# castorini/dhr

Measured on AMD Instinct MI355X. Metric: queries/sec (exact top-1000, brute-force dense-hybrid GIP retrieval), higher is better.
Workload: dtype i8 (bound GEMM: gated AND ungated columns int8 x int8 -> int32 on the matrix cores, every gated rounding upward, the ungated quantisation error paid by the filter margin) + f64-accumulated f16 x f32 exact rescoring of the survivors -- the returned scores are the exact scores rounded once, identical

## Files before the change

dhr_amd/csrc/dhr_internal.h:

```cpp
#pragma once
#include <hip/hip_runtime.h>
#include <hip/hip_fp16.h>
#include <stdint.h>

#include "../../include/dhr_hip.h"
#include "abi_guard.h"

extern "C" int dhr_set_error_message(int code, const char* msg);
extern "C" int dhr_index_device(const dhr_index* ix);
extern "C" void dhr_internal_index_arena(dhr_index* ix, void*** base, size_t** bytes);
extern "C" int dhr_internal_search_begin_async(dhr_index* ix, const dhr_query_batch* qb, int32_t k, float* out_sample_scores_dev, void* stream);
extern "C" void dhr_internal_search_abort(dhr_index* ix);
extern "C" int dhr_internal_search_pre_async(dhr_index* ix, const dhr_query_batch* qb, int32_t k, int32_t r_local, float* out_scores_dev, void* stream);
extern "C" int dhr_internal_search_begin_rest_async(dhr_index* ix, const float* tau_dev, float* out_sample_scores_dev, void* stream);
extern "C" int dhr_internal_search_mid_async(dhr_index* ix, const float* tau_hat_dev, int32_t r_local, float* out_scores_dev, void* stream);
extern "C" int dhr_internal_search_finish_async(dhr_index* ix, const float* tau_hat_dev, float* out_scores, int64_t* out_rows, int32_t* out_count_dev,
                                                int32_t out_mem_kind, void* stream);

namespace dhr {

constexpr int TILE_ROWS = 256;
constexpr int TILE_K = 64;
constexpr int CHUNK = 8;
constexpr int TILE_HALVES = TILE_ROWS * TILE_K;
// ... 127 lines not shown
__host__ __device__ inline int quant_i8(float v, float inv_scale) {
  float r = rintf(v * inv_scale);
  r = r < -127.f ? -127.f : (r > 127.f ? 127.f : r);
  return (int)r;
}

struct RescoreArgs {
  const __half* vals_rm;
  const void* c_idx;
  int c_idx_dtype;
  const float* q32;
  const int16_t* q_idx;
  const __half* q16; const uint8_t* q_idx8; const uint32_t* q_inexact;
  int d_dlr, k_rm;
  int gate;
  int64_t n_rows;
  const uint2* cand; const uint32_t* cnt; uint32_t cap;
  const uint32_t* rows32;
  int64_t ld_rows;
  int64_t row0; uint32_t count_all;
  const float* thr_exact;
  uint64_t* out_keys;
  int64_t ld_keys;
  float* out_scores;
  int64_t ld_scores;
  int n_queries;
  uint32_t max_count;
  const uint32_t* blk_off; uint32_t flat_blocks;
  int split;
};

struct SelectArgs {
  uint64_t* topk_keys;
  const uint64_t* in_keys;
  int64_t ld_keys;
  const uint32_t* cnt;
  uint32_t count_all, cap;
  int k, kp, sort_n;
  int k_keep;
  int kps;
  int monotone;
  const float* margin;
  float* tau;
  float* thr;
  int n_queries;
};

hipError_t launch_scan_rows(const __half* src, int64_t ld, int64_t n_rows, int d_dlr, int k, uint32_t* max_sq_bits,
                            uint32_t* neg_flag, hipStream_t s);
hipError_t launch_i8_row_err(const __half* vals_rm, int k_rm, int64_t n_rows, int d_dlr, int d_cls, float scale, const float* col_scale,
                             uint32_t* out_bits, hipStream_t s);
hipError_t launch_col_absmax(const __half* vals_rm, int k_rm, int64_t n_rows, int col0, int n_cols, uint32_t* colmax_bits, hipStream_t s);
hipError_t launch_tile_rows_sparse(const __half* src, int64_t ld, int64_t row_lo, int64_t n_rows_src, int64_t n_rows_fill,
                                   int d_dlr, int d_cls, int ts, int td, const void* idx, int idx_dtype, const uint8_t* map,
                                   bool abs_dlr, char* tiles, float i8_inv_scale , const float* col_scale,
                                   const float* g8_inv_cs , hipStream_t s);
hipError_t launch_g8_row_sum(const __half* vals_rm, int k_rm, int64_t n_rows, int64_t n_rows_fill, int d_dlr, bool abs_dlr, const float* g8_inv_cs,
                             int32_t* rsum128, hipStream_t s);
hipError_t launch_copy_rows(const __half* src, int64_t ld, int64_t n_rows, int k, int k_rm, __half* dst, hipStream_t s);
hipError_t launch_idx_hist(const uint8_t* idx, const __half* vals_rm, int k_rm, int64_t n_rows, int d_dlr, float* hist, hipStream_t s);
struct G8Prep {
  const float* inv_cs;
  const float* w;
  float s_ref;
  int max_shift;
  uint8_t* q8;
  int32_t* shift;
  float* unit;
  float* thr_raise;
  float resid_ec2;
};
hipError_t launch_query_prep(const void* src, int src_is_f32, int64_t ld, const void* idx, int idx_dtype, int64_t ld_idx,
                             int n_queries, int q_pad, int d_dlr, int d_cls, int k_rm, int n_buckets, int kt,
                             const uint8_t* map, bool abs_dlr, float dmax, __half* q_tiles, float* q32, int16_t* q_idx,
                             float* margin, float* tau, float* thr, int ts, int td, uint32_t* q_pack, __half* q16, uint8_t* q_idx8,
                             uint32_t* q_inexact, int c_idx_dtype,
                             float i8_scale , float i8_ec, float i8_nc, float* i8_mul, const float* col_scale,
                             const G8Prep& g8, hipStream_t s);
#if defined(__HIPCC__)
constexpr int MAP_SPREAD_Q = 0x100;
__device__ __forceinline__ bool gemm_wg_tile(const GemmArgs& p, int64_t& dt, int& qt) {
  const int r = (int)blockIdx.y;
  const int mode = p.map_mode;
  int64_t seq;
  if (mode & MAP_SPREAD_Q) {
    const int qg = r / DOC_GROUP;
    const int dl = r - qg * DOC_GROUP;
    qt = qg * 8 + (int)blockIdx.x;
    if (qt >= p.n_qtiles) return false;
    seq = p.seq_lo + (int64_t)blockIdx.z * DOC_GROUP + dl;
  } else {
    qt = r / DOC_GROUP;
    const int dl = r - qt * DOC_GROUP;
    seq = p.seq_lo + ((int64_t)blockIdx.z * 8 + (int64_t)blockIdx.x) * DOC_GROUP + dl;
  }
  if (seq >= p.seq_hi) return false;
  dt = seq_to_tile_fast(seq, mode & 0xff, p.period, p.head, p.perm_mul, p.perm_n, p.inv_perm_n, p.inv_pm1);
  return dt < p.n_tiles;
}
#endif
inline int sparse_query_stages(int ts, bool gated, bool g8 = false) { return ts > 0 ? ((gated || g8) ? ts : 2 * ts) : 0; }
hipError_t launch_gemm_filter(const GemmArgs& a, hipStream_t s);
hipError_t launch_heavy_build(const __half* vals_rm, int k_rm, const void* idx, int idx_dtype, int64_t n_rows, int d_dlr,
                              const uint8_t* map, int n_buckets, uint32_t* heavy_key, __half* heavy_val,
                              const float* g8_inv_cs , int abs_mode, hipStream_t s);
#ifndef REFINE_PER_WG_N
#define REFINE_PER_WG_N 512
#endif
constexpr int REFINE_PER_WG = REFINE_PER_WG_N;
struct RefineArgs {
  const uint2* cand; const uint32_t* cnt; uint32_t cap;
  const uint2* ovf; const uint32_t* ovf_off; const uint32_t* ovf_cap;
  const uint32_t* heavy_key; const __half* heavy_val;
  const uint32_t* q_pack; int d_dlr;
  const float* thr;
  uint2* out; uint32_t* out_cnt; uint32_t out_cap;
  int n_queries; uint32_t max_count;
  const uint32_t* blk_off; uint32_t flat_blocks;
  const uint8_t* g8_q8;
  const float* g8_inv_cs;
  const float* g8_unit;
  int abs_mode;
  int ungated;
  const uint8_t* resid8; int resid_ld;
  const float* q32; int64_t q32_ld;
  const float* col_scale; int d_cls;
  const float* thr_raise;
};
hipError_t launch_resid_build(const __half* vals_rm, int k_rm, int64_t n_rows, int d_dlr, int d_cls, const float* col_scale, uint8_t* resid8, int resid_ld, hipStream_t s);
hipError_t launch_refine(const RefineArgs& a, hipStream_t s);
hipError_t launch_rescore(const RescoreArgs& a, hipStream_t s);
hipError_t launch_select(const SelectArgs& a, hipStream_t s);
hipError_t launch_select_global(const SelectArgs& a, hipStream_t s);
hipError_t launch_merge_topk_global(int n_queries, int n_in, const float* in_scores, const int64_t* in_rows, int k_out, float* out_scores,
                                    int64_t* out_rows, hipStream_t s);
hipError_t launch_emit(const uint64_t* topk_keys, int kp, int n_queries, int k, int64_t row_offset, float* out_scores,
                       int64_t* out_rows, hipStream_t s);
hipError_t launch_keys_to_rows(const uint64_t* topk_keys, int kp, int n_queries, int k, uint32_t* rows, hipStream_t s);
hipError_t launch_bound_topm(const float* bound , int n_rows, int n_queries, int m, uint32_t* rows , hipStream_t s);
hipError_t launch_densify(const void* lex, int in_is_f32, int64_t ld, int64_t batch, int remove, int dims, int n_groups, void* out_val,
                          int val_is_f32, int64_t ld_val, void* out_idx, int idx_is_i16, int64_t ld_idx, hipStream_t s);
hipError_t launch_pq_init(const __half* vals, int64_t ld, int64_t n, int64_t stride, int dsub, int M, float* cb, int ksub, hipStream_t s);
hipError_t launch_pq_assign(const __half* vals, int64_t ld, int64_t n, int64_t stride, int dsub, int M, const float* cb, uint8_t* codes,
                            int64_t ld_codes, float* sums, uint32_t* counts, float* err, int ksub, hipStream_t s);
hipError_t launch_pq_update(float* cb, const float* sums, const uint32_t* counts, int dsub, int M, int ksub, hipStream_t s);
hipError_t launch_pq_decode(const uint8_t* codes, int64_t ld_codes, int64_t n, int M, int dsub, const float* cb, __half* out, int64_t ld_out,
                            int ksub, hipStream_t s);
hipError_t launch_block_offsets(const uint32_t* cnt, uint32_t cap, int n_queries, uint32_t per, uint32_t* offs, hipStream_t s);
hipError_t launch_plan_overflow(const uint32_t* cnt_prev, double rows_ratio, uint32_t cap, uint32_t max_extra, uint32_t arena_entries, int n_queries,
                                uint32_t* ovf_off, uint32_t* ovf_cap, hipStream_t s);
hipError_t launch_max_u32(const uint32_t* v, int n, uint32_t* out_max, unsigned long long* out_sum, hipStream_t s);
hipError_t launch_lists_ready(const uint32_t* cnt, uint32_t cap, int n_queries, uint32_t per, uint32_t* offs, uint32_t* out_max, uint32_t* out_max2,
                              unsigned long long* out_sum, unsigned long long* out_sum2, uint32_t* fail_flags, uint32_t* zero, int n_zero,
                              hipStream_t s, const uint32_t* ovf_cap = nullptr);
hipError_t launch_rows_to_local(const int64_t* rows, int64_t n, int64_t row_offset, int64_t n_rows, uint32_t* out,
                                hipStream_t s);
hipError_t launch_mark_overflow(const uint32_t* cnt, uint32_t cap, int n_queries, uint32_t* fail_flags, hipStream_t s);
hipError_t launch_verify(const uint64_t* topk_keys, int kp, int k, const float* tau_hat, int n_queries, uint32_t* fail_flags,
                         uint32_t* n_fail, hipStream_t s);
hipError_t launch_gather_queries(const float* q32, const int16_t* q_idx, int k_rm, int d_dlr, const int32_t* ids, int n,
                                 float* out32, int16_t* out_idx, hipStream_t s);
hipError_t launch_scatter_keys(const uint64_t* src, uint64_t* dst, int kp, const int32_t* ids, int n, hipStream_t s);
hipError_t launch_emit_scores(const uint64_t* topk_keys, int kp, int n_queries, int r, float* out, hipStream_t s);
hipError_t launch_make_thr(const float* tau, const float* margin, int n_queries, int q_pad, float* thr, hipStream_t s);
hipError_t launch_raise_thr(float* thr_hat, const float* thr_run, int n_queries, hipStream_t s);
hipError_t launch_flag_tau_above(const float* tau_own, const float* tau_ext, int n_queries, uint32_t* fail_flags, hipStream_t s);
hipError_t launch_raise_thr_rank(float* thr_hat, float* tau_hat, const uint64_t* topk_keys, int kp, int r, const float* margin, int n_queries, hipStream_t s);
hipError_t launch_count_ge(const uint64_t* topk_keys, int kp, int k, const float* tau, const uint32_t* fail_flags, int n_queries,
                           int32_t* out, hipStream_t s);
hipError_t launch_merge_topk(int n_queries, int n_in, const float* in_scores, const int64_t* in_rows, int k_out,
                             float* out_scores, int64_t* out_rows, hipStream_t s);
hipError_t launch_merge_lists(int n_queries, int n_lists, int list_len, const float* in_scores, const int64_t* in_rows, int k_out,
                              float* out_scores, int64_t* out_rows, hipStream_t s, int64_t stride_s = 0, int64_t stride_r = 0);

extern int g_gemm_variant;
extern thread_local int g_last_gemm_kernel;
constexpr int RESCORE_CANDS_PER_WG = 32;
constexpr uint32_t FLAT_GRID_MAX = 1u << 20;
constexpr uint32_t FLAT_GRID_ASYNC = 16384;
constexpr int SELECT_THREADS = 1024;

}
```

dhr_amd/csrc/dhr_state.h:

```cpp
#pragma once
#include <algorithm>
#include <cmath>
#include <cstdio>
#include <cstring>
#include <string>
#include <vector>

#include "dhr_internal.h"
#include "search_plan.h"
#include <hip/hip_ext.h>

using namespace dhr;
static_assert(plan::TILE_ROWS == TILE_ROWS && plan::DOC_GROUP == DOC_GROUP, "search_plan.h restates the tile geometry of dhr_internal.h");
using plan::BOOT_M;
using plan::SearchPlan;
using plan::round_up;

inline int set_error(int code, const std::string& msg) { return dhr_set_error_message(code, msg.c_str()); }
#define HIP_TRY(expr)                                                                                          \
  do {                                                                                                         \
    hipError_t _e = (expr);                                                                                    \
    if (_e != hipSuccess)                                                                                      \
      return set_error(DHR_ERR_HIP, std::string(#expr) + ": " + hipGetErrorString(_e) + " (" __FILE__ ":" +    \
                                        std::to_string(__LINE__) + ")");                                       \
  } while (0)

struct DevMem {
  void* p = nullptr;
  DevMem() = default;
  DevMem(const DevMem&) = delete;
  DevMem& operator=(const DevMem&) = delete;
  ~DevMem() { if (p) (void)hipFree(p); }
};
struct Events {
  std::vector<hipEvent_t> v;
  Events() = default;
  Events(const Events&) = delete;
  Events& operator=(const Events&) = delete;
  ~Events() { for (hipEvent_t e : v) if (e) (void)hipEventDestroy(e); }
  hipError_t add(hipEvent_t* out, unsigned flags = hipEventDefault) {
    v.reserve(v.size() + 1);
    hipEvent_t e = nullptr;
    const hipError_t rc = hipEventCreateWithFlags(&e, flags);
    if (rc == hipSuccess) v.push_back(e);
    *out = e;
    return rc;
  }
};
static inline int idx_esize(int dt) { return dt == DHR_IDX_I16 ? 2 : 1; }

struct Workspace {
  int q_pad = 0, kp = 0;
  int q_alloc = 0;
  int64_t cap = 0;
  int64_t cap_deep = 0;
  int64_t arena = 0;
  uint2 *ovf = nullptr, *ovf2 = nullptr;
  uint32_t *ovf_off = nullptr, *ovf_cap = nullptr;
  uint32_t* boot_rows = nullptr;
  float* boot_bound = nullptr;
  bool keys_alias = false;
  ListTier* tier_dev = nullptr;
  uint32_t* cnt_plan = nullptr;
  int64_t plan_rows = 0;
  uint32_t last_maxr = 0;
  int64_t cap_r = 0;
  int64_t keys_ld = 0, kt = 0, d_dlr = 0;
  int ts_q = 0;
  __half* q_tiles = nullptr;
  float* q32 = nullptr;
  int16_t* q_idx = nullptr;
  __half* q16 = nullptr;
  uint8_t* q_idx8 = nullptr;
  uint32_t* q_inexact = nullptr;
  float *margin = nullptr, *tau = nullptr, *thr = nullptr;
  float* i8_mul = nullptr;
  uint8_t* g8_q8 = nullptr;
  int32_t* g8_shift = nullptr;
  float* g8_unit = nullptr;
  uint32_t* cnt = nullptr;
  uint2* cand = nullptr;
  uint64_t *rs_keys = nullptr, *topk_keys = nullptr;
  uint32_t* d_max = nullptr;
  float* tau_hat = nullptr;
  float* thr_hat = nullptr;
  uint32_t* fail_flags = nullptr;
  uint32_t* q_pack = nullptr;
  float* thr_raise = nullptr;
  uint2* cand_r = nullptr;
  uint32_t* cnt_r = nullptr;
  uint32_t* blk_off = nullptr;
  uint2* cand2 = nullptr;
  uint32_t* cnt2 = nullptr;
  void* h_pinned = nullptr;
  char* h_pinned2 = nullptr;
  uint32_t* d_max2 = nullptr;
  unsigned long long* d_stats = nullptr;
  void* h_stats = nullptr;
  uint32_t* d_ref = nullptr;
  void* h_ref = nullptr;
  void* q_stage = nullptr;  size_t q_stage_bytes = 0;
  void* qi_stage = nullptr; size_t qi_stage_bytes = 0;
  void* out_stage = nullptr; size_t out_stage_bytes = 0;
  int64_t bytes = 0;
};

enum class StagedState { None, AfterPre, AfterBegin, AfterMid, Complete };
enum class Stage { Whole, Begin, Finish, Mid, Pre, BeginRest };

struct dhr_index {
  int device = 0;
  int64_t n_rows = 0, n_tiles = 0, row_offset = 0;
  int d_dlr = 0, d_cls = 0, k = 0, idx_dtype = DHR_IDX_NONE;
  int dlr_pad = 0;
  int k_rm = 0;
  int n_buckets = 1;
  int idx_buckets_req = 0;
  int kt = 0;
  int ksteps = 0;
  int ts = 0, td = 0;
  __half* tiles = nullptr;
  __half* vals_rm = nullptr;
  void* c_idx = nullptr;
  uint8_t* bucket_map = nullptr;
  uint32_t* heavy_key = nullptr;
  __half* heavy_val = nullptr;
  bool abs_mode = false;
  float dmax = 0.f;
  bool dense_i8 = false;
  float i8_scale = 0.f, i8_ec = 0.f, i8_nc = 0.f;
  uint8_t* resid8 = nullptr;
  int resid_ld = 0;
  float resid_ec2 = 0.f;
  float* i8_col_scale = nullptr;
  bool gated_i8 = false;
  float g8_sref = 0.f;
  int g8_max_shift = 0;
  float* g8_inv_cs = nullptr;
  float* g8_w = nullptr;
  int32_t* g8_rsum = nullptr;
  int64_t index_bytes = 0;
  int64_t cand_cap = 0, first_rows = 0;
  int64_t list_stride = 0;
  int profile = 0, max_growth16 = 32;
  int sample_period = 32;
  int async_ctl = 2;
  int sample_share = 1;
  int main_chunks = 2;
  int progressive_thr = 2;
  int n_cu = 256;
  int gemm_variant = 0;
  int last_gemm_kernel = 0;
  int overlap_aux = -1;
  int aux_cus = -1, gemm_exclusive = 0;
  int aux_cus_made = -1, gemm_excl_made = -1;
  hipStream_t s_gemm = nullptr;
  hipStream_t s_aux = nullptr;
  struct {
    StagedState state = StagedState::None;
    bool gate = false; int Q = 0, k = 0;
    double rate = 0.0, rate_r = 0.0;
    int64_t dev_bound = 0, dev_exact = 0;
    int64_t pre_pos = 0, pre_seen = 0, pre_last_rows = 0;
  } pend;
  Workspace ws, ws_fb[2];
  void* sh_arena = nullptr;
  size_t sh_arena_bytes = 0;
  dhr_search_stats stats{};
};

inline void free_ws(Workspace& w) {
  hipFree(w.q_tiles); hipFree(w.q32); hipFree(w.q_idx); hipFree(w.q16); hipFree(w.q_idx8); hipFree(w.q_inexact); hipFree(w.margin); hipFree(w.i8_mul); hipFree(w.g8_q8); hipFree(w.g8_shift); hipFree(w.g8_unit); hipFree(w.tau); hipFree(w.thr);
  hipFree(w.cnt); hipFree(w.cand); if (!w.keys_alias) hipFree(w.rs_keys); hipFree(w.topk_keys); hipFree(w.d_max); hipFree(w.tau_hat); hipFree(w.fail_flags); hipFree(w.thr_hat); hipFree(w.cand2); hipFree(w.cnt2); hipFree(w.q_pack); hipFree(w.cand_r); hipFree(w.cnt_r); hipFree(w.thr_raise); hipFree(w.blk_off); hipFree(w.ovf); hipFree(w.ovf2); hipFree(w.ovf_off); hipFree(w.ovf_cap); hipFree(w.cnt_plan); hipFree(w.tier_dev); hipFree(w.boot_rows); hipFree(w.boot_bound);
  if (w.h_pinned) hipHostFree(w.h_pinned);
  if (w.h_pinned2) hipHostFree(w.h_pinned2);
  hipFree(w.d_max2); hipFree(w.d_ref); hipFree(w.d_stats);
  if (w.h_ref) hipHostFree(w.h_ref);
  if (w.h_stats) hipHostFree(w.h_stats);
  hipFree(w.q_stage); hipFree(w.qi_stage); hipFree(w.out_stage);
  w = Workspace();
}


constexpr int32_t MEM_DEVICE_PADDED = 2;
#ifndef SELECT_SORT_Q
#define SELECT_SORT_Q 8
#endif
inline int select_sort_n(int kp) { return kp * SELECT_SORT_Q / 4; }
enum { T_GEMM = 0, T_REFINE = 1, T_RESCORE = 2, T_SELECT = 3, T_PREP = 4 };
struct Drain {
  dhr_index* ix; hipStream_t s; bool armed = true;
  ~Drain() {
    if (!armed) return;
    (void)hipStreamSynchronize(s);
    if (ix->s_aux) (void)hipStreamSynchronize(ix->s_aux);
    if (ix->s_gemm) (void)hipStreamSynchronize(ix->s_gemm);
    (void)hipGetLastError();
  }
};
struct Timer {
  bool on; hipStream_t s; std::vector<std::pair<hipEvent_t, hipEvent_t>> ev; std::vector<int> kind;
  ~Timer() { for (auto& e : ev) { (void)hipEventDestroy(e.first); (void)hipEventDestroy(e.second); } }
  void begin(int k) { begin_on(k, s); }
  void end() { end_on(s); }
  void begin_on(int k, hipStream_t st) { if (!on) return; ev.reserve(ev.size() + 1); kind.reserve(kind.size() + 1); hipEvent_t a, b; hipEventCreate(&a); hipEventCreate(&b); hipEventRecord(a, st); ev.push_back({a, b}); kind.push_back(k); }
  void end_on(hipStream_t st) { if (!on) return; hipEventRecord(ev.back().second, st); }
  void collect(double* ms ) {
    for (size_t i = 0; i < ev.size(); ++i) {
      float t = 0.f;
      if (hipEventElapsedTime(&t, ev[i].first, ev[i].second) == hipSuccess) ms[kind[i]] += t;
      hipEventDestroy(ev[i].first); hipEventDestroy(ev[i].second);
    }
    ev.clear(); kind.clear();
  }
};

int ensure_ws(dhr_index* ix, Workspace& w, int n_queries, int k, int64_t keys_ld_min, int64_t cap_mult = 1, bool use_refine = true, bool queries_only = false);
int check_queries(const dhr_index* ix, const dhr_query_batch* qb);
int grow(void*& p, size_t& have, size_t need, int64_t& total);
int prep_queries(dhr_index* ix, Workspace& w, const dhr_query_batch* qb, hipStream_t s);
dhr::RescoreArgs base_rescore_args(const dhr_index* ix, const Workspace& w, int n_queries, bool gate);
inline SearchPlan search_plan_of(const dhr_index* ix, int k, int depth, bool staged) {
  plan::PlanInput in;
  in.n_rows = ix->n_rows; in.n_tiles = ix->n_tiles; in.k = k; in.sample_period = ix->sample_period; in.sample_share = ix->sample_share;
  in.first_rows = ix->first_rows; in.depth = depth; in.staged = staged;
  return plan::make_search_plan(in);
}
inline void staged_set(dhr_index* ix, StagedState to) { ix->pend.state = to; }
inline void staged_open(dhr_index* ix, StagedState to, bool gate, int Q, int k) { staged_set(ix, to); ix->pend.gate = gate; ix->pend.Q = Q; ix->pend.k = k; }
int search_core(dhr_index* ix, Workspace& w, const dhr_query_batch* qb, int k, int depth, Timer& tm, dhr_search_stats& st, hipStream_t s,
                Stage stage = Stage::Whole, const float* tau_ext = nullptr);
```

dhr_amd/csrc/gemm_g8.hip:

```cpp
#include "gemm_g8.h"
#include <mutex>
#include <type_traits>

#ifndef G8_TRACE
#define G8_TRACE 0
#endif
#ifndef G8_ABL
#define G8_ABL 0
#endif
namespace dhr {

#if G8_TRACE
constexpr int G8_TRACE_SLOTS = 1 << 18;
__device__ unsigned long long g8_trace_buf[G8_TRACE_SLOTS * 8];
__device__ unsigned int g8_trace_n;
#define G8_T(i) do { if (threadIdx.x == 0 && tslot < G8_TRACE_SLOTS) g8_trace_buf[(size_t)tslot * 8 + (i)] = __builtin_readcyclecounter(); } while (0)
#else
#define G8_T(i) do { } while (0)
#endif
__device__ __forceinline__ void g8_dump_tile(const GemmArgs& p, floatx16 (&acc)[4][2], int64_t dt, int qt, int wm, int wn, int lane,
                                             const float (&mul_r)[2]) {
  const int fhalf = lane >> 5;
  const int64_t row_base = dt * TILE_ROWS + wm * 128;
#pragma unroll
  for (int ni = 0; ni < 2; ++ni) {
    const int q = qt * TILE_ROWS + wn * 64 + ni * 32 + (lane & 31);
    if (q < p.n_queries) {
#pragma unroll
      for (int mi = 0; mi < 4; ++mi)
#pragma unroll
        for (int e = 0; e < 16; ++e) {
          const int64_t row = row_base + mi * 32 + (e & 3) + 8 * (e >> 2) + 4 * fhalf;
          if (row < p.n_rows && row >= p.dump_row0 && row - p.dump_row0 < p.dump_ld)
            p.dump[(int64_t)q * p.dump_ld + (row - p.dump_row0)] = g8_score(__float_as_int(acc[mi][ni][e]), mul_r[ni]);
        }
    }
  }
}

template <bool SURPLUS, int NI_, bool CHECK_ROWS = true>
__device__ __forceinline__ void g8_scan_half(const GemmArgs& p, floatx16 (&acc)[4][2], int qt, int wm, int wn, int lane, int rows_valid, int64_t row0,
                                             uint2* stack, const int t, const float mul, uint32_t& j) {
  const int fhalf = lane >> 5;
  const int rbase = wm * 128 + 4 * fhalf;
  const int q = qt * TILE_ROWS + wn * 64 + NI_ * 32 + (lane & 31);
#pragma unroll
  for (int mi = 0; mi < 4; ++mi) {
    const floatx16& a = acc[mi][NI_];
#pragma unroll
    for (int g = 0; g < 4; ++g) {
      const int gm = max(max(__float_as_int(a[4 * g]), __float_as_int(a[4 * g + 1])), max(__float_as_int(a[4 * g + 2]), __float_as_int(a[4 * g + 3])));
      if (gm >= t) {
        asm volatile("");
        if constexpr (!SURPLUS && !CHECK_ROWS) {
#pragma unroll
          for (int e = 4 * g; e < 4 * g + 4; ++e) {
            const int v = __float_as_int(a[e]);
            const int rl = rbase + mi * 32 + (e & 3) + 8 * (e >> 2);
            const uint32_t slot = j < (uint32_t)EPI_STACK ? j : (uint32_t)EPI_STACK;
            stack[slot * G8_NT] = make_uint2((uint32_t)rl, (uint32_t)v);
            j += v >= t ? 1u : 0u;
          }
        } else
#pragma unroll
        for (int e = 4 * g; e < 4 * g + 4; ++e) {
          const int v = __float_as_int(a[e]);
          const int rl = rbase + mi * 32 + (e & 3) + 8 * (e >> 2);
          if (v >= t && (!CHECK_ROWS || rl < rows_valid)) {
            asm volatile("");
            if constexpr (SURPLUS) {
              if (j >= EPI_STACK) {
                const uint32_t slot = atomicAdd(p.cnt + q, 1u);
                cand_store(p, q, slot, make_uint2((uint32_t)(row0 + rl), __float_as_uint(g8_score(v, mul))));
              }
            } else if (j < EPI_STACK) stack[j * G8_NT] = make_uint2((uint32_t)rl, (uint32_t)v);
            ++j;
          }
        }
      }
    }
  }
}
__device__ __forceinline__ void g8_epilogue_surplus(const GemmArgs& p, floatx16 (&acc)[4][2], int qt, int wm, int wn, int lane, int rows_valid, int64_t row0,
                                                 const int (&thr_r)[2], const float (&mul_r)[2]) {
  uint32_t j = 0;
  g8_scan_half<true, 0>(p, acc, qt, wm, wn, lane, rows_valid, row0, nullptr, thr_r[0], mul_r[0], j);
  g8_scan_half<true, 1>(p, acc, qt, wm, wn, lane, rows_valid, row0, nullptr, thr_r[1], mul_r[1], j);
}
__device__ __forceinline__ void g8_epilogue(const GemmArgs& p, floatx16 (&acc)[4][2], int64_t dt, int qt, int wm, int wn, int tid, int lane,
                                            char* smem, const int (&thr_r)[2], const float (&mul_r)[2]) {
  __syncthreads();
  const int64_t row0 = dt * TILE_ROWS;
  const int rows_valid = (int)(p.n_rows - row0 < TILE_ROWS ? p.n_rows - row0 : TILE_ROWS);
  uint2* stack = (uint2*)smem + tid;
  const int q0 = qt * TILE_ROWS + wn * 64 + (lane & 31);
  const bool full = rows_valid == TILE_ROWS;
  uint32_t j = 0;
  if (full) g8_scan_half<false, 0, false>(p, acc, qt, wm, wn, lane, rows_valid, row0, stack, thr_r[0], mul_r[0], j);
  else g8_scan_half<false, 0, true>(p, acc, qt, wm, wn, lane, rows_valid, row0, stack, thr_r[0], mul_r[0], j);
  const uint32_t s0 = j < (uint32_t)EPI_STACK ? j : (uint32_t)EPI_STACK;
#if G8_ABL != 16
  uint32_t base0 = 0u, base1 = 0u;
  if (s0 > 0) base0 = atomicAdd(p.cnt + q0, s0);
#endif
  if (full) g8_scan_half<false, 1, false>(p, acc, qt, wm, wn, lane, rows_valid, row0, stack, thr_r[1], mul_r[1], j);
  else g8_scan_half<false, 1, true>(p, acc, qt, wm, wn, lane, rows_valid, row0, stack, thr_r[1], mul_r[1], j);
  const uint32_t s1 = j < (uint32_t)EPI_STACK ? j : (uint32_t)EPI_STACK;
#if G8_ABL == 16
  return;
#else
  if (s1 > s0) base1 = atomicAdd(p.cnt + q0 + 32, s1 - s0);
  if (__builtin_amdgcn_ballot_w64(j > (uint32_t)EPI_STACK) != 0) g8_epilogue_surplus(p, acc, qt, wm, wn, lane, rows_valid, row0, thr_r, mul_r);
  for (uint32_t i = 0; i < s0; ++i) {
    const uint2 en = stack[i * G8_NT];
    const uint32_t slot = base0 + i;
    cand_store(p, q0, slot, make_uint2((uint32_t)row0 + en.x, __float_as_uint(g8_score((int)en.y, mul_r[0]))));
  }
  for (uint32_t i = s0; i < s1; ++i) {
    const uint2 en = stack[i * G8_NT];
    const uint32_t slot = base1 + (i - s0);
    cand_store(p, q0 + 32, slot, make_uint2((uint32_t)row0 + en.x, __float_as_uint(g8_score((int)en.y, mul_r[1]))));
  }
#endif
}

#if G8_ABL == 2
#define G8_PAIR_SYNC() do { asm volatile("s_waitcnt lgkmcnt(0)" ::: "memory"); __builtin_amdgcn_s_barrier(); } while (0)
#elif G8_ABL == 3
#define G8_PAIR_SYNC() do { asm volatile("s_waitcnt lgkmcnt(0)" ::: "memory"); } while (0)
#else
#define G8_PAIR_SYNC() do { asm volatile("s_waitcnt vmcnt(0) lgkmcnt(0)" ::: "memory"); __builtin_amdgcn_s_barrier(); } while (0)
#endif

#ifndef G8_DMA_SCHED
#define G8_DMA_SCHED 1
#endif
#if G8_DMA_SCHED == 1
__host__ __device__ constexpr int g8_dma_piece(int ph, int g) { return ph == 0 ? g : -1; }
#elif G8_DMA_SCHED == 2
__host__ __device__ constexpr int g8_dma_piece(int ph, int g) { return ph == 0 ? (g >= 2 ? g - 2 : -1) : (ph == 1 && g < 2) ? 6 + g : -1; }
#else
__host__ __device__ constexpr int g8_dma_piece(int ph, int g) { return (ph <= 1 && (g & 1)) ? ph * 4 + (g >> 1) : -1; }
#endif

template <bool DUMP, bool PARTIAL>
__device__ __forceinline__ void g8_tile(const GemmArgs& p, char* smem, const int64_t dt, const int qt, const unsigned tslot = 0) {
  const int lane = threadIdx.x & 63;
  const int wave = __builtin_amdgcn_readfirstlane(threadIdx.x >> 6);
  const int ts = p.ts, td = p.td;
  const int nsp = ts >> 1, npairs = (ts + td) >> 1;
  const char* a_src = (const char*)p.a_tiles + dt * ((int64_t)ts * S8_STAGE_A + (int64_t)td * SP_DENSE);
  const char* b_src = (const char*)p.b_tiles + (int64_t)qt * ((int64_t)ts * SP_STAGE_B + (int64_t)td * SP_DENSE);
  const int wm = PARTIAL ? (wave & 1) : (wave >> 2), wn = PARTIAL ? (wave >> 1) : (wave & 3);
  const bool active = !PARTIAL || wn < p.partial_wn;

  const bool dma_b = ((wave >> 1) & 1) != 0;
  const int dma_s = wave >> 2;
  const int dma_h = wave & 1;
  const uint32_t lane_off = (uint32_t)lane * 16u;
  const uint32_t smem_u = (uint32_t)(uintptr_t)LDS_PTR(smem);
  const __amdgpu_buffer_rsrc_t role_rsrc = __builtin_amdgcn_make_buffer_rsrc((void*)(dma_b ? b_src : a_src), (short)0, 0x7fffffff, 0x00020000);
  int dma_soff = 0, dma_n = 0, nx_soff = 0, nx_n = 0;
  uint32_t dma_lds = 0, nx_lds = 0;
  auto dma_prepare = [&](int g) __attribute__((always_inline)) {
    const int u = 2 * g + dma_s;
    const bool sp = u < ts;
    const int half_bytes = dma_h * ((!dma_b && sp) ? S8_STAGE_A / 2 : 8192);
    if (dma_b) nx_soff = (sp ? u * SP_STAGE_B : ts * SP_STAGE_B + (u - ts) * SP_DENSE) + half_bytes;
    else nx_soff = (sp ? u * S8_STAGE_A : ts * S8_STAGE_A + (u - ts) * SP_DENSE) + half_bytes;
    nx_lds = smem_u + (uint32_t)((u & 3) * G8_SLOT + (dma_b ? G8_QOFF : 0) + half_bytes);
    nx_n = g < npairs ? ((!dma_b && sp) ? 5 : 8) : 0;
    if ((G8_ABL == 4 || G8_ABL == 8) && g >= 2) nx_n = 0;
  };
  auto dma_commit = [&]() __attribute__((always_inline)) { dma_soff = nx_soff; dma_lds = nx_lds; dma_n = nx_n; };
  auto dma_piece = [&](int j) __attribute__((always_inline)) {
    if (j < dma_n) {
      __attribute__((address_space(3))) void* l = (__attribute__((address_space(3))) void*)(uintptr_t)(dma_lds + (uint32_t)(j >> 2) * 4096u);
      const int so = dma_soff + (j >> 2) * 4096;
      switch (j & 3) {
        case 0: __builtin_amdgcn_raw_ptr_buffer_load_lds(role_rsrc, l, 16, (int)lane_off, so, 0, 0); break;
        case 1: __builtin_amdgcn_raw_ptr_buffer_load_lds(role_rsrc, l, 16, (int)lane_off, so, 1024, 0); break;
        case 2: __builtin_amdgcn_raw_ptr_buffer_load_lds(role_rsrc, l, 16, (int)lane_off, so, 2048, 0); break;
        default: __builtin_amdgcn_raw_ptr_buffer_load_lds(role_rsrc, l, 16, (int)lane_off, so, 3072, 0); break;
      }
    }
  };
  auto issue_pair = [&](int g) {
    dma_prepare(g);
    dma_commit();
#pragma unroll
    for (int j = 0; j < 8; ++j) dma_piece(j);
  };

  floatx16 acc[4][2];
  const int frow = lane & 31;
  const int fhalf = lane >> 5;
  const int swz4 = (frow >> 2) & 3;
  const int c0 = (fhalf ^ swz4) << 4, c1 = ((2 + fhalf) ^ swz4) << 4;
  const int a8_off = ((wm * 8 + fhalf) * 32 + frow) * 16;
  const int p8_off = S8_A_BYTES + ((wm * 2 + fhalf) * 32 + frow) * 16;
  const int ad_row = (wm * 128 + frow) * 64;
  const int q_row = G8_QOFF + (wn * 64 + frow) * 64;

  auto read_s8 = [&](G8Frag& f, const char* sl, int g) __attribute__((always_inline)) {
    if (g < 4) f.b[g >> 1].h[g & 1] = *(const intx4*)(sl + q_row + (g >> 1) * 2048 + ((g & 1) ? c1 : c0));
    else if (g < 8) f.a[g - 4] = *(const intx4*)(sl + a8_off + (g - 4) * 1024);
    else if (g == 8) f.pw = *(const intx4*)(sl + p8_off);
  };
  auto read_dn = [&](G8Frag& f, const char* sl, int cc, int g) __attribute__((always_inline)) {
    if (g < 2) f.b[g].h[0] = *(const intx4*)(sl + q_row + g * 2048 + cc);
    else if (g < 6) f.a[g - 2] = *(const intx4*)(sl + ad_row + (g - 2) * 2048 + cc);
  };
  auto blk_s8 = [&](const G8Frag& fc, G8Frag& fn, int un, bool do_load, auto ph_c) __attribute__((always_inline)) {
    constexpr int PH = decltype(ph_c)::value;
    const char* sl = smem + (un & 3) * G8_SLOT;
#pragma unroll
    for (int g = 0; g < 8; ++g) {
      const int ni = g >> 2, mi = g & 3;
      if (!PARTIAL || active) {
        if (do_load && G8_ABL != 8) {
          read_s8(fn, sl, g);
          if (g == 0) read_s8(fn, sl, 8);
        }
        g8_smfmac(acc[mi][ni], fc.a[mi], fc.b[ni].v, (uint32_t)fc.pw[mi]);
      }
      if (g8_dma_piece(PH, g) >= 0) dma_piece(g8_dma_piece(PH, g));
      __builtin_amdgcn_sched_barrier(0);
    }
  };
  auto blk_dn = [&](const G8Frag& fc, G8Frag& fn, int tn, bool do_load, auto ph_c) __attribute__((always_inline)) {
    constexpr int PH = decltype(ph_c)::value;
    const char* sl = smem + ((ts + (tn >> 1)) & 3) * G8_SLOT;
    const int cc = (tn & 1) ? c1 : c0;
#pragma unroll
    for (int g = 0; g < 8; ++g) {
      const int ni = g >> 2, mi = g & 3;
      if (!PARTIAL || active) {
        if (do_load && G8_ABL != 8) read_dn(fn, sl, cc, g);
        g8_mfma(acc[mi][ni], fc.a[mi], fc.b[ni].h[0]);
      }
      if (g8_dma_piece(PH, g) >= 0) dma_piece(g8_dma_piece(PH, g));
      __builtin_amdgcn_sched_barrier(0);
    }
  };

  if (wave < 4 && (ts > 0 || wave == 1 || wave == 2)) {
    const char* src = wave == 0 ? (const char*)(p.g8_rsum + dt * TILE_ROWS) : wave == 1 ? (const char*)(p.i8_mul + qt * TILE_ROWS)
                    : wave == 2 ? (const char*)(p.thr + qt * TILE_ROWS) : (const char*)(p.g8_shift + qt * TILE_ROWS);
    __builtin_amdgcn_global_load_lds(GLOBAL_PTR(src + lane_off), LDS_PTR(smem + G8_META + wave * 1024), 16, 0, 0);
  }
  issue_pair(0);
  if (npairs > 1) {
    issue_pair(1);
    if (dma_n == 5) asm volatile("s_waitcnt vmcnt(5)" ::: "memory"); else asm volatile("s_waitcnt vmcnt(8)" ::: "memory");
  } else asm volatile("s_waitcnt vmcnt(0)" ::: "memory");
  __builtin_amdgcn_s_barrier();
  G8_T(2);
  if (ts > 0) {
    const int32_t* rs = (const int32_t*)(smem + G8_META) + wm * 128 + 4 * (lane >> 5);
#pragma unroll
    for (int mi = 0; mi < 4; ++mi)
#pragma unroll
      for (int g4 = 0; g4 < 4; ++g4) {
        const intx4 v = *(const intx4*)(rs + mi * 32 + 8 * g4);
#pragma unroll
        for (int i4 = 0; i4 < 4; ++i4) acc[mi][0][4 * g4 + i4] = acc[mi][1][4 * g4 + i4] = __int_as_float(v[i4]);
      }
  } else {
#pragma unroll
    for (int mi = 0; mi < 4; ++mi)
#pragma unroll
      for (int e = 0; e < 16; ++e) acc[mi][0][e] = acc[mi][1][e] = 0.f;
  }
  int sh_r[2];
  float mul_r[2], thr_f[2];
#pragma unroll
  for (int ni = 0; ni < 2; ++ni) {
    const int ql = wn * 64 + ni * 32 + (lane & 31);
    mul_r[ni] = ((const float*)(smem + G8_META + 1024))[ql];
    thr_f[ni] = ((const float*)(smem + G8_META + 2048))[ql];
    sh_r[ni] = ts > 0 ? ((const int*)(smem + G8_META + 3072))[ql] : 0;
    asm volatile("" : "+v"(mul_r[ni]), "+v"(thr_f[ni]), "+v"(sh_r[ni]));
  }
  G8Frag f0, f1;
  if (ts > 0) {
#pragma unroll
    for (int g = 0; g < 9; ++g) read_s8(f0, smem, g);
  }
  if (G8_ABL == 8) f1 = f0;
  constexpr std::integral_constant<int, 0> PH0{};
  constexpr std::integral_constant<int, 1> PH1{};
  constexpr std::integral_constant<int, 2> PH2{};
  dma_n = 0;
#pragma unroll 1
  for (int g = 0; g + 1 < nsp; ++g) {
    blk_s8(f0, f1, 2 * g + 1, true, PH1);
    dma_prepare(g + 2);
    __builtin_amdgcn_sched_barrier(0);
    G8_PAIR_SYNC();
    dma_commit();
    blk_s8(f1, f0, 2 * g + 2, true, PH0);
  }
  if (nsp > 0) {
    const int g = nsp - 1;
    blk_s8(f0, f1, 2 * g + 1, true, PH1);
    dma_prepare(g + 2);
    __builtin_amdgcn_sched_barrier(0);
    G8_PAIR_SYNC();
    dma_commit();
    blk_s8(f1, f0, 2 * g + 2, false, PH0);
  }
  G8_T(3);
  if (td > 0) {
    __builtin_amdgcn_sched_barrier(0);
    asm volatile("s_waitcnt lgkmcnt(0)\n\ts_nop 15\n\ts_nop 7" ::: "memory");
    __builtin_amdgcn_sched_barrier(0);
    if (ts > 0)
#pragma unroll
    for (int mi = 0; mi < 4; ++mi)
#pragma unroll
      for (int ni = 0; ni < 2; ++ni)
#pragma unroll
        for (int e = 0; e < 16; ++e) acc[mi][ni][e] = __uint_as_float(__float_as_uint(acc[mi][ni][e]) << sh_r[ni]);
    __builtin_amdgcn_sched_barrier(0);
    {
      const char* sl = smem + (ts & 3) * G8_SLOT;
#pragma unroll
      for (int g = 0; g < 6; ++g) read_dn(f0, sl, c0, g);
    }
    asm volatile("s_nop 4" ::: "memory");
    __builtin_amdgcn_sched_barrier(0);
#pragma unroll 1
    for (int g = nsp; g + 1 < npairs; ++g) {
      const int t0 = 4 * (g - nsp);
      blk_dn(f0, f1, t0 + 1, true, PH1);
      blk_dn(f1, f0, t0 + 2, true, PH2);
      blk_dn(f0, f1, t0 + 3, true, PH2);
      dma_prepare(g + 2);
      __builtin_amdgcn_sched_barrier(0);
      G8_PAIR_SYNC();
      dma_commit();
      blk_dn(f1, f0, t0 + 4, true, PH0);
    }
    {
      const int g = npairs - 1;
      const int t0 = 4 * (g - nsp);
      blk_dn(f0, f1, t0 + 1, true, PH1);
      blk_dn(f1, f0, t0 + 2, true, PH2);
      blk_dn(f0, f1, t0 + 3, true, PH2);
      dma_prepare(g + 2);
      __builtin_amdgcn_sched_barrier(0);
      G8_PAIR_SYNC();
      dma_commit();
      blk_dn(f1, f0, t0 + 4, false, PH0);
    }
  }
  G8_T(4);
  asm volatile("s_waitcnt vmcnt(0) lgkmcnt(0)\n\ts_nop 15\n\ts_nop 7" ::: "memory");
  G8_T(5);
  if (DUMP) { g8_dump_tile(p, acc, dt, qt, wm, wn, lane, mul_r); return; }
  int thr_r[2];
#pragma unroll
  for (int ni = 0; ni < 2; ++ni) {
    asm volatile("" : "+v"(thr_f[ni]));
    thr_r[ni] = g8_thr_units(thr_f[ni], mul_r[ni]);
  }
#if G8_ABL == 32
  if (p.n_queries >= 0) { if (__float_as_int(acc[0][0][0]) == 0x7fffffff) p.cnt[0] = 1; return; }
#endif
  if (PARTIAL && !active) { __syncthreads(); return; }
  g8_epilogue(p, acc, dt, qt, wm, wn, (int)threadIdx.x, lane, smem, thr_r, mul_r);
}

#define G8_KERNEL_ATTR __attribute__((amdgpu_waves_per_eu(2, 2)))
template <bool DUMP>
__global__ void __launch_bounds__(G8_NT) G8_KERNEL_ATTR gemm_filter_g8_kernel(GemmArgs p) {
  extern __shared__ __attribute__((aligned(16))) char smem[];
  int64_t dt;
  int qt;
  if (!gemm_wg_tile(p, dt, qt)) return;
#if G8_TRACE
  unsigned tslot = 0;
  if (threadIdx.x == 0) tslot = atomicAdd(&g8_trace_n, 1u);
  tslot = __builtin_amdgcn_readfirstlane(tslot);
  if (threadIdx.x == 0 && tslot < G8_TRACE_SLOTS) {
    unsigned hw, xcc;
    asm volatile("s_getreg_b32 %0, hwreg(HW_REG_HW_ID)" : "=s"(hw));
    asm volatile("s_getreg_b32 %0, hwreg(HW_REG_XCC_ID)" : "=s"(xcc));
    g8_trace_buf[(size_t)tslot * 8 + 0] = __builtin_amdgcn_s_memrealtime();
    g8_trace_buf[(size_t)tslot * 8 + 7] = (unsigned long long)hw | ((unsigned long long)(xcc & 0xf) << 32) | ((unsigned long long)qt << 40) | ((unsigned long long)(dt & 0xffff) << 48);
  }
  G8_T(1);
  if (!DUMP && p.partial_wn > 0 && qt == p.n_qtiles - 1) g8_tile<false, true>(p, smem, dt, qt, tslot);
  else g8_tile<DUMP, false>(p, smem, dt, qt, tslot);
  G8_T(6);
#else
  if (!DUMP && p.partial_wn > 0 && qt == p.n_qtiles - 1) g8_tile<false, true>(p, smem, dt, qt);
  else g8_tile<DUMP, false>(p, smem, dt, qt);
#endif
}
#if G8_TRACE
}
extern "C" int dhr_debug_g8_trace(unsigned long long* out, int max_slots, unsigned* n_out) try {
  unsigned n = 0;
  if (hipMemcpyFromSymbol(&n, HIP_SYMBOL(dhr::g8_trace_n), 4) != hipSuccess) return -1;
  if (n_out) *n_out = n;
  const unsigned m = n < (unsigned)max_slots ? n : (unsigned)max_slots;
  const unsigned mm = m < (unsigned)dhr::G8_TRACE_SLOTS ? m : (unsigned)dhr::G8_TRACE_SLOTS;
  if (out && mm && hipMemcpyFromSymbol(out, HIP_SYMBOL(dhr::g8_trace_buf), (size_t)mm * 64) != hipSuccess) return -1;
  const unsigned zero = 0;
  if (hipMemcpyToSymbol(HIP_SYMBOL(dhr::g8_trace_n), &zero, 4) != hipSuccess) return -1;
  return 0;
} DHR_CATCH_STATUS
namespace dhr {
#endif

hipError_t launch_gemm_g8(const GemmArgs& a, dim3 grid, hipStream_t s) {
  static std::mutex attr_mu;
  static bool attr_set_dev[64] = {};
  int dev_ = 0;
  (void)hipGetDevice(&dev_);
  {
    std::lock_guard<std::mutex> attr_lock(attr_mu);
    bool& attr_set = attr_set_dev[dev_ & 63];
    if (!attr_set) {
      hipError_t e = hipFuncSetAttribute((const void*)gemm_filter_g8_kernel<false>, hipFuncAttributeMaxDynamicSharedMemorySize, G8_RING_LDS);
      if (e != hipSuccess) return e;
      e = hipFuncSetAttribute((const void*)gemm_filter_g8_kernel<true>, hipFuncAttributeMaxDynamicSharedMemorySize, G8_RING_LDS);
      if (e != hipSuccess) return e;
      attr_set = true;
    }
  }
  if (a.dump) { hipLaunchKernelGGL(gemm_filter_g8_kernel<true>, grid, dim3(G8_NT), G8_RING_LDS, s, a); return hipGetLastError(); }
  GemmArgs b = a;
  constexpr int partial_on = 1;
  const int valid_last = a.n_queries - (a.n_qtiles - 1) * TILE_ROWS;
  b.partial_wn = (partial_on && valid_last > 0 && valid_last <= 128) ? (valid_last + 63) / 64 : 0;
  hipLaunchKernelGGL(gemm_filter_g8_kernel<false>, grid, dim3(G8_NT), G8_RING_LDS, s, b);
  return hipGetLastError();
}

}
```

dhr_amd/csrc/index_build.hip:

```cpp
#include <fcntl.h>
#include <sys/mman.h>
#include <sys/stat.h>
#include <unistd.h>

#include "dhr_state.h"

extern "C" void dhr_index_destroy(dhr_index* ix) try {
  if (!ix) return;
  hipSetDevice(ix->device);
  free_ws(ix->ws);
  free_ws(ix->ws_fb[0]);
  free_ws(ix->ws_fb[1]);
  if (ix->s_aux) hipStreamDestroy(ix->s_aux);
  if (ix->s_gemm) hipStreamDestroy(ix->s_gemm);
  hipFree(ix->sh_arena);
  hipFree(ix->resid8); hipFree(ix->i8_col_scale); hipFree(ix->g8_inv_cs); hipFree(ix->g8_w); hipFree(ix->g8_rsum); hipFree(ix->tiles); hipFree(ix->c_idx); hipFree(ix->vals_rm); hipFree(ix->bucket_map); hipFree(ix->heavy_key);
  delete ix;
} DHR_CATCH_VOID

static int g_opt_dense_i8 = -1;
static int g_opt_gated_i8 = -1;
constexpr int64_t GATED_I8_MIN_ROWS = 1000000, GATED_I8_MIN_ROWS_NARROW = 4000000;
constexpr int64_t DENSE_ONLY_I8_MIN_ROWS = 1000000;
extern "C" int dhr_set_option(int32_t option, int64_t value) try {
  if (option == DHR_OPT_DENSE_I8) { g_opt_dense_i8 = value < 0 ? -1 : (value != 0); return DHR_OK; }
  if (option == DHR_OPT_GATED_I8) { g_opt_gated_i8 = value < 0 ? -1 : (value != 0); return DHR_OK; }
  return set_error(DHR_ERR_INVALID, "unknown option");
} DHR_CATCH_STATUS
extern "C" int dhr_index_get_info(const dhr_index* ix, int32_t what, double* out) try {
  if (!ix || !out) return set_error(DHR_ERR_INVALID, "null argument");
  switch (what) {
    case DHR_INFO_DENSE_I8: *out = ix->dense_i8 ? 1.0 : 0.0; return DHR_OK;
    case DHR_INFO_I8_SCALE: *out = ix->i8_scale; return DHR_OK;
    case DHR_INFO_I8_ROW_ERR: *out = ix->i8_ec; return DHR_OK;
    case DHR_INFO_I8_ROW_NORM: *out = ix->i8_nc; return DHR_OK;
    case DHR_INFO_ROW_NORM_MAX: *out = ix->dmax; return DHR_OK;
    case DHR_INFO_GATED_I8: *out = ix->gated_i8 ? 1.0 : 0.0; return DHR_OK;
    case DHR_INFO_GEMM_KERNEL: *out = (double)ix->last_gemm_kernel; return DHR_OK;
    case DHR_INFO_TILE_BYTES: *out = (double)((size_t)ix->n_tiles * ((size_t)ix->ts * (ix->gated_i8 ? S8_STAGE_A : SP_STAGE_A) + (size_t)ix->td * SP_DENSE)); return DHR_OK;
  }
  return set_error(DHR_ERR_INVALID, "unknown info id");
} DHR_CATCH_STATUS

extern "C" int dhr_index_set_param(dhr_index* ix, int32_t param, int64_t value) try {
  if (!ix) return set_error(DHR_ERR_INVALID, "null index");
  switch (param) {
    case DHR_PARAM_CAND_CAP:
      if (value < DOC_GROUP * TILE_ROWS || value > (1 << 22)) return set_error(DHR_ERR_INVALID, "cand_cap must be in [1024, 4194304]");
      ix->cand_cap = value; return DHR_OK;
    case DHR_PARAM_FIRST_ROWS:
      if (value < 0) return set_error(DHR_ERR_INVALID, "first_rows must be >= 0");
      ix->first_rows = value; return DHR_OK;
    case DHR_PARAM_PROFILE: ix->profile = value != 0; return DHR_OK;
    case DHR_PARAM_SAMPLE_PERIOD:
      if (value < 0 || value > 256) return set_error(DHR_ERR_INVALID, "sample_period must be in [0,256] (0/1 = off)");
      ix->sample_period = (int)value; return DHR_OK;
    case DHR_PARAM_ASYNC_CONTROLLER: ix->async_ctl = value < 0 ? 0 : (value > 2 ? 2 : (int)value); return DHR_OK;
    case DHR_PARAM_LIST_STRIDE:
      if (value != 0 && (value < DOC_GROUP * TILE_ROWS || value > (1 << 22) || value % 256))
        return set_error(DHR_ERR_INVALID, "list_stride must be 0 (default) or a multiple of 256 in [1024, 4194304]");
      ix->list_stride = value; return DHR_OK;
    case DHR_PARAM_SAMPLE_SHARE:
      if (value < 1 || value > 4096) return set_error(DHR_ERR_INVALID, "sample_share must be in [1,4096]");
      ix->sample_share = (int)value; return DHR_OK;
    case DHR_PARAM_MAIN_CHUNKS:
      if (value < 1 || value > 64) return set_error(DHR_ERR_INVALID, "main_chunks must be in [1,64]");
      ix->main_chunks = (int)value; return DHR_OK;
    case DHR_PARAM_PROGRESSIVE_THR: ix->progressive_thr = value < 0 ? 0 : (value > 2 ? 2 : (int)value); return DHR_OK;
    case DHR_PARAM_AUX_CUS:
      if (value < 0 || value > 192 || value % 8) return set_error(DHR_ERR_INVALID, "aux_cus must be a multiple of 8 in [0,192]");
      ix->aux_cus = (int)value; return DHR_OK;
    case DHR_PARAM_GEMM_EXCLUSIVE: ix->gemm_exclusive = value != 0; return DHR_OK;
    case DHR_PARAM_OVERLAP_AUX: ix->overlap_aux = value < 0 ? -1 : value != 0; return DHR_OK;
    case DHR_PARAM_GEMM_VARIANT:
#ifdef DHR_AB_VARIANTS
      if (value == 6) { ix->gemm_variant = 6; return DHR_OK; }
#endif
      if (value != 4 && value != 5) return set_error(DHR_ERR_INVALID, "gemm_variant: 4 (4 waves, 128 x 128 wave tiles) or 5 (8 waves, 128 x 64 wave tiles; default) -- the fp16-gated kernel; integer (gated_i8) indexes have one kernel");
      ix->gemm_variant = (int)value; return DHR_OK;
    case DHR_PARAM_MAX_GROWTH:
      if (value < 1 || value > 1024) return set_error(DHR_ERR_INVALID, "max_growth must be in [1,1024] sixteenths");
      ix->max_growth16 = (int)value; return DHR_OK;
  }
  return set_error(DHR_ERR_INVALID, "unknown parameter");
} DHR_CATCH_STATUS

extern "C" int dhr_index_device(const dhr_index* ix) try { return ix ? ix->device : -1; } DHR_CATCH_VALUE(-1)
extern "C" void dhr_internal_index_arena(dhr_index* ix, void*** base, size_t** bytes) try { *base = &ix->sh_arena; *bytes = &ix->sh_arena_bytes; } DHR_CATCH_VOID
extern "C" int64_t dhr_index_device_bytes(const dhr_index* ix) try { return ix ? ix->index_bytes + ix->ws.bytes + ix->ws_fb[0].bytes + ix->ws_fb[1].bytes + (int64_t)ix->sh_arena_bytes : 0; } DHR_CATCH_VALUE(0)
extern "C" int dhr_get_stats(const dhr_index* ix, dhr_search_stats* out) try {
  if (!ix || !out) return set_error(DHR_ERR_INVALID, "null argument");
  *out = ix->stats;
  return DHR_OK;
} DHR_CATCH_STATUS

static int ingest(dhr_index* ix, const dhr_index_desc* d, uint32_t* d_flags , void* stage, int64_t block_rows,
                  hipStream_t s) {
  const int64_t n = ix->n_rows;
  for (int64_t lo = 0; lo < n; lo += block_rows) {
    const int64_t rows = std::min(block_rows, n - lo);
    const __half* src;
    int64_t ld;
    if (ix->dlr_pad > 0) {
      const hipMemcpyKind kind = d->mem_kind == DHR_MEM_HOST ? hipMemcpyHostToDevice : hipMemcpyDeviceToDevice;
      const int d_in = ix->d_dlr - ix->dlr_pad;
      const char* base = (const char*)d->value + lo * d->ld_value * 2;
      HIP_TRY(hipMemcpy2DAsync(stage, (size_t)ix->k * 2, base, (size_t)d->ld_value * 2, (size_t)d_in * 2, (size_t)rows, kind, s));
      if (ix->d_cls > 0)
        HIP_TRY(hipMemcpy2DAsync((char*)stage + (size_t)ix->d_dlr * 2, (size_t)ix->k * 2, base + (size_t)d_in * 2, (size_t)d->ld_value * 2,
                                 (size_t)ix->d_cls * 2, (size_t)rows, kind, s));
      src = (const __half*)stage;
      ld = ix->k;
    } else if (d->mem_kind == DHR_MEM_HOST) {
      HIP_TRY(hipMemcpy2DAsync(stage, (size_t)ix->k * 2, (const char*)d->value + lo * d->ld_value * 2,
                               (size_t)d->ld_value * 2, (size_t)ix->k * 2, (size_t)rows, hipMemcpyHostToDevice, s));
      src = (const __half*)stage;
      ld = ix->k;
    } else {
      src = (const __half*)d->value + lo * d->ld_value;
      ld = d->ld_value;
    }
    HIP_TRY(launch_scan_rows(src, ld, rows, ix->d_dlr, ix->k, d_flags, d_flags + 1, s));
    HIP_TRY(launch_copy_rows(src, ld, rows, ix->k, ix->k_rm, ix->vals_rm + lo * ix->k_rm, s));
    if (d->mem_kind == DHR_MEM_HOST || ix->dlr_pad > 0) HIP_TRY(hipStreamSynchronize(s));
  }
  return DHR_OK;
}
static int build_tiles(dhr_index* ix, hipStream_t s) {
  const int64_t n = ix->n_rows, fill = ix->n_tiles * TILE_ROWS;
  HIP_TRY(launch_tile_rows_sparse(ix->vals_rm, ix->k_rm, 0, n, fill, ix->d_dlr, ix->d_cls, ix->ts, ix->td, ix->c_idx, ix->idx_dtype,
                                  ix->bucket_map, ix->abs_mode, (char*)ix->tiles, ix->dense_i8 ? 1.f / ix->i8_scale : 0.f, ix->i8_col_scale,
                                  ix->gated_i8 ? ix->g8_inv_cs : nullptr, s));
  return DHR_OK;
}

static void build_bucket_map(const std::vector<float>& hist, int d_dlr, int nb, std::vector<uint8_t>& map) {
  map.assign((size_t)d_dlr * 256, 0);
  std::vector<int> order(256);
  std::vector<double> load(nb);
  for (int j = 0; j < d_dlr; ++j) {
    const float* h = &hist[(size_t)j * 256];
    for (int v = 0; v < 256; ++v) order[v] = v;
    std::stable_sort(order.begin(), order.end(), [&](int a, int b) { return h[a] > h[b]; });
    std::fill(load.begin(), load.end(), 0);
    int rr = 0;
    for (int v : order) {
      int best = 0;
      if (h[v] == 0) best = rr++ % nb;
      else
        for (int b = 1; b < nb; ++b)
          if (load[b] < load[best]) best = b;
      map[(size_t)j * 256 + v] = (uint8_t)best;
      load[best] += h[v];
    }
  }
}

extern "C" int dhr_index_create(const dhr_index_desc* d_user, dhr_index** out) try {
  if (!d_user || !out) return set_error(DHR_ERR_INVALID, "null argument");
  dhr_index_desc d_padded = *d_user;
  const int dlr_pad = (d_user->d_dlr > 0 && d_user->index != nullptr && d_user->d_dlr % 8) ? 8 - d_user->d_dlr % 8 : 0;
  if (d_user->ld_value < (int64_t)d_user->d_dlr + d_user->d_cls) return set_error(DHR_ERR_INVALID, "bad value pointer / ld_value");
  if (d_user->index && d_user->index_dtype != DHR_IDX_NONE && d_user->ld_index < d_user->d_dlr) return set_error(DHR_ERR_INVALID, "bad ld_index");
  d_padded.d_dlr += dlr_pad;
  if (dlr_pad) { d_padded.ld_value = std::max<int64_t>(d_padded.ld_value, (int64_t)d_padded.d_dlr + d_padded.d_cls); d_padded.ld_index = std::max<int64_t>(d_padded.ld_index, d_padded.d_dlr); }
  const dhr_index_desc* d = &d_padded;
  *out = nullptr;
  if (d->n_rows <= 0 || d->n_rows >= (int64_t)0xFFFFFF00ll) return set_error(DHR_ERR_INVALID, "n_rows must be in [1, 2^32-256)");
  if (d->d_dlr < 0 || d->d_cls < 0 || d->d_dlr + d->d_cls <= 0) return set_error(DHR_ERR_INVALID, "bad d_dlr/d_cls");
  if (!d->value || d->ld_value < d->d_dlr + d->d_cls) return set_error(DHR_ERR_INVALID, "bad value pointer / ld_value");
  const bool has_idx = d->index != nullptr && d->index_dtype != DHR_IDX_NONE;
  if (has_idx != (d->d_dlr > 0))
    return set_error(DHR_ERR_INVALID, "an index array is required iff d_dlr > 0 (dense-only: index=NULL, d_dlr=0)");
  if (has_idx && (d->index_dtype < DHR_IDX_U8 || d->index_dtype > DHR_IDX_I16)) return set_error(DHR_ERR_INVALID, "bad index_dtype");
  if (has_idx && d->ld_index < d->d_dlr) return set_error(DHR_ERR_INVALID, "bad ld_index");
  if (d->d_dlr + d->d_cls > 8192) return set_error(DHR_ERR_UNSUPPORTED, "more than 8192 columns");
  if (d->idx_buckets < 0 || d->idx_buckets > 2)
    return set_error(d->idx_buckets > 2 ? DHR_ERR_UNSUPPORTED : DHR_ERR_INVALID, "idx_buckets must be 0 (default: 2), 1 (ungated bound) or 2: the bucket-split operands of more than two buckets went with the K-step tile layout (round 6)");
  if (d->mem_kind != DHR_MEM_HOST && d->mem_kind != DHR_MEM_DEVICE) return set_error(DHR_ERR_INVALID, "bad mem_kind");
  dhr::alloc_checkpoint();
  HIP_TRY(hipSetDevice(d->device));

  struct Build {
    dhr_index* ix = nullptr; void* stage = nullptr; uint32_t* d_flags = nullptr; uint32_t* d_hist = nullptr;
    ~Build() { (void)hipFree(stage); (void)hipFree(d_flags); (void)hipFree(d_hist); if (ix) dhr_index_destroy(ix); }
  } build;
  dhr_index* ix = build.ix = new dhr_index();
  ix->device = d->device;
  ix->idx_buckets_req = d->idx_buckets;
  { hipDeviceProp_t pr; HIP_TRY(hipGetDeviceProperties(&pr, d->device)); ix->n_cu = pr.multiProcessorCount; }
  ix->n_rows = d->n_rows;
  ix->row_offset = d->row_offset;
  ix->d_dlr = d->d_dlr;
  ix->d_cls = d->d_cls;
  ix->dlr_pad = dlr_pad;
  ix->k = d->d_dlr + d->d_cls;
  ix->k_rm = (int)round_up(ix->k, TILE_K);
  auto even_up = [](int v) { return v + (v & 1); };
  int want_i8 = g_opt_dense_i8;
  if (const char* e = getenv("DHR_DENSE_I8")) want_i8 = atoi(e);
  bool dense_only_trial = false;
  if (has_idx) {
    ix->n_buckets = d->idx_buckets == 1 ? 1 : 2;
    ix->ts = even_up((d->d_dlr + 31) / 32);
    ix->dense_i8 = d->d_cls > 0 && (want_i8 < 0 || want_i8 > 0);
    ix->td = ix->dense_i8 ? 2 * ((d->d_cls + 127) / 128) : even_up((d->d_cls + 31) / 32);
    ix->kt = ix->ts * TILE_K + ix->td * 32;
    int want_g8 = g_opt_gated_i8;
    if (const char* e = getenv("DHR_GATED_I8")) want_g8 = atoi(e);
    if (want_g8 < 0) want_g8 = d->n_rows >= (2 * d->d_cls >= d->d_dlr ? GATED_I8_MIN_ROWS : GATED_I8_MIN_ROWS_NARROW) ? 1 : 0;
    ix->gated_i8 = want_g8 != 0 && ix->n_buckets == 2 && (d->d_cls == 0 || ix->dense_i8) && d->d_dlr <= 4096;
  } else {
    ix->n_buckets = 1;
    ix->ts = 0;
    dense_only_trial = want_i8 < 0 && d->n_rows >= DENSE_ONLY_I8_MIN_ROWS && d->d_cls >= 128;
    ix->dense_i8 = want_i8 > 0 || dense_only_trial;
    ix->td = ix->dense_i8 ? 2 * ((d->d_cls + 127) / 128) : even_up((d->d_cls + 31) / 32);
    ix->kt = ix->td * 32;
  }
  ix->ksteps = (ix->kt + TILE_K - 1) / TILE_K;
  ix->idx_dtype = has_idx ? d->index_dtype : DHR_IDX_NONE;
// ... 298 lines not shown
```

dhr_amd/csrc/kernels.hip:

```cpp
#include <algorithm>
#include <cstdlib>
#include <mutex>

#include "dhr_internal.h"
#include "gemm_common.h"
#include <type_traits>

namespace dhr {

typedef short short8 __attribute__((ext_vector_type(8)));

static hipError_t ensure_lds_attr(const void* fn, int bytes, int (&have)[64]) {
  static std::mutex mu;
  int dev = 0;
  (void)hipGetDevice(&dev);
  std::lock_guard<std::mutex> lock(mu);
  if (bytes <= have[dev & 63]) return hipSuccess;
  const hipError_t e = hipFuncSetAttribute(fn, hipFuncAttributeMaxDynamicSharedMemorySize, bytes);
  if (e == hipSuccess) have[dev & 63] = bytes;
  return e;
}

__device__ __forceinline__ float wave_sum(float v) {
#pragma unroll
// ... 446 lines not shown
        *(half8*)(tile + (int64_t)st * SP_STAGE_B + r * 64 + ((cc ^ ((r >> 2) & 3)) * 16)) = o.h;
      } else if (c < ts_q * 4) {
        const int st = c >> 2, cc = c & 3;
        const int kb = cc >> 1, hh = cc & 1;
        const int cst = st < ts ? st : st - ts;
#pragma unroll
        for (int e8 = 0; e8 < 8; ++e8) {
          float v = 0.f;
          const int j = cst * 32 + kb * 16 + 8 * (e8 >> 2) + 4 * hh + (e8 & 3);
          bool neg_b = false;
          if (j < d_dlr) {
            v = qval(j);
            v = abs_dlr ? fabsf(v) : fmaxf(v, 0.f);
            neg_b = (idx ? bucket_of(qidx(j), j, map, 2) : (st >= ts)) != 0;
          }
          _Float16 hv = (i8_scale > 0.f && v > 0.f) ? half_up(v * i8_inv_q) : (_Float16)v;
          h8[e8] = neg_b ? -hv : hv;
        }
        *(half8*)(tile + (int64_t)st * SP_STAGE_B + r * 64 + ((cc ^ ((r >> 2) & 3)) * 16)) = h8;
      } else if (i8_scale > 0.f) {
        const int dc = c - ts_q * 4, st = dc >> 2, cc = dc & 3;
        union { half8 h; int8_t b[16]; } o;
#pragma unroll
        for (int e = 0; e < 16; ++e) {
          const int j = d_dlr + dc * 16 + e;
          o.b[e] = (i8_zero || j >= k) ? (int8_t)0 : (int8_t)quant_i8(qval(j) * (col_scale[j - d_dlr] * (1.f / i8_scale)), i8_inv_q);
        }
        *(half8*)(tile + (int64_t)ts_q * SP_STAGE_B + (int64_t)st * SP_DENSE + r * 64 + ((cc ^ ((r >> 2) & 3)) * 16)) = o.h;
      } else {
        const int dc = c - ts_q * 4, st = dc >> 2, cc = dc & 3;
#pragma unroll
        for (int e8 = 0; e8 < 8; ++e8) h8[e8] = (_Float16)qval(d_dlr + dc * 8 + e8);
        *(half8*)(tile + (int64_t)ts_q * SP_STAGE_B + (int64_t)st * SP_DENSE + r * 64 + ((cc ^ ((r >> 2) & 3)) * 16)) = h8;
      }
    }
  }
  s16 = wave_sum(s16);
  sr = wave_sum(sr);
  if (lane == 0) {
    float m = 1.05f * (float)(kt + 256) * 5.9604645e-8f * sqrtf(s16) * dmax + 1.0001f * sqrtf(sr) * dmax;
    if (g8.inv_cs) {
      m = 1.001f * (i8_qn * i8_ec + i8_qe * i8_nc) + 1.2e-6f * (i8_qn + i8_qe) * i8_nc + 2.f * g8_uf;
      if (!(m >= 0.f)) m = INFINITY;
      i8_mul[q] = real ? g8_uf : 0.f;
      g8.shift[q] = g8_sh;
      g8.unit[q] = ldexpf(g8_uf, g8_sh);
    } else
    if (i8_scale > 0.f) {
      const float mul = __uint_as_float(__float_as_uint(i8_scale * i8_sq) + 8u);
      m += 1.001f * (i8_qn * i8_ec + i8_qe * i8_nc) + 1.2e-6f * (i8_qn + i8_qe) * i8_nc + 4.f * (float)(2 * (idx ? ts : 2 * ts) + 8) * mul;
      if (!(m >= 0.f)) m = INFINITY;
      i8_mul[q] = real ? mul : 0.f;
      if (g8.thr_raise) {
        const float gone = 1.001f * i8_qn * i8_ec;
        const float left = 1.01f * i8_qn * g8.resid_ec2 + 1e-3f * gone + 4e-6f * (i8_qn + i8_qe) * i8_nc;
        const float up = gone - left;
        g8.thr_raise[q] = (up > 0.f && m < INFINITY) ? up : 0.f;
      }
    }
    margin[q] = m;
    tau[q] = -INFINITY;
    thr[q] = real ? -INFINITY : INFINITY;
  }
}

hipError_t launch_query_prep(const void* src, int src_is_f32, int64_t ld, const void* idx, int idx_dtype, int64_t ld_idx,
                             int n_queries, int q_pad, int d_dlr, int d_cls, int k_rm, int n_buckets, int kt,
                             const uint8_t* map, bool abs_dlr, float dmax, __half* q_tiles, float* q32, int16_t* q_idx,
                             float* margin, float* tau, float* thr, int ts, int td, uint32_t* q_pack, __half* q16, uint8_t* q_idx8,
                             uint32_t* q_inexact, int c_idx_dtype, float i8_scale, float i8_ec, float i8_nc, float* i8_mul,
                             const float* col_scale, const G8Prep& g8, hipStream_t s) {
  hipLaunchKernelGGL(query_prep_kernel, dim3((q_pad + 3) / 4), dim3(256), 0, s, src, src_is_f32, ld, idx, idx_dtype,
                     ld_idx, n_queries, q_pad, d_dlr, d_cls, k_rm, n_buckets, kt, map, abs_dlr ? 1 : 0, dmax, q_tiles, q32,
                     q_idx, margin, tau, thr, ts, td, q_pack, q16, q_idx8, q_inexact, c_idx_dtype, i8_scale, i8_ec, i8_nc, i8_mul, col_scale, g8);
  return hipGetLastError();
}


int g_gemm_variant = 5;

thread_local int g_last_gemm_kernel = 0;
static hipError_t launch_gemm_filter_grid(const GemmArgs& a, dim3 grid, hipStream_t s);
hipError_t launch_gemm_filter(const GemmArgs& a_in, hipStream_t s) {
  static bool env_read = false;
  if (!env_read) {
    if (const char* e = getenv("DHR_GEMM_VARIANT")) g_gemm_variant = atoi(e) == 4 ? 4 : 5;
    env_read = true;
  }
  const int64_t n_tiles = a_in.seq_hi - a_in.seq_lo;
  if (n_tiles <= 0) return hipSuccess;
  const int64_t groups = (n_tiles + DOC_GROUP - 1) / DOC_GROUP;
  const int64_t groups_per_xcd = (groups + 7) / 8;
  if ((int64_t)DOC_GROUP * a_in.n_qtiles > 65535 || a_in.perm_n >= (1 << 24) || a_in.period > (1 << 20)) return hipErrorInvalidValue;
  if (a_in.map_mode >= 2 && a_in.period < 2) return hipErrorInvalidValue;
#ifdef DHR_AB_VARIANTS
  static const int g8_persist = getenv("DHR_G8_PERSIST") ? atoi(getenv("DHR_G8_PERSIST")) : 0;
  if (a_in.g8_shift && (g8_persist || a_in.variant == 6) && gemm_g8p_ok(a_in)) { g_last_gemm_kernel = 6; return launch_gemm_g8p(a_in, s); }
#endif
  GemmArgs a = a_in;
  a.inv_perm_n = 1.0 / (double)(a.perm_n > 0 ? a.perm_n : 1);
  a.inv_pm1 = 1.0 / (double)(a.period > 1 ? a.period - 1 : 1);
  if (groups < 8) {
    a.map_mode |= MAP_SPREAD_Q;
    const dim3 grid(8u, (unsigned)(DOC_GROUP * ((a.n_qtiles + 7) / 8)), (unsigned)groups);
    return launch_gemm_filter_grid(a, grid, s);
  }
  for (int64_t z0 = 0; z0 < groups_per_xcd; z0 += 65535) {
    GemmArgs c = a;
    c.seq_lo = a.seq_lo + z0 * 8 * DOC_GROUP;
    const dim3 grid(8u, (unsigned)(DOC_GROUP * a.n_qtiles), (unsigned)std::min<int64_t>(65535, groups_per_xcd - z0));
    const hipError_t e = launch_gemm_filter_grid(c, grid, s);
    if (e != hipSuccess) return e;
  }
  return hipSuccess;
}
static hipError_t launch_gemm_filter_grid(const GemmArgs& a, dim3 grid, hipStream_t s) {
  const int variant = a.variant == 4 ? 4 : a.variant ? 5 : g_gemm_variant;
  if (a.ts + a.td <= 0 || (a.ts & 1) || (a.td & 1) || (a.ts_q & 1)) return hipErrorInvalidValue;
  if (a.g8_shift) { g_last_gemm_kernel = 5; return (a.ts > 0 && a.ts_q == a.ts) ? launch_gemm_g8(a, grid, s) : hipErrorInvalidValue; }
  static const int dense_g8 = getenv("DHR_DENSE_G8") ? atoi(getenv("DHR_DENSE_G8")) : 1;
  if (a.i8_mul && dense_g8 && a.ts == 0 && a.ts_q == 0 && a.td > 0) { g_last_gemm_kernel = 5; return launch_gemm_g8(a, grid, s); }
  g_last_gemm_kernel = variant == 4 ? 4 : 3;
  return launch_gemm_wx(a, grid, variant, s);
}

__global__ void __launch_bounds__(1024) block_offsets_kernel(const uint32_t* __restrict__ cnt, uint32_t cap, int n_queries, uint32_t per,
                                                             uint32_t* __restrict__ offs) {
  __shared__ uint32_t part[1024];
  const int tid = threadIdx.x;
  const int chunk = (n_queries + 1023) / 1024;
  const int lo = tid * chunk, hi = min(lo + chunk, n_queries);
  uint32_t s = 0;
  for (int q = lo; q < hi; ++q) { uint32_t c = cnt[q]; if (c > cap) c = cap; s += (c + per - 1) / per; }
  part[tid] = s;
  __syncthreads();
  for (int d = 1; d < 1024; d <<= 1) {
    const uint32_t v = tid >= d ? part[tid - d] : 0u;
    __syncthreads();
    part[tid] += v;
    __syncthreads();
  }
  uint32_t run = tid ? part[tid - 1] : 0u;
  for (int q = lo; q < hi; ++q) { offs[q] = run; uint32_t c = cnt[q]; if (c > cap) c = cap; run += (c + per - 1) / per; }
  if (tid == 1023) offs[n_queries] = part[1023];
}
hipError_t launch_block_offsets(const uint32_t* cnt, uint32_t cap, int n_queries, uint32_t per, uint32_t* offs, hipStream_t s) {
  hipLaunchKernelGGL(block_offsets_kernel, dim3(1), dim3(1024), 0, s, cnt, cap, n_queries, per, offs);
  return hipGetLastError();
}
__global__ void __launch_bounds__(1024) lists_ready_kernel(const uint32_t* __restrict__ cnt, uint32_t cap, int n_queries, uint32_t per,
                                                           uint32_t* __restrict__ offs, uint32_t* __restrict__ out_max, uint32_t* __restrict__ out_max2,
                                                           unsigned long long* __restrict__ out_sum, unsigned long long* __restrict__ out_sum2,
                                                           uint32_t* __restrict__ fail_flags, uint32_t* __restrict__ zero, int n_zero,
                                                           const uint32_t* __restrict__ ovf_cap) {
  __shared__ uint32_t part[1024];
  __shared__ uint32_t wmax[16];
  __shared__ unsigned long long wsum[16];
  const int tid = threadIdx.x;
  const int chunk = (n_queries + 1023) / 1024;
  const int lo = tid * chunk, hi = min(lo + chunk, n_queries);
  uint32_t s = 0, m = 0;
  unsigned long long tot = 0;
  for (int q = lo; q < hi; ++q) {
    uint32_t c = cnt[q];
    m = c > m ? c : m;
    tot += c;
    const uint32_t cq = ovf_cap ? cap + ovf_cap[q] : cap;
    if (c > cq) { c = cq; if (fail_flags) fail_flags[q] = 1u; }
    s += (c + per - 1) / per;
  }
  part[tid] = s;
#pragma unroll
  for (int o = 32; o > 0; o >>= 1) {
    const uint32_t om = __shfl_xor(m, o, 64);
    m = om > m ? om : m;
    tot += __shfl_xor(tot, o, 64);
  }
  if ((tid & 63) == 0) { wmax[tid >> 6] = m; wsum[tid >> 6] = tot; }
  __syncthreads();
  for (int d = 1; d < 1024; d <<= 1) {
    const uint32_t v = tid >= d ? part[tid - d] : 0u;
    __syncthreads();
    part[tid] += v;
    __syncthreads();
  }
  uint32_t run = tid ? part[tid - 1] : 0u;
  for (int q = lo; q < hi; ++q) { offs[q] = run; uint32_t c = cnt[q]; const uint32_t cq = ovf_cap ? cap + ovf_cap[q] : cap; if (c > cq) c = cq; run += (c + per - 1) / per; }
  if (tid == 1023) offs[n_queries] = part[1023];
  if (tid == 0) {
    for (int i = 1; i < 16; ++i) { m = wmax[i] > m ? wmax[i] : m; tot += wsum[i]; }
    if (out_max) *out_max = m;
    if (out_max2) *out_max2 = m;
    if (out_sum) atomicAdd(out_sum, tot);
    if (out_sum2) atomicAdd(out_sum2, tot);
  }
  for (int j = tid; j < n_zero; j += 1024) zero[j] = 0u;
}
hipError_t launch_lists_ready(const uint32_t* cnt, uint32_t cap, int n_queries, uint32_t per, uint32_t* offs, uint32_t* out_max, uint32_t* out_max2,
                              unsigned long long* out_sum, unsigned long long* out_sum2, uint32_t* fail_flags, uint32_t* zero, int n_zero,
                              hipStream_t s, const uint32_t* ovf_cap) {
  hipLaunchKernelGGL(lists_ready_kernel, dim3(1), dim3(1024), 0, s, cnt, cap, n_queries, per, offs, out_max, out_max2, out_sum, out_sum2, fail_flags,
                     zero, n_zero, ovf_cap);
  return hipGetLastError();
}
__global__ void __launch_bounds__(1024) plan_overflow_kernel(const uint32_t* __restrict__ cnt_prev, double rows_ratio, uint32_t cap, uint32_t max_extra,
                                                             uint32_t arena_entries, int n_queries, uint32_t* __restrict__ ovf_off,
                                                             uint32_t* __restrict__ ovf_cap) {
  __shared__ unsigned long long part[1024];
  __shared__ double scale_s;
  const int tid = threadIdx.x;
  const int chunk = (n_queries + 1023) / 1024;
  const int lo = tid * chunk, hi = min(lo + chunk, n_queries);
  auto want = [&](int q) -> uint32_t {
    if (!cnt_prev) return 0u;
    const double need = 2.0 * (double)cnt_prev[q] * rows_ratio + 2048.0;
    if (!(need > (double)cap)) return 0u;
    const double extra = need - (double)cap;
    return extra >= (double)max_extra ? max_extra : (uint32_t)extra;
  };
  unsigned long long s = 0;
  for (int q = lo; q < hi; ++q) s += want(q);
  part[tid] = s;
  __syncthreads();
  for (int d = 512; d > 0; d >>= 1) {
    if (tid < d) part[tid] += part[tid + d];
    __syncthreads();
  }
  if (tid == 0) {
    const unsigned long long total = part[0] + 256ull * (unsigned long long)n_queries;
    scale_s = total > arena_entries ? (double)arena_entries / (double)total : 1.0;
  }
  __syncthreads();
  const double scale = scale_s;
  auto seg = [&](int q) -> uint32_t {
    const uint32_t w = want(q);
    if (w == 0u) return 0u;
    const uint32_t v = scale < 1.0 ? (uint32_t)((double)w * scale) : w;
    return (v + 255u) & ~255u;
  };
  __syncthreads();
  s = 0;
  for (int q = lo; q < hi; ++q) s += seg(q);
  part[tid] = s;
  __syncthreads();
  for (int d = 1; d < 1024; d <<= 1) {
    const unsigned long long v = tid >= d ? part[tid - d] : 0ull;
    __syncthreads();
    part[tid] += v;
    __syncthreads();
  }
  unsigned long long run = tid ? part[tid - 1] : 0ull;
  for (int q = lo; q < hi; ++q) {
    uint32_t w = seg(q);
    if (run >= arena_entries) w = 0u;
    else if (run + w > arena_entries) w = (uint32_t)(arena_entries - run);
    ovf_off[q] = (uint32_t)(run < arena_entries ? run : arena_entries);
    ovf_cap[q] = w;
    run += seg(q);
  }
}
hipError_t launch_plan_overflow(const uint32_t* cnt_prev, double rows_ratio, uint32_t cap, uint32_t max_extra, uint32_t arena_entries, int n_queries,
                                uint32_t* ovf_off, uint32_t* ovf_cap, hipStream_t s) {
  hipLaunchKernelGGL(plan_overflow_kernel, dim3(1), dim3(1024), 0, s, cnt_prev, rows_ratio, cap, max_extra, arena_entries, n_queries, ovf_off, ovf_cap);
  return hipGetLastError();
}
__device__ __forceinline__ bool flat_block(const uint32_t* __restrict__ offs, int n_queries, uint32_t b, int& q, uint32_t& blk) {
  if (b >= offs[n_queries]) return false;
  int lo = 0, hi = n_queries;
  while (hi - lo > 1) {
    const int mid = (lo + hi) >> 1;
    if (offs[mid] <= b) lo = mid; else hi = mid;
  }
  q = lo; blk = b - offs[lo];
  return true;
}

template <int SL>
__global__ void __launch_bounds__(256) heavy_build_kernel(const __half* __restrict__ vals_rm, int k_rm,
                                                          const void* __restrict__ idx, int idx_dtype, int64_t n_rows,
                                                          int d_dlr, const uint8_t* __restrict__ map, int n_buckets,
                                                          uint32_t* __restrict__ heavy_key, __half* __restrict__ heavy_val,
                                                          const float* __restrict__ g8_inv_cs, int abs_mode) {
  const int lane = threadIdx.x & 63;
  const int64_t wave0 = (int64_t)blockIdx.x * 4 + (threadIdx.x >> 6);
  const int64_t nwaves = (int64_t)gridDim.x * 4;
  for (int64_t row = wave0; row < n_rows; row += nwaves) {
    constexpr int MAXJ = 64 * SL - 1;
    uint32_t key[SL];
#pragma unroll
    for (int sl = 0; sl < SL; ++sl) {
      const int j = lane + 64 * sl;
      key[sl] = 0u;
      if (j < d_dlr) {
        union { _Float16 h; uint16_t u; } cv; cv.h = (_Float16)__half2float(vals_rm[row * k_rm + j]);
        const uint32_t mag = cv.u & 0x7FFFu;
        if (mag) key[sl] = (mag << 16) | (uint32_t)(MAXJ - j);
      }
    }
    for (int r = 0; r < HEAVY; ++r) {
      uint32_t best = 0u;
#pragma unroll
      for (int sl = 0; sl < SL; ++sl) best = key[sl] > best ? key[sl] : best;
#pragma unroll
      for (int o = 32; o > 0; o >>= 1) { const uint32_t ob = __shfl_xor(best, o, 64); best = ob > best ? ob : best; }
      if (best == 0u) {
        if (lane == 0) for (int rr = r; rr < HEAVY; ++rr) { heavy_key[row * HEAVY_KEY_STRIDE + heavy_key_word(rr)] = 0xFFFFFFFFu; heavy_val[row * HEAVY_VAL_STRIDE + heavy_val_half(rr)] = __float2half(0.f); }
        break;
      }
      const int j = MAXJ - (int)(best & 0xFFFFu);
      if ((j & 63) == lane) {
        const int iv = load_idx(idx, idx_dtype, row * d_dlr + j);
        const uint32_t bk = n_buckets > 1 ? (uint32_t)bucket_of(iv, j, map, n_buckets) : 0u;
        uint32_t key_out = ((uint32_t)j << 20) | (bk << 16) | ((uint32_t)iv & 0xFFFFu);
        if (g8_inv_cs) {
          float d = __half2float(vals_rm[row * k_rm + j]);
          if (abs_mode) d = fabsf(d);
          const uint32_t lvl = d > 0.f ? (uint32_t)quant_up_i8(d, g8_inv_cs[j]) : 0u;
          key_out = ((uint32_t)j << 20) | ((lvl >> 4) << 17) | ((bk & 1u) << 16) | ((lvl & 0xFu) << 12) | ((uint32_t)iv & 0xFFFu);
        }
        heavy_key[row * HEAVY_KEY_STRIDE + heavy_key_word(r)] = key_out;
        heavy_val[row * HEAVY_VAL_STRIDE + heavy_val_half(r)] = vals_rm[row * k_rm + j];
#pragma unroll
        for (int sl = 0; sl < SL; ++sl) if (sl == (j >> 6)) key[sl] = 0u;
      }
    }
  }
}
hipError_t launch_heavy_build(const __half* vals_rm, int k_rm, const void* idx, int idx_dtype, int64_t n_rows, int d_dlr,
                              const uint8_t* map, int n_buckets, uint32_t* heavy_key, __half* heavy_val, const float* g8_inv_cs, int abs_mode, hipStream_t s) {
  if (n_rows <= 0) return hipSuccess;
  const int64_t blocks = (n_rows + 3) / 4;
  if (d_dlr <= 1024)
    hipLaunchKernelGGL(heavy_build_kernel<16>, dim3((unsigned)(blocks < 16384 ? blocks : 16384)), dim3(256), 0, s, vals_rm, k_rm,
                       idx, idx_dtype, n_rows, d_dlr, map, n_buckets, heavy_key, heavy_val, g8_inv_cs, abs_mode);
  else
    hipLaunchKernelGGL(heavy_build_kernel<64>, dim3((unsigned)(blocks < 16384 ? blocks : 16384)), dim3(256), 0, s, vals_rm, k_rm,
                       idx, idx_dtype, n_rows, d_dlr, map, n_buckets, heavy_key, heavy_val, g8_inv_cs, abs_mode);
  return hipGetLastError();
}

static __device__ __forceinline__ uint4 gather16(const void* p) { return *(const uint4*)p; }
static __device__ __forceinline__ uint2 gather8(const void* p) { return *(const uint2*)p; }
#ifndef REFINE_PREFETCH
#define REFINE_PREFETCH 2
#endif
#ifndef REFINE_L2_PREFETCH
#define REFINE_L2_PREFETCH 0
#endif
#ifndef REFINE_WPE
#define REFINE_WPE 8
#endif
#if REFINE_WPE > 0
#define REFINE_ATTR __attribute__((amdgpu_waves_per_eu(REFINE_WPE)))
#else
#define REFINE_ATTR
// ... 1175 lines not shown
  const int64_t g = (int64_t)blockIdx.x * blockDim.x + threadIdx.x;
  if (g >= (int64_t)n_queries * k) return;
  const int q = (int)(g / k), j = (int)(g - (int64_t)q * k);
  const uint64_t key = topk_keys[(int64_t)q * kp + j];
  rows[g] = key ? 0xFFFFFFFFu - (uint32_t)key : 0xFFFFFFFFu;
}
__global__ void __launch_bounds__(256) bound_topm_kernel(const float* __restrict__ bound, int n_rows, int n_queries, int m, uint32_t* __restrict__ rows) {
  __shared__ uint64_t key[256];
  const int q = blockIdx.x, t = threadIdx.x;
  uint64_t mine = 0ull;
  if (t < n_rows) mine = make_key(bound[(int64_t)q * 256 + t], (uint32_t)t);
  key[t] = mine;
  if (t < m) rows[(int64_t)q * m + t] = 0xFFFFFFFFu;
  __syncthreads();
  if (mine) {
    int rank = 0;
    for (int j = 0; j < 256; ++j) rank += key[j] > mine ? 1 : 0;
    if (rank < m) rows[(int64_t)q * m + rank] = 0xFFFFFFFFu - (uint32_t)mine;
  }
}
hipError_t launch_bound_topm(const float* bound, int n_rows, int n_queries, int m, uint32_t* rows, hipStream_t s) {
  if (n_queries <= 0) return hipSuccess;
  hipLaunchKernelGGL(bound_topm_kernel, dim3((unsigned)n_queries), dim3(256), 0, s, bound, n_rows, n_queries, m, rows);
  return hipGetLastError();
}
hipError_t launch_keys_to_rows(const uint64_t* topk_keys, int kp, int n_queries, int k, uint32_t* rows, hipStream_t s) {
  const int64_t total = (int64_t)n_queries * k;
  if (total <= 0) return hipSuccess;
  hipLaunchKernelGGL(keys_to_rows_kernel, dim3((unsigned)((total + 255) / 256)), dim3(256), 0, s, topk_keys, kp, n_queries, k, rows);
  return hipGetLastError();
}
hipError_t launch_emit(const uint64_t* topk_keys, int kp, int n_queries, int k, int64_t row_offset, float* out_scores,
                       int64_t* out_rows, hipStream_t s) {
  const int64_t total = (int64_t)n_queries * k;
  if (total <= 0) return hipSuccess;
  hipLaunchKernelGGL(emit_kernel, dim3((unsigned)((total + 255) / 256)), dim3(256), 0, s, topk_keys, kp, n_queries, k,
                     row_offset, out_scores, out_rows);
  return hipGetLastError();
}

__global__ void max_u32_kernel(const uint32_t* __restrict__ v, int n, uint32_t* out_max, unsigned long long* out_sum) {
  uint32_t m = 0;
  unsigned long long s = 0;
  for (int i = blockIdx.x * blockDim.x + threadIdx.x; i < n; i += gridDim.x * blockDim.x) {
    const uint32_t x = v[i];
    m = x > m ? x : m;
    s += x;
  }
#pragma unroll
  for (int o = 32; o > 0; o >>= 1) {
    const uint32_t om = __shfl_xor(m, o, 64);
    m = om > m ? om : m;
    s += __shfl_xor(s, o, 64);
  }
  if ((threadIdx.x & 63) == 0) {
    atomicMax(out_max, m);
    atomicAdd(out_sum, s);
  }
}
hipError_t launch_max_u32(const uint32_t* v, int n, uint32_t* out_max, unsigned long long* out_sum, hipStream_t s) {
  hipLaunchKernelGGL(max_u32_kernel, dim3(32), dim3(256), 0, s, v, n, out_max, out_sum);
  return hipGetLastError();
}

__global__ void rows_to_local_kernel(const int64_t* __restrict__ rows, int64_t n, int64_t row_offset, int64_t n_rows,
                                     uint32_t* __restrict__ out) {
  const int64_t g = (int64_t)blockIdx.x * blockDim.x + threadIdx.x;
  if (g >= n) return;
  const int64_t r = rows[g] - row_offset;
  out[g] = (rows[g] >= 0 && r >= 0 && r < n_rows) ? (uint32_t)r : 0xFFFFFFFFu;
}
hipError_t launch_rows_to_local(const int64_t* rows, int64_t n, int64_t row_offset, int64_t n_rows, uint32_t* out,
                                hipStream_t s) {
  if (n <= 0) return hipSuccess;
  hipLaunchKernelGGL(rows_to_local_kernel, dim3((unsigned)((n + 255) / 256)), dim3(256), 0, s, rows, n, row_offset,
                     n_rows, out);
  return hipGetLastError();
}

__global__ void mark_overflow_kernel(const uint32_t* __restrict__ cnt, uint32_t cap, int n_queries, uint32_t* fail_flags) {
  const int q = blockIdx.x * blockDim.x + threadIdx.x;
  if (q < n_queries && cnt[q] > cap) fail_flags[q] = 1u;
}
hipError_t launch_mark_overflow(const uint32_t* cnt, uint32_t cap, int n_queries, uint32_t* fail_flags, hipStream_t s) {
  hipLaunchKernelGGL(mark_overflow_kernel, dim3((n_queries + 255) / 256), dim3(256), 0, s, cnt, cap, n_queries, fail_flags);
  return hipGetLastError();
}
__global__ void verify_kernel(const uint64_t* __restrict__ topk_keys, int kp, int k, const float* __restrict__ tau_hat,
                              int n_queries, uint32_t* fail_flags, uint32_t* n_fail) {
  const int q = blockIdx.x * blockDim.x + threadIdx.x;
  if (q >= n_queries) return;
  const uint64_t kth = topk_keys[(int64_t)q * kp + (k - 1)];
  const bool ok = fail_flags[q] == 0u && kth != 0ull && ordered_f32((uint32_t)(kth >> 32)) >= tau_hat[q];
  fail_flags[q] = ok ? 0u : 1u;
  if (!ok) atomicAdd(n_fail, 1u);
}
hipError_t launch_verify(const uint64_t* topk_keys, int kp, int k, const float* tau_hat, int n_queries, uint32_t* fail_flags,
                         uint32_t* n_fail, hipStream_t s) {
  hipLaunchKernelGGL(verify_kernel, dim3((n_queries + 255) / 256), dim3(256), 0, s, topk_keys, kp, k, tau_hat, n_queries,
                     fail_flags, n_fail);
  return hipGetLastError();
}

__global__ void gather_queries_kernel(const float* __restrict__ q32, const int16_t* __restrict__ q_idx, int k_pad,
                                      int d_dlr, const int32_t* __restrict__ ids, int n, float* __restrict__ out32,
                                      int16_t* __restrict__ out_idx) {
  const int i = blockIdx.x;
  if (i >= n) return;
  const int64_t src = ids[i];
  for (int j = threadIdx.x; j < k_pad; j += blockDim.x) out32[(int64_t)i * k_pad + j] = q32[src * k_pad + j];
  for (int j = threadIdx.x; j < d_dlr; j += blockDim.x) out_idx[(int64_t)i * d_dlr + j] = q_idx[src * d_dlr + j];
}
hipError_t launch_gather_queries(const float* q32, const int16_t* q_idx, int k_pad, int d_dlr, const int32_t* ids, int n,
                                 float* out32, int16_t* out_idx, hipStream_t s) {
  if (n <= 0) return hipSuccess;
  hipLaunchKernelGGL(gather_queries_kernel, dim3(n), dim3(256), 0, s, q32, q_idx, k_pad, d_dlr, ids, n, out32, out_idx);
  return hipGetLastError();
}

__global__ void scatter_keys_kernel(const uint64_t* __restrict__ src, uint64_t* __restrict__ dst, int kp,
                                    const int32_t* __restrict__ ids, int n) {
  const int i = blockIdx.x;
  if (i >= n) return;
  for (int j = threadIdx.x; j < kp; j += blockDim.x) dst[(int64_t)ids[i] * kp + j] = src[(int64_t)i * kp + j];
}
hipError_t launch_scatter_keys(const uint64_t* src, uint64_t* dst, int kp, const int32_t* ids, int n, hipStream_t s) {
  if (n <= 0) return hipSuccess;
  hipLaunchKernelGGL(scatter_keys_kernel, dim3(n), dim3(256), 0, s, src, dst, kp, ids, n);
  return hipGetLastError();
}

__global__ void emit_scores_kernel(const uint64_t* __restrict__ topk_keys, int kp, int n_queries, int r, float* __restrict__ out) {
  const int64_t g = (int64_t)blockIdx.x * blockDim.x + threadIdx.x;
  if (g >= (int64_t)n_queries * r) return;
  const int q = (int)(g / r), j = (int)(g - (int64_t)q * r);
  const uint64_t key = topk_keys[(int64_t)q * kp + j];
  out[g] = key ? ordered_f32((uint32_t)(key >> 32)) : -INFINITY;
}
hipError_t launch_emit_scores(const uint64_t* topk_keys, int kp, int n_queries, int r, float* out, hipStream_t s) {
  const int64_t total = (int64_t)n_queries * r;
  if (total <= 0) return hipSuccess;
  hipLaunchKernelGGL(emit_scores_kernel, dim3((unsigned)((total + 255) / 256)), dim3(256), 0, s, topk_keys, kp, n_queries, r, out);
  return hipGetLastError();
}
__global__ void make_thr_kernel(const float* __restrict__ tau, const float* __restrict__ margin, int n_queries, int q_pad,
                                float* __restrict__ thr) {
  const int q = blockIdx.x * blockDim.x + threadIdx.x;
  if (q < q_pad) thr[q] = q < n_queries ? tau[q] - margin[q] : INFINITY;
}
hipError_t launch_make_thr(const float* tau, const float* margin, int n_queries, int q_pad, float* thr, hipStream_t s) {
  hipLaunchKernelGGL(make_thr_kernel, dim3((q_pad + 255) / 256), dim3(256), 0, s, tau, margin, n_queries, q_pad, thr);
  return hipGetLastError();
}
__global__ void raise_thr_kernel(float* __restrict__ thr_hat, const float* __restrict__ thr_run, int n_queries) {
  const int q = blockIdx.x * blockDim.x + threadIdx.x;
  if (q < n_queries) thr_hat[q] = fmaxf(thr_hat[q], thr_run[q]);
}
hipError_t launch_raise_thr(float* thr_hat, const float* thr_run, int n_queries, hipStream_t s) {
  hipLaunchKernelGGL(raise_thr_kernel, dim3((n_queries + 255) / 256), dim3(256), 0, s, thr_hat, thr_run, n_queries);
  return hipGetLastError();
}
__global__ void flag_tau_above_kernel(const float* __restrict__ tau_own, const float* __restrict__ tau_ext, int n_queries, uint32_t* __restrict__ fail_flags) {
  const int q = blockIdx.x * blockDim.x + threadIdx.x;
  if (q < n_queries && tau_own[q] > tau_ext[q]) fail_flags[q] = 1u;
}
hipError_t launch_flag_tau_above(const float* tau_own, const float* tau_ext, int n_queries, uint32_t* fail_flags, hipStream_t s) {
  hipLaunchKernelGGL(flag_tau_above_kernel, dim3((n_queries + 255) / 256), dim3(256), 0, s, tau_own, tau_ext, n_queries, fail_flags);
  return hipGetLastError();
}
__global__ void raise_thr_rank_kernel(float* __restrict__ thr_hat, float* __restrict__ tau_hat, const uint64_t* __restrict__ topk_keys, int kp, int r,
                                      const float* __restrict__ margin, int n_queries) {
  const int q = blockIdx.x * blockDim.x + threadIdx.x;
  if (q >= n_queries) return;
  const uint64_t key = topk_keys[(int64_t)q * kp + (r - 1)];
  if (key == 0ull) return;
  const float t = ordered_f32((uint32_t)(key >> 32));
  if (!(t > tau_hat[q])) return;
  tau_hat[q] = t;
  thr_hat[q] = fmaxf(thr_hat[q], t - margin[q]);
}
hipError_t launch_raise_thr_rank(float* thr_hat, float* tau_hat, const uint64_t* topk_keys, int kp, int r, const float* margin, int n_queries, hipStream_t s) {
  hipLaunchKernelGGL(raise_thr_rank_kernel, dim3((n_queries + 255) / 256), dim3(256), 0, s, thr_hat, tau_hat, topk_keys, kp, r, margin, n_queries);
  return hipGetLastError();
}
__global__ void count_ge_kernel(const uint64_t* __restrict__ topk_keys, int kp, int k, const float* __restrict__ tau,
                                const uint32_t* __restrict__ fail_flags, int n_queries, int32_t* __restrict__ out) {
  const int q = blockIdx.x;
  if (q >= n_queries) return;
  __shared__ int cnt;
  if (threadIdx.x == 0) cnt = 0;
  __syncthreads();
  const float t = tau ? tau[q] : -INFINITY;
  int c = 0;
  for (int j = threadIdx.x; j < k; j += blockDim.x) {
    const uint64_t key = topk_keys[(int64_t)q * kp + j];
    if (key && ordered_f32((uint32_t)(key >> 32)) >= t) ++c;
  }
  atomicAdd(&cnt, c);
  __syncthreads();
  if (threadIdx.x == 0) out[q] = (fail_flags && fail_flags[q]) ? -1 : cnt;
}
hipError_t launch_count_ge(const uint64_t* topk_keys, int kp, int k, const float* tau, const uint32_t* fail_flags, int n_queries,
                           int32_t* out, hipStream_t s) {
  if (n_queries <= 0) return hipSuccess;
  hipLaunchKernelGGL(count_ge_kernel, dim3((unsigned)n_queries), dim3(256), 0, s, topk_keys, kp, k, tau, fail_flags, n_queries, out);
  return hipGetLastError();
}

__global__ void __launch_bounds__(1024) merge_topk_kernel(int n_in, int n_pad, const float* __restrict__ in_scores,
                                                          const int64_t* __restrict__ in_rows, int k_out,
                                                          float* __restrict__ out_scores, int64_t* __restrict__ out_rows) {
  extern __shared__ __attribute__((aligned(16))) char smem[];
  uint32_t* sk = (uint32_t*)smem;
  uint32_t* pos = sk + n_pad;
  const int q = blockIdx.x, tid = threadIdx.x;
  const float* s = in_scores + (int64_t)q * n_in;
  const int64_t* r = in_rows + (int64_t)q * n_in;
  for (int j = tid; j < n_pad; j += 1024) {
    const bool ok = j < n_in && r[j] >= 0;
    sk[j] = ok ? f32_ordered(s[j]) : 0u;
    pos[j] = ok ? (uint32_t)j : 0xFFFFFFFFu;
  }
  __syncthreads();
  auto before = [&](uint32_t ka, uint32_t pa, uint32_t kb, uint32_t pb) -> bool {
    if (pa == 0xFFFFFFFFu) return false;
    if (pb == 0xFFFFFFFFu) return true;
    if (ka != kb) return ka > kb;
    return r[pa] < r[pb];
  };
  for (int size = 2; size <= n_pad; size <<= 1)
    for (int stride = size >> 1; stride > 0; stride >>= 1) {
      for (int t = tid; t < (n_pad >> 1); t += 1024) {
        const int p0 = 2 * t - (t & (stride - 1)), p1 = p0 + stride;
        const uint32_t ka = sk[p0], pa = pos[p0], kb = sk[p1], pb = pos[p1];
        const bool desc = (p0 & size) == 0;
        const bool swap = desc ? before(kb, pb, ka, pa) : before(ka, pa, kb, pb);
        if (swap) { sk[p0] = kb; pos[p0] = pb; sk[p1] = ka; pos[p1] = pa; }
      }
      __syncthreads();
    }
  for (int j = tid; j < k_out; j += 1024) {
    const uint32_t pj = (j < n_pad) ? pos[j] : 0xFFFFFFFFu;
    out_scores[(int64_t)q * k_out + j] = (pj != 0xFFFFFFFFu) ? s[pj] : -INFINITY;
    out_rows[(int64_t)q * k_out + j] = (pj != 0xFFFFFFFFu) ? r[pj] : -1;
  }
}
hipError_t launch_merge_topk(int n_queries, int n_in, const float* in_scores, const int64_t* in_rows, int k_out,
                             float* out_scores, int64_t* out_rows, hipStream_t s) {
  if (n_queries <= 0) return hipSuccess;
  int n_pad = 2;
  while (n_pad < n_in) n_pad <<= 1;
  const int bytes = n_pad * 8;
  if (bytes > 160 * 1024) return hipErrorInvalidValue;
  static int attr_bytes[64] = {};
  if (hipError_t e = ensure_lds_attr((const void*)merge_topk_kernel, bytes, attr_bytes); e != hipSuccess) return e;
  hipLaunchKernelGGL(merge_topk_kernel, dim3((unsigned)n_queries), dim3(1024), bytes, s, n_in, n_pad, in_scores, in_rows,
                     k_out, out_scores, out_rows);
  return hipGetLastError();
}

template <int NL>
__global__ void __launch_bounds__(1024) merge_lists_kernel(int n_lists, int L, int n_queries, const float* __restrict__ in_scores,
                                                          const int64_t* __restrict__ in_rows, int k_out,
                                                          float* __restrict__ out_scores, int64_t* __restrict__ out_rows,
                                                          int64_t stride_s, int64_t stride_r) {
  extern __shared__ __attribute__((aligned(16))) char smem[];
  const int n_tot = n_lists * L;
  int64_t* rw = (int64_t*)smem;
  int64_t* orow = rw + (in_rows ? n_tot : 0);
  uint32_t* sk = (uint32_t*)(orow + (in_rows ? k_out : 0));
  float* osc = (float*)(sk + n_tot);
  const int q = blockIdx.x, tid = threadIdx.x, nthr = blockDim.x;
  for (int j = tid; j < k_out; j += nthr) {
    osc[j] = -INFINITY;
    if (in_rows) orow[j] = -1;
  }
  for (int l0 = 0; l0 < n_lists; l0 += 8)
    for (int j = tid; j < L; j += nthr) {
      float sc[8];
      int64_t rr[8];
      const int64_t in_list = (int64_t)q * L + j;
#pragma unroll
      for (int u = 0; u < 8; ++u) {
        sc[u] = 0.f; rr[u] = 0;
        if (l0 + u < n_lists) {
          sc[u] = in_scores[(int64_t)(l0 + u) * stride_s + in_list];
          if (in_rows) rr[u] = in_rows[(int64_t)(l0 + u) * stride_r + in_list];
        }
      }
#pragma unroll
      for (int u = 0; u < 8; ++u)
        if (l0 + u < n_lists) {
          const int e = (l0 + u) * L + j;
          uint32_t key = f32_ordered(sc[u]);
          if (in_rows) {
            if (rr[u] < 0) key = 0u;
            rw[e] = rr[u] < 0 ? INT64_MAX : rr[u];
          }
          sk[e] = key;
        }
    }
  __syncthreads();
  __shared__ int act[64];
  __shared__ uint32_t t_min;
  if (tid == 0) t_min = 0xFFFFFFFFu;
  __syncthreads();
  const int P = (k_out + n_lists - 1) / n_lists;
  if (tid < n_lists) atomicMin(&t_min, P <= L ? sk[tid * L + P - 1] : 0u);
  __syncthreads();
  if (tid < n_lists) {
    const uint32_t t = t_min;
    int lo = 0, hi = L;
    while (lo < hi) {
      const int mid = (lo + hi) >> 1;
      if (sk[tid * L + mid] >= t) lo = mid + 1; else hi = mid;
    }
    act[tid] = lo;
  }
  __syncthreads();
  int n_act = 0;
  for (int m = 0; m < n_lists; ++m) n_act += act[m];
  const int run = (n_act + nthr - 1) / nthr;
  const int f0 = tid * run, f1 = min(n_act, f0 + run);
  if (f0 < f1) {
    int l = 0, base = 0;
    while (f0 >= base + act[l]) { base += act[l]; ++l; }
    int j = f0 - base;
    bool fresh = true;
    int pos[NL];
    for (int f = f0; f < f1; ++f, ++j) {
      while (j >= act[l]) { ++l; j = 0; fresh = true; }
      const int e = l * L + j;
// ... 73 lines not shown
```

dhr_amd/csrc/search_core.hip:

```cpp
#include "dhr_state.h"

template <typename T>
static hipError_t re_malloc(T*& p, size_t bytes, int64_t& total) {
  if (p) hipFree(p);
  p = nullptr;
  total += (int64_t)bytes;
  return hipMalloc((void**)&p, bytes ? bytes : 16);
}

int ensure_ws(dhr_index* ix, Workspace& w, int n_queries, int k, int64_t keys_ld_min, int64_t cap_mult, bool use_refine, bool queries_only) {
  const int q_pad = (int)round_up(n_queries, TILE_ROWS);
  if (queries_only && w.q_alloc >= q_pad && w.kt == ix->kt && w.q32 != nullptr) { w.q_pad = q_pad; return DHR_OK; }
  int kp = 1;
  while (kp < k) kp <<= 1;
  if (kp < 64) kp = 64;
  const bool refine = (ix->heavy_key != nullptr || ix->resid8 != nullptr) && use_refine;
  int64_t cap = 0, cap_r = 0, keys_ld = 0, cap_deep = 0, arena = 0;
  auto plan_depths = [&](int q_for_cap) {
    int64_t base_cap = refine ? 262144 : 65536;
    const int64_t by_rows = ix->gated_i8 ? std::min<int64_t>(std::max<int64_t>(ix->n_rows / 8, 32768), 262144)
                                         : std::max<int64_t>(ix->n_rows / 128, refine ? 32768 : 16384);
    while (base_cap > by_rows && base_cap > 4096) base_cap >>= 1;
    while (base_cap > 4096 && (int64_t)q_for_cap * base_cap * 16 > ((int64_t)32 << 30)) base_cap >>= 1;
    if (ix->cand_cap > 0) base_cap = ix->cand_cap;
    cap = std::min<int64_t>(base_cap * cap_mult, (int64_t)1 << 22);
    cap_deep = cap;
    const int64_t stride = ix->list_stride > 0 ? ix->list_stride : 32768;
    arena = 0;
    const int variant = ix->gemm_variant ? ix->gemm_variant : g_gemm_variant;
    const bool kernel_writes_tier = ix->gated_i8 || variant != 4;
    if (refine && cap_mult == 1 && ix->cand_cap <= 0 && cap > stride && kernel_writes_tier) {
      cap = stride;
      arena = std::max<int64_t>((int64_t)4 << 20, std::min<int64_t>((int64_t)q_for_cap * 8192, (int64_t)128 << 20));
      arena = std::max(arena, 2 * (cap_deep - cap));
    }
    cap_r = refine ? std::min<int64_t>(cap_deep, std::max<int64_t>(32768, 4 * (int64_t)kp) * cap_mult) : cap;
    keys_ld = std::max<int64_t>(cap_r, keys_ld_min);
  };
  if (w.q_alloc >= q_pad && w.kt == ix->kt) {
    plan_depths(w.q_alloc);
    if (w.kp == kp && w.cap == cap && w.cap_deep == cap_deep && w.arena == arena && w.cap_r == cap_r && w.keys_ld >= keys_ld) { w.q_pad = q_pad; return DHR_OK; }
  }
  plan_depths(q_pad);
  free_ws(w);
  int64_t tot = 0;
  HIP_TRY(re_malloc(w.q_tiles, (size_t)q_pad * ix->kt * 2, tot));
  HIP_TRY(re_malloc(w.q32, (size_t)q_pad * ix->k_rm * 4, tot));
  HIP_TRY(re_malloc(w.q_idx, (size_t)q_pad * std::max(ix->d_dlr, 8) * 2, tot));
  HIP_TRY(re_malloc(w.q16, (size_t)q_pad * ix->k_rm * 2, tot));
  HIP_TRY(re_malloc(w.q_idx8, (size_t)q_pad * std::max(ix->d_dlr, 8), tot));
  HIP_TRY(re_malloc(w.q_inexact, 16, tot));
  HIP_TRY(re_malloc(w.margin, (size_t)q_pad * 4, tot));
  HIP_TRY(re_malloc(w.i8_mul, (size_t)q_pad * 4, tot));
  if (ix->gated_i8) {
    HIP_TRY(re_malloc(w.g8_q8, (size_t)q_pad * ix->d_dlr, tot));
    HIP_TRY(re_malloc(w.g8_shift, (size_t)q_pad * 4, tot));
    HIP_TRY(re_malloc(w.g8_unit, (size_t)q_pad * 4, tot));
  }
  HIP_TRY(re_malloc(w.tau, (size_t)q_pad * 4, tot));
  HIP_TRY(re_malloc(w.thr, (size_t)q_pad * 4, tot));
  HIP_TRY(re_malloc(w.cnt, (size_t)q_pad * 4, tot));
  HIP_TRY(re_malloc(w.cand, (size_t)q_pad * cap * 8, tot));
  const bool alias = refine && keys_ld == cap_r;
  if (!alias) HIP_TRY(re_malloc(w.rs_keys, (size_t)q_pad * keys_ld * 8, tot));
  HIP_TRY(re_malloc(w.topk_keys, (size_t)q_pad * kp * 8, tot));
  HIP_TRY(re_malloc(w.d_max, 16, tot));
  HIP_TRY(re_malloc(w.tau_hat, (size_t)q_pad * 4, tot));
  HIP_TRY(re_malloc(w.fail_flags, (size_t)q_pad * 4, tot));
  HIP_TRY(re_malloc(w.thr_hat, (size_t)q_pad * 4, tot));
  HIP_TRY(re_malloc(w.blk_off, (size_t)2 * (q_pad + 1) * 4, tot));
  HIP_TRY(re_malloc(w.boot_rows, (size_t)q_pad * BOOT_M * 4, tot));
  HIP_TRY(re_malloc(w.boot_bound, (size_t)q_pad * TILE_ROWS * 4, tot));
  if (ix->resid8) HIP_TRY(re_malloc(w.thr_raise, (size_t)q_pad * 4, tot));
  if (arena > 0) {
    HIP_TRY(re_malloc(w.ovf, (size_t)arena * 8, tot));
    HIP_TRY(re_malloc(w.ovf_off, (size_t)q_pad * 4, tot));
    HIP_TRY(re_malloc(w.ovf_cap, (size_t)q_pad * 4, tot));
    HIP_TRY(re_malloc(w.cnt_plan, (size_t)q_pad * 4, tot));
    HIP_TRY(re_malloc(w.tier_dev, 2 * sizeof(ListTier), tot));
    { const ListTier t0{w.ovf, w.ovf_off, w.ovf_cap}; HIP_TRY(hipMemcpy(w.tier_dev, &t0, sizeof t0, hipMemcpyHostToDevice)); }
    HIP_TRY(hipMemset(w.cnt_plan, 0, (size_t)q_pad * 4));
    HIP_TRY(hipMemset(w.ovf_off, 0, (size_t)q_pad * 4));
    HIP_TRY(hipMemset(w.ovf_cap, 0, (size_t)q_pad * 4));
  }
  if (refine) {
    HIP_TRY(re_malloc(w.q_pack, (size_t)q_pad * std::max(ix->d_dlr, 8) * 4, tot));
    HIP_TRY(re_malloc(w.cand_r, (size_t)q_pad * cap_r * 8, tot));
    HIP_TRY(re_malloc(w.cnt_r, (size_t)q_pad * 4, tot));
    if (alias) { w.rs_keys = (uint64_t*)w.cand_r; w.keys_alias = true; }
  }
  HIP_TRY(hipHostMalloc(&w.h_pinned, 16, hipHostMallocDefault));
  HIP_TRY(hipHostMalloc((void**)&w.h_pinned2, 32, hipHostMallocDefault));
  HIP_TRY(re_malloc(w.d_max2, 32, tot));
  HIP_TRY(re_malloc(w.d_ref, 16, tot));
  HIP_TRY(hipHostMalloc(&w.h_ref, 16, hipHostMallocDefault));
  HIP_TRY(re_malloc(w.d_stats, 32, tot));
  HIP_TRY(hipHostMalloc(&w.h_stats, 32, hipHostMallocDefault));
  w.q_pad = w.q_alloc = q_pad; w.kp = kp; w.cap = cap; w.cap_deep = cap_deep; w.arena = arena; w.cap_r = cap_r; w.keys_ld = keys_ld; w.kt = ix->kt; w.d_dlr = ix->d_dlr;
  w.bytes = tot;
  return DHR_OK;
}

int check_queries(const dhr_index* ix, const dhr_query_batch* qb) {
  if (!ix || !qb) return set_error(DHR_ERR_INVALID, "null argument");
  if (qb->n_queries <= 0) return set_error(DHR_ERR_INVALID, "n_queries must be > 0");
  if ((int64_t)DOC_GROUP * ((qb->n_queries + TILE_ROWS - 1) / TILE_ROWS) > 65535)
    return set_error(DHR_ERR_UNSUPPORTED, "more than 4 194 048 queries in one call: split the batch (the Python mirror hands over 8 192 at a time)");
  if (!qb->value || qb->ld_value < ix->k - ix->dlr_pad) return set_error(DHR_ERR_INVALID, "bad query value pointer / ld_value");
  if (qb->value_dtype != DHR_VAL_F16 && qb->value_dtype != DHR_VAL_F32) return set_error(DHR_ERR_INVALID, "bad value_dtype");
  const bool has_idx = qb->index != nullptr && qb->index_dtype != DHR_IDX_NONE;
  if (has_idx && ix->d_dlr == 0)
    return set_error(DHR_ERR_INVALID, "the query batch has an index array but the corpus index was built without one");
  if (has_idx && (qb->index_dtype < DHR_IDX_U8 || qb->index_dtype > DHR_IDX_I16)) return set_error(DHR_ERR_INVALID, "bad index_dtype");
  if (has_idx && qb->ld_index < ix->d_dlr - ix->dlr_pad) return set_error(DHR_ERR_INVALID, "bad query ld_index");
  if (qb->mem_kind != DHR_MEM_HOST && qb->mem_kind != DHR_MEM_DEVICE) return set_error(DHR_ERR_INVALID, "bad mem_kind");
  return DHR_OK;
}

int grow(void*& p, size_t& have, size_t need, int64_t& total) {
  if (have >= need) return DHR_OK;
  if (p) hipFree(p);
  p = nullptr;
  HIP_TRY(hipMalloc(&p, need));
  total += (int64_t)(need - have);
  have = need;
  return DHR_OK;
}

int prep_queries(dhr_index* ix, Workspace& w, const dhr_query_batch* qb, hipStream_t s) {
  const void* v = qb->value;
  const void* qi = qb->index;
  int64_t ldv = qb->ld_value, ldi = qb->ld_index;
  const int es = qb->value_dtype == DHR_VAL_F32 ? 4 : 2;
  if (ix->dlr_pad > 0 && qb->mem_kind != MEM_DEVICE_PADDED) {
    const hipMemcpyKind kind = qb->mem_kind == DHR_MEM_HOST ? hipMemcpyHostToDevice : hipMemcpyDeviceToDevice;
    const int d_in = ix->d_dlr - ix->dlr_pad;
    int rc = grow(w.q_stage, w.q_stage_bytes, (size_t)qb->n_queries * ix->k * es, w.bytes);
    if (rc) return rc;
    HIP_TRY(hipMemsetAsync(w.q_stage, 0, (size_t)qb->n_queries * ix->k * es, s));
    HIP_TRY(hipMemcpy2DAsync(w.q_stage, (size_t)ix->k * es, qb->value, (size_t)qb->ld_value * es, (size_t)d_in * es, (size_t)qb->n_queries, kind, s));
    if (ix->d_cls > 0)
      HIP_TRY(hipMemcpy2DAsync((char*)w.q_stage + (size_t)ix->d_dlr * es, (size_t)ix->k * es, (const char*)qb->value + (size_t)d_in * es,
                               (size_t)qb->ld_value * es, (size_t)ix->d_cls * es, (size_t)qb->n_queries, kind, s));
    v = w.q_stage; ldv = ix->k;
    if (qb->index && qb->index_dtype != DHR_IDX_NONE) {
      const int ies = idx_esize(qb->index_dtype);
      rc = grow(w.qi_stage, w.qi_stage_bytes, (size_t)qb->n_queries * ix->d_dlr * ies, w.bytes);
      if (rc) return rc;
      HIP_TRY(hipMemsetAsync(w.qi_stage, 0, (size_t)qb->n_queries * ix->d_dlr * ies, s));
      HIP_TRY(hipMemcpy2DAsync(w.qi_stage, (size_t)ix->d_dlr * ies, qb->index, (size_t)qb->ld_index * ies, (size_t)d_in * ies,
                               (size_t)qb->n_queries, kind, s));
      qi = w.qi_stage; ldi = ix->d_dlr;
    }
  } else if (qb->mem_kind == DHR_MEM_HOST) {
    int rc = grow(w.q_stage, w.q_stage_bytes, (size_t)qb->n_queries * ix->k * es, w.bytes);
    if (rc) return rc;
    HIP_TRY(hipMemcpy2DAsync(w.q_stage, (size_t)ix->k * es, qb->value, (size_t)qb->ld_value * es, (size_t)ix->k * es,
                             (size_t)qb->n_queries, hipMemcpyHostToDevice, s));
    v = w.q_stage; ldv = ix->k;
    if (ix->d_dlr > 0 && qb->index && qb->index_dtype != DHR_IDX_NONE) {
      const int ies = idx_esize(qb->index_dtype);
      rc = grow(w.qi_stage, w.qi_stage_bytes, (size_t)qb->n_queries * ix->d_dlr * ies, w.bytes);
      if (rc) return rc;
      HIP_TRY(hipMemcpy2DAsync(w.qi_stage, (size_t)ix->d_dlr * ies, qb->index, (size_t)qb->ld_index * ies,
                               (size_t)ix->d_dlr * ies, (size_t)qb->n_queries, hipMemcpyHostToDevice, s));
      qi = w.qi_stage; ldi = ix->d_dlr;
    }
  }
  w.ts_q = sparse_query_stages(ix->ts, ix->d_dlr > 0 && qb->index, ix->gated_i8);
  G8Prep g8{};
  if (ix->gated_i8) { g8.inv_cs = ix->g8_inv_cs; g8.w = ix->g8_w; g8.s_ref = ix->g8_sref; g8.max_shift = ix->g8_max_shift; g8.q8 = w.g8_q8; g8.shift = w.g8_shift; g8.unit = w.g8_unit; }
  if (ix->resid8) { g8.thr_raise = w.thr_raise; g8.resid_ec2 = ix->resid_ec2; }
  HIP_TRY(hipMemsetAsync(w.q_inexact, 0, 8, s));
  HIP_TRY(launch_query_prep(v, qb->value_dtype == DHR_VAL_F32, ldv, (ix->d_dlr > 0 && qb->index) ? qi : nullptr, qb->index_dtype, ldi,
                            qb->n_queries, w.q_pad, ix->d_dlr, ix->d_cls, ix->k_rm, ix->n_buckets, ix->kt, ix->bucket_map,
                            ix->abs_mode, ix->dmax, w.q_tiles, w.q32,
                            w.q_idx, w.margin, w.tau, w.thr, ix->ts, ix->td, w.q_pack, w.q16, w.q_idx8, w.q_inexact, ix->idx_dtype,
                            ix->dense_i8 ? ix->i8_scale : 0.f, ix->i8_ec, ix->i8_nc, w.i8_mul, ix->i8_col_scale, g8, s));
  return DHR_OK;
}

static inline bool uses_refine(const dhr_index* ix, bool gate) { return (ix->heavy_key != nullptr && (gate || ix->gated_i8)) || ix->resid8 != nullptr; }
RescoreArgs base_rescore_args(const dhr_index* ix, const Workspace& w, int n_queries, bool gate) {
  RescoreArgs r{};
  r.vals_rm = ix->vals_rm; r.c_idx = ix->c_idx; r.c_idx_dtype = ix->idx_dtype;
  r.q32 = w.q32; r.q_idx = w.q_idx; r.d_dlr = ix->d_dlr; r.k_rm = ix->k_rm;
  r.q16 = w.q16; r.q_idx8 = w.q_idx8; r.q_inexact = w.q_inexact;
  r.n_rows = ix->n_rows; r.n_queries = n_queries; r.gate = gate ? 1 : 0;
  return r;
}
static GemmArgs base_gemm_args(const dhr_index* ix, const Workspace& w, int Q) {
  GemmArgs g{};
  g.a_tiles = ix->tiles; g.b_tiles = w.q_tiles; g.ksteps = ix->ksteps; g.k_split = ix->d_dlr / TILE_K; g.ts = ix->ts; g.td = ix->td; g.ts_q = w.ts_q; g.variant = ix->gemm_variant;
  g.i8_mul = (ix->dense_i8 || ix->gated_i8) ? w.i8_mul : nullptr; g.g8_shift = ix->gated_i8 ? w.g8_shift : nullptr; g.g8_rsum = ix->g8_rsum;
  g.n_tiles = ix->n_tiles; g.n_qtiles = w.q_pad / TILE_ROWS; g.n_rows = ix->n_rows; g.cap = (uint32_t)w.cap; g.n_queries = Q;
  return g;
}
static RefineArgs base_refine_args(const dhr_index* ix, const Workspace& w, int Q, bool gate, const float* thr) {
  RefineArgs f{};
  f.cap = (uint32_t)w.cap; f.heavy_key = ix->heavy_key; f.heavy_val = ix->heavy_val;
  f.q_pack = w.q_pack; f.d_dlr = ix->d_dlr; f.thr = thr; f.out = w.cand_r; f.out_cnt = w.cnt_r; f.out_cap = (uint32_t)w.cap_r;
  f.n_queries = Q;
  if (ix->gated_i8) { f.g8_q8 = w.g8_q8; f.g8_inv_cs = ix->g8_inv_cs; f.g8_unit = w.g8_unit; f.abs_mode = ix->abs_mode ? 1 : 0; f.ungated = gate ? 0 : 1; }
  if (ix->resid8) { f.resid8 = ix->resid8; f.resid_ld = ix->resid_ld; f.q32 = w.q32; f.q32_ld = ix->k_rm; f.col_scale = ix->i8_col_scale; f.d_cls = ix->d_cls; f.thr_raise = w.thr_raise; }
  return f;
}

struct Search {
  dhr_index* ix; Workspace& w; Timer& tm; dhr_search_stats& st; hipStream_t s;
  Stage stage; int depth, k; const float* tau_ext;
  int Q = 0;
  bool gate = false;
  bool after_mid = false;
  bool async_ctl = false;
  SearchPlan p;
  SelectArgs sel{};
  double rate = 0.0, rate_r = 0.0;
  bool whole() const { return stage == Stage::Whole; }
  bool fresh() const { return whole() || stage == Stage::Begin || stage == Stage::Pre; }
};

static void count_gemm(const Search& c, int64_t tiles) {
  const double rows = (double)tiles * TILE_ROWS;
  c.st.phases++;
  c.st.gemm_rows += (int64_t)rows;
  c.st.gemm_flops += 2.0 * (double)c.w.q_pad * rows * (double)c.ix->kt;
  c.st.gemm_flops_alg += 2.0 * (double)c.Q * rows * (double)c.ix->k;
}

static int gemm_phase(Search& c, int64_t lo, int64_t hi, int period, bool enqueue_only, uint32_t* maxc, unsigned long long* sumc) {
  dhr_index* ix = c.ix; Workspace& w = c.w; hipStream_t s = c.s;
  GemmArgs g = base_gemm_args(ix, w, c.Q);
  if (enqueue_only && w.arena > 0) g.tier = w.tier_dev;
  g.seq_lo = lo; g.seq_hi = hi; g.map_mode = 1; g.period = period; g.head = c.p.head;
  g.thr = w.thr; g.cand = w.cand; g.cnt = w.cnt;
  HIP_TRY(hipMemsetAsync(w.cnt, 0, (size_t)w.q_pad * 4, s));
  if (!enqueue_only) HIP_TRY(hipMemsetAsync(w.d_max, 0, 16, s));
  c.tm.begin(T_GEMM); HIP_TRY(launch_gemm_filter(g, s)); c.tm.end();
  ix->last_gemm_kernel = g_last_gemm_kernel;
  if (!enqueue_only) {
    HIP_TRY(launch_max_u32(w.cnt, c.Q, w.d_max, (unsigned long long*)(w.d_max + 2), s));
    HIP_TRY(hipMemcpyAsync(w.h_pinned, w.d_max, 16, hipMemcpyDeviceToHost, s));
    HIP_TRY(hipStreamSynchronize(s));
    *maxc = ((uint32_t*)w.h_pinned)[0];
    memcpy(sumc, (uint32_t*)w.h_pinned + 2, 8);
  }
  count_gemm(c, hi - lo);
  return DHR_OK;
}
static int rescore_and_select(Search& c, const uint2* cand, const uint32_t* cnt, uint32_t list_cap, uint32_t max_count, uint32_t flat_blocks, hipStream_t s) {
  Workspace& w = c.w;
  RescoreArgs r = base_rescore_args(c.ix, w, c.Q, c.gate);
  r.cand = cand; r.cnt = cnt; r.cap = list_cap; r.max_count = max_count;
  r.out_keys = w.rs_keys; r.ld_keys = w.keys_ld;
  r.blk_off = w.blk_off + w.q_pad + 1; r.flat_blocks = flat_blocks;
  c.tm.begin_on(T_RESCORE, s); HIP_TRY(launch_rescore(r, s)); c.tm.end_on(s);
  c.sel.cnt = cnt; c.sel.count_all = 0; c.sel.cap = list_cap;
  c.tm.begin_on(T_SELECT, s); HIP_TRY(launch_select(c.sel, s)); c.tm.end_on(s);
  return DHR_OK;
}
static int rescore_select_async(Search& c, const uint2* cand, const uint32_t* cnt, const float* thr, hipStream_t s, uint32_t* d_fullest_bound = nullptr,
                                uint32_t* d_fullest = nullptr, const uint2* ovf = nullptr) {
  dhr_index* ix = c.ix; Workspace& w = c.w; Timer& tm = c.tm; const int Q = c.Q;
  uint32_t list_cap = (uint32_t)w.cap;
  const bool refine = uses_refine(ix, c.gate);
  if (!refine) ovf = nullptr;
  const uint32_t* ovf_cap = ovf ? w.ovf_cap : nullptr;
  HIP_TRY(launch_lists_ready(cnt, (uint32_t)w.cap, Q, refine ? (uint32_t)REFINE_PER_WG : (uint32_t)RESCORE_CANDS_PER_WG, refine ? w.blk_off : w.blk_off + w.q_pad + 1,
                             d_fullest_bound, refine ? nullptr : d_fullest, w.d_stats + 0, refine ? nullptr : w.d_stats + 1, w.fail_flags,
                             refine ? w.cnt_r : nullptr, refine ? (int)w.q_pad : 0, s, ovf_cap));
  if (refine) {
    RefineArgs f = base_refine_args(ix, w, Q, c.gate, thr);
    f.ovf = ovf; f.ovf_off = ovf ? w.ovf_off : nullptr; f.ovf_cap = ovf_cap;
    f.cand = cand; f.cnt = cnt; f.max_count = 1;
    f.blk_off = w.blk_off; f.flat_blocks = FLAT_GRID_ASYNC;
    tm.begin_on(T_REFINE, s); HIP_TRY(launch_refine(f, s)); tm.end_on(s);
    list_cap = (uint32_t)w.cap_r;
    cand = w.cand_r; cnt = w.cnt_r;
    HIP_TRY(launch_lists_ready(cnt, list_cap, Q, (uint32_t)RESCORE_CANDS_PER_WG, w.blk_off + w.q_pad + 1, d_fullest, nullptr, w.d_stats + 1,
                               nullptr, w.fail_flags, nullptr, 0, s));
  }
  return rescore_and_select(c, cand, cnt, list_cap, 1, FLAT_GRID_ASYNC, s);
}
static int rescore_select(Search& c, const uint2* cand, const uint32_t* cnt, const float* thr, uint32_t maxc, hipStream_t s, int64_t bound_sum,
                          uint32_t* fail_flags) {
  dhr_index* ix = c.ix; Workspace& w = c.w; Timer& tm = c.tm; const int Q = c.Q;
  uint32_t maxr = std::min<uint32_t>(maxc, (uint32_t)w.cap);
  if (maxr == 0) return DHR_OK;
  int64_t exact = bound_sum;
  uint32_t list_cap = (uint32_t)w.cap;
  if (uses_refine(ix, c.gate)) {
    RefineArgs f = base_refine_args(ix, w, Q, c.gate, thr);
    f.cand = cand; f.cnt = cnt; f.max_count = maxr;
    HIP_TRY(launch_block_offsets(cnt, (uint32_t)w.cap, Q, REFINE_PER_WG, w.blk_off, s));
    f.blk_off = w.blk_off; f.flat_blocks = (uint32_t)std::min<int64_t>(bound_sum / REFINE_PER_WG + Q, (int64_t)0x7fffffff);
    HIP_TRY(hipMemsetAsync(w.cnt_r, 0, (size_t)w.q_pad * 4, s));
    HIP_TRY(hipMemsetAsync(w.d_ref, 0, 16, s));
    tm.begin_on(T_REFINE, s); HIP_TRY(launch_refine(f, s)); tm.end_on(s);
    HIP_TRY(launch_max_u32(w.cnt_r, Q, w.d_ref, (unsigned long long*)(w.d_ref + 2), s));
    HIP_TRY(hipMemcpyAsync(w.h_ref, w.d_ref, 16, hipMemcpyDeviceToHost, s));
    HIP_TRY(hipStreamSynchronize(s));
    w.last_maxr = ((uint32_t*)w.h_ref)[0];
    maxr = std::min<uint32_t>(((uint32_t*)w.h_ref)[0], (uint32_t)w.cap_r);
    if (((uint32_t*)w.h_ref)[0] > (uint32_t)w.cap_r) {
      if (fail_flags) HIP_TRY(launch_mark_overflow(w.cnt_r, (uint32_t)w.cap_r, Q, fail_flags, s));
      else return 1;
    }
    list_cap = (uint32_t)w.cap_r;
    unsigned long long sum;
    memcpy(&sum, (uint32_t*)w.h_ref + 2, 8);
    exact = (int64_t)sum;
    cand = w.cand_r; cnt = w.cnt_r;
  }
  c.st.candidates_exact += exact;
  if (getenv("DHR_DEBUG_PLAN"))
    fprintf(stderr, "[dhr]   lists: bound %.0f per query (fullest %u) -> exact %.0f per query (fullest %u)\n", (double)bound_sum / Q, maxc, (double)exact / Q, maxr);
  if (maxr == 0) return DHR_OK;
  HIP_TRY(launch_block_offsets(cnt, list_cap, Q, RESCORE_CANDS_PER_WG, w.blk_off + w.q_pad + 1, s));
  return rescore_and_select(c, cand, cnt, list_cap, maxr, (uint32_t)std::min<int64_t>(exact / RESCORE_CANDS_PER_WG + Q, (int64_t)0x7fffffff), s);
}

struct StreamOpts {
  bool async_ctl = false;
  double *last_rate = nullptr, *last_rate_r = nullptr;
  int64_t* last_rows = nullptr;
  int rank_target = 0;
  int64_t rank_rows = 0;
  int64_t pos0 = 0;
  int64_t prev_rows0 = 0;
  int growth16 = 0;
};
static int stream_phases(Search& c, int64_t n_seq, int period, int64_t first_chunk, int64_t seen_rows, const StreamOpts& o = {}) {
  dhr_index* ix = c.ix; Workspace& w = c.w; dhr_search_stats& st = c.st; const int Q = c.Q;
  const int growth16 = o.growth16 > 0 ? o.growth16 : ix->max_growth16;
  int64_t pos = o.pos0;
  int64_t prev_rows = o.prev_rows0;
  int64_t chunk = std::max<int64_t>(DOC_GROUP, first_chunk);
  while (pos < n_seq) {
    chunk = std::min(chunk, round_up(n_seq - pos, DOC_GROUP));
    const int64_t hi = std::min(pos + chunk, n_seq);
    const int64_t chunk_rows = (hi - pos) * TILE_ROWS;
    if (o.rank_target > 0) {
      c.sel.k = plan::adaptive_rank(o.rank_target, (double)(seen_rows + chunk_rows) / (double)std::max<int64_t>(o.rank_rows, 1));
      c.sel.monotone = 1;
    }
    if (o.async_ctl) {
      if (w.arena > 0)
        HIP_TRY(launch_plan_overflow(prev_rows > 0 ? w.cnt : nullptr, prev_rows > 0 ? (double)chunk_rows / (double)prev_rows : 0.0, (uint32_t)w.cap,
                                     (uint32_t)(w.cap_deep - w.cap), (uint32_t)w.arena, Q, w.ovf_off, w.ovf_cap, c.s));
      int rc = gemm_phase(c, pos, hi, period, true, nullptr, nullptr);
      if (rc) return rc;
      if ((rc = rescore_select_async(c, w.cand, w.cnt, w.thr, c.s, w.d_max2, w.d_max2 + 4, w.arena > 0 ? w.ovf : nullptr)) != DHR_OK) return rc;
      prev_rows = chunk_rows;
      if (o.last_rows) *o.last_rows = chunk_rows;
      seen_rows += chunk_rows;
      pos = hi;
      chunk = std::max<int64_t>(DOC_GROUP, round_up(seen_rows * growth16 / 16 / TILE_ROWS, DOC_GROUP));
      continue;
    }
    uint32_t maxc; unsigned long long sumc;
    int rc = gemm_phase(c, pos, hi, period, false, &maxc, &sumc);
    if (rc) return rc;
    if (getenv("DHR_DEBUG_PLAN")) fprintf(stderr, "[dhr] stream phase: tiles [%lld, %lld) of %lld (period %d)\n", (long long)pos, (long long)hi, (long long)n_seq, period);
    if (maxc > w.cap && chunk > DOC_GROUP) {
      st.overflow_retries++;
      chunk = std::max<int64_t>(DOC_GROUP, round_up(chunk / 2, DOC_GROUP));
      continue;
    }
    if (maxc > w.cap) return set_error(DHR_ERR_INTERNAL, "bound list overflow at the minimum chunk size");
    st.candidates_bound += (int64_t)sumc;
    if (o.last_rate) *o.last_rate = (double)maxc / (double)chunk_rows;
    rc = rescore_select(c, w.cand, w.cnt, w.thr, maxc, c.s, (int64_t)sumc, nullptr);
    if (rc == 1 && chunk > DOC_GROUP) {
      st.overflow_retries++;
      chunk = std::max<int64_t>(DOC_GROUP, round_up(chunk / 2, DOC_GROUP));
      continue;
    }
    if (rc != DHR_OK) return rc < 0 ? rc : set_error(DHR_ERR_INTERNAL, "survivor list overflow at the minimum chunk size");
    if (o.last_rate_r) *o.last_rate_r = (uses_refine(ix, c.gate) && maxc > 0) ? (double)w.last_maxr / (double)chunk_rows : 0.0;
    pos = hi;
    seen_rows += chunk_rows;
    const double target = (double)w.cap / 2.0;
    double next_rows = (maxc == 0) ? (double)chunk_rows * 4.0 : (double)chunk_rows * target / (double)maxc;
    next_rows = std::min(next_rows, (double)seen_rows * ix->max_growth16 / 16.0);
    chunk = std::max<int64_t>(DOC_GROUP, (int64_t)(next_rows / (DOC_GROUP * TILE_ROWS)) * DOC_GROUP);
  }
  return DHR_OK;
}

static int prepare_and_phase0(Search& c, const dhr_query_batch* qb) {
  dhr_index* ix = c.ix; Workspace& w = c.w; Timer& tm = c.tm; hipStream_t s = c.s; const SearchPlan& p = c.p; const int Q = c.Q;
  int rc;
  tm.begin(T_PREP);
  if ((rc = prep_queries(ix, w, qb, s)) != DHR_OK) return rc;
  HIP_TRY(hipMemsetAsync(w.topk_keys, 0, (size_t)w.q_pad * w.kp * 8, s));
  HIP_TRY(hipMemsetAsync(w.fail_flags, 0, (size_t)w.q_pad * 4, s));
  HIP_TRY(hipMemsetAsync(w.d_stats, 0, 32, s));
  tm.end();
  RescoreArgs r = base_rescore_args(ix, w, Q, c.gate);
  r.out_keys = w.rs_keys; r.ld_keys = w.keys_ld;
  c.sel.cnt = nullptr;
  if (p.bootstrap) {
    const int m = p.boot_m;
    {
      GemmArgs g = base_gemm_args(ix, w, Q);
      g.seq_lo = 0; g.seq_hi = 1; g.map_mode = 0; g.period = 1; g.head = 0;
      g.thr = w.thr; g.cand = w.cand; g.cnt = w.cnt;
      g.dump = w.boot_bound; g.dump_ld = TILE_ROWS; g.dump_row0 = 0;
      tm.begin(T_GEMM); HIP_TRY(launch_gemm_filter(g, s)); tm.end();
      c.st.phases++;
    }
    HIP_TRY(launch_bound_topm(w.boot_bound, (int)std::min<int64_t>(TILE_ROWS, ix->n_rows), Q, m, w.boot_rows, s));
    r.rows32 = w.boot_rows; r.ld_rows = m; r.count_all = (uint32_t)m; r.max_count = (uint32_t)m;
    tm.begin(T_RESCORE); HIP_TRY(launch_rescore(r, s)); tm.end();
    c.sel.count_all = (uint32_t)m;
    c.sel.k = std::min(p.boot_r0, m); c.sel.monotone = 1;
    tm.begin(T_SELECT); HIP_TRY(launch_select(c.sel, s)); tm.end();
    HIP_TRY(hipMemsetAsync(w.topk_keys, 0, (size_t)w.q_pad * w.kp * 8, s));
    c.st.candidates_exact += (int64_t)m * Q;
    return DHR_OK;
  }
  r.row0 = 0; r.count_all = (uint32_t)p.first_valid; r.max_count = (uint32_t)p.first_valid;
  tm.begin(T_RESCORE); HIP_TRY(launch_rescore(r, s)); tm.end();
  c.sel.count_all = (uint32_t)p.first_valid;
  if (p.sampled) { c.sel.k = p.head_rank; c.sel.monotone = 1; }
  tm.begin(T_SELECT); HIP_TRY(launch_select(c.sel, s)); tm.end();
  c.st.candidates_exact += (int64_t)p.first_valid * Q;
  return DHR_OK;
}

static int sampled_run(Search& c) {
  dhr_index* ix = c.ix; Workspace& w = c.w; hipStream_t s = c.s; const SearchPlan& p = c.p; const int Q = c.Q;
  int64_t last_rows = 0;
  int64_t seen0 = p.first_valid, n_hi = p.n_sample, chunk0 = std::max<int64_t>(p.head, DOC_GROUP);
  StreamOpts o;
  o.async_ctl = c.async_ctl; o.last_rate = &c.rate; o.last_rate_r = &c.rate_r; o.last_rows = &last_rows;
  o.rank_target = p.r_eff; o.rank_rows = p.sample_rows;
  const bool pre = c.stage == Stage::Pre;
  if (pre) {
    n_hi = p.pre_positions;
    if (n_hi <= 0) return set_error(DHR_ERR_INVALID, "the sample of this index is too small for a pre step");
    constexpr int pre_growth = 64;
    o.growth16 = std::max(ix->max_growth16, pre_growth);
  }
  if (c.stage == Stage::BeginRest) {
    o.pos0 = ix->pend.pre_pos; seen0 = ix->pend.pre_seen;
    o.prev_rows0 = ix->pend.pre_last_rows;
    HIP_TRY(launch_raise_thr(w.tau, c.tau_ext, Q, s));
    HIP_TRY(launch_make_thr(w.tau, w.margin, Q, w.q_pad, w.thr, s));
    chunk0 = round_up(p.n_sample - o.pos0, DOC_GROUP);
  }
  int rc = stream_phases(c, n_hi, p.S, chunk0, seen0, o);
  if (rc != DHR_OK) return rc;
  if (pre) {
    staged_open(ix, StagedState::AfterPre, c.gate, Q, c.k);
    ix->pend.pre_pos = n_hi; ix->pend.pre_seen = p.first_valid + n_hi * TILE_ROWS; ix->pend.pre_last_rows = last_rows;
    return DHR_OK;
  }
  HIP_TRY(hipMemcpyAsync(w.tau_hat, w.tau, (size_t)w.q_pad * 4, hipMemcpyDeviceToDevice, s));
  if (c.async_ctl && w.arena > 0) {
    HIP_TRY(hipMemcpyAsync(w.cnt_plan, w.cnt, (size_t)w.q_pad * 4, hipMemcpyDeviceToDevice, s));
    w.plan_rows = last_rows;
  } else w.plan_rows = 0;
  if (c.async_ctl && ix->async_ctl >= 2 && c.whole() && last_rows > 0) {
    HIP_TRY(hipMemcpyAsync(w.h_pinned2, w.d_max2, 32, hipMemcpyDeviceToHost, s));
    HIP_TRY(hipStreamSynchronize(s));
    const uint32_t* hp = (const uint32_t*)w.h_pinned2;
    c.rate = (double)hp[0] / (double)last_rows;
    c.rate_r = uses_refine(ix, c.gate) ? (double)hp[4] / (double)last_rows : 0.0;
  }
  if (!c.whole()) {
    staged_open(ix, StagedState::AfterBegin, c.gate, Q, c.k);
    ix->pend.rate = c.rate; ix->pend.rate_r = c.rate_r;
  }
  return DHR_OK;
}

static int adopt_thresholds(Search& c) {
  Workspace& w = c.w; hipStream_t s = c.s; const int Q = c.Q;
  c.rate = c.ix->pend.rate; c.rate_r = c.ix->pend.rate_r;
  if (c.after_mid) {
    HIP_TRY(launch_raise_thr(w.tau_hat, c.tau_ext, Q, s));
    HIP_TRY(launch_make_thr(w.tau_hat, w.margin, Q, w.q_pad, w.thr, s));
    HIP_TRY(launch_raise_thr(w.thr_hat, w.thr, Q, s));
  } else {
    HIP_TRY(hipMemcpyAsync(w.tau_hat, c.tau_ext, (size_t)Q * 4, hipMemcpyDeviceToDevice, s));
    HIP_TRY(launch_flag_tau_above(w.tau, w.tau_hat, Q, w.fail_flags, s));
    HIP_TRY(launch_make_thr(w.tau_hat, w.margin, Q, w.q_pad, w.thr, s));
  }
  return DHR_OK;
}
struct MainPass {
  hipStream_t sg = nullptr, sb = nullptr;
  bool extrapolate = false, scatter = false, two_tier = false;
  int M = 0, c_lo = 0, c_hi = 0;
  std::vector<int64_t> bound;
  std::vector<hipEvent_t> ev_gemm, ev_done;
  Events evs;
};
static int main_streams(Search& c, MainPass& mp) {
  dhr_index* ix = c.ix;
  const int aux_cus = ix->aux_cus >= 0 ? ix->aux_cus : (ix->d_dlr == 0 ? 128 : 0);
  if (ix->aux_cus_made != aux_cus || ix->gemm_excl_made != ix->gemm_exclusive) {
    if (ix->s_aux) { hipStreamDestroy(ix->s_aux); ix->s_aux = nullptr; }
    if (ix->s_gemm) { hipStreamDestroy(ix->s_gemm); ix->s_gemm = nullptr; }
    if (aux_cus > 0) {
      uint32_t m_aux[8], m_gemm[8];
      for (int i = 0; i < 8; ++i) {
        const int lo = i * 32;
        const int n = std::max(0, std::min(32, aux_cus - lo));
        m_aux[i] = n >= 32 ? 0xffffffffu : ((1u << n) - 1u);
        m_gemm[i] = ix->gemm_exclusive ? ~m_aux[i] : 0xffffffffu;
      }
      if (hipExtStreamCreateWithCUMask(&ix->s_aux, 8, m_aux) != hipSuccess ||
          hipExtStreamCreateWithCUMask(&ix->s_gemm, 8, m_gemm) != hipSuccess) {
        (void)hipGetLastError();
        if (ix->s_aux) { hipStreamDestroy(ix->s_aux); ix->s_aux = nullptr; }
        if (ix->s_gemm) { hipStreamDestroy(ix->s_gemm); ix->s_gemm = nullptr; }
      }
    }
    if (!ix->s_aux) {
      HIP_TRY(hipStreamCreateWithFlags(&ix->s_aux, hipStreamNonBlocking));
    }
    ix->aux_cus_made = aux_cus; ix->gemm_excl_made = ix->gemm_exclusive;
  }
  mp.sg = ix->s_gemm ? ix->s_gemm : c.s;
  const bool overlap = ix->overlap_aux < 0 ? true : ix->overlap_aux != 0;
  mp.sb = overlap ? ix->s_aux : mp.sg;
  return DHR_OK;
}
static int main_chunk_count(const Search& c, const MainPass& mp, bool mid_proto) {
  const dhr_index* ix = c.ix; const Workspace& w = c.w; const int64_t n_main = c.p.n_main; const double rate = c.rate, rate_r = c.rate_r;
  const bool plan_read = ix->async_ctl >= 2 && c.whole();
  const int64_t plan_cap = mp.two_tier ? w.cap_deep : w.cap;
  const int64_t need = std::max((int64_t)std::ceil(1.5 * rate * (double)n_main * TILE_ROWS / (double)plan_cap),
                                (int64_t)std::ceil(1.5 * rate_r * (double)n_main * TILE_ROWS / (double)w.cap_r));
  int64_t by_size = std::min<int64_t>(8, std::max<int64_t>(2, (n_main + 4199) / 4200));
  const int64_t no_overflow = (3 * n_main * TILE_ROWS + 2 * std::min(plan_cap, w.cap_r) - 1) / (2 * std::min(plan_cap, w.cap_r));
  if (no_overflow <= 12) by_size = std::max(by_size, no_overflow);
  {
    const double k_eff = (double)c.k / (double)std::max(1, c.whole() ? 1 : ix->sample_share);
    const int64_t by_hot = (int64_t)std::ceil(300.0 * k_eff / (double)plan_cap);
    const int64_t by_hot_r = (int64_t)std::ceil(65.0 * k_eff / (double)w.cap_r);
    by_size = std::max(by_size, std::min<int64_t>(24, std::max(by_hot, by_hot_r)));
  }
  if (mp.extrapolate) by_size = std::max(by_size, std::min<int64_t>(12, (n_main + 2799) / 2800));
  const int64_t want = c.async_ctl ? std::max<int64_t>(std::max<int64_t>(ix->main_chunks, by_size), plan_read ? need : 0) : std::max<int64_t>(ix->main_chunks, need);
  const int M_plain = (int)std::max<int64_t>(1, std::min<int64_t>(std::min<int64_t>(want, 64), n_main / (16 * DOC_GROUP)));
  if (getenv("DHR_DEBUG_PLAN"))
    fprintf(stderr, "[dhr] main pass: rate %.3e (x n_main rows = %.0f of cap %lld), rate_r %.3e (%.0f of cap_r %lld), need %lld, chunks %d, n_main %lld tiles\n", rate,
            rate * (double)n_main * TILE_ROWS, (long long)w.cap, rate_r, rate_r * (double)n_main * TILE_ROWS, (long long)w.cap_r, (long long)need, M_plain + (mid_proto ? 1 : 0), (long long)n_main);
  return M_plain;
}
static int main_gemm(Search& c, MainPass& mp, int i) {
  dhr_index* ix = c.ix; Workspace& w = c.w; hipStream_t sg = mp.sg;
  uint32_t* cnt = (i & 1) ? w.cnt2 : w.cnt;
  if (i >= mp.c_lo + 2) HIP_TRY(hipStreamWaitEvent(sg, mp.ev_done[i - 2], 0));
  GemmArgs g = base_gemm_args(ix, w, c.Q);
  g.seq_lo = mp.bound[i]; g.seq_hi = mp.bound[i + 1]; g.map_mode = mp.scatter ? 3 : 2; g.period = c.p.S; g.head = c.p.head;
  g.perm_mul = mp.scatter ? c.p.perm_mul : 1; g.perm_n = c.p.n_main;
  g.thr = w.thr_hat; g.cand = (i & 1) ? w.cand2 : w.cand; g.cnt = cnt;
  if (mp.two_tier) g.tier = w.tier_dev + (i & 1);
  HIP_TRY(hipMemsetAsync(cnt, 0, (size_t)w.q_pad * 4, sg));
  if (!c.async_ctl) HIP_TRY(hipMemsetAsync(w.d_max2 + 4 * (i & 1), 0, 16, sg));
  c.tm.begin_on(T_GEMM, sg); HIP_TRY(launch_gemm_filter(g, sg)); c.tm.end_on(sg);
  ix->last_gemm_kernel = g_last_gemm_kernel;
  if (!c.async_ctl) {
    HIP_TRY(launch_max_u32(cnt, c.Q, w.d_max2 + 4 * (i & 1), (unsigned long long*)(w.d_max2 + 4 * (i & 1) + 2), sg));
    HIP_TRY(hipMemcpyAsync(w.h_pinned2 + 16 * (i & 1), w.d_max2 + 4 * (i & 1), 16, hipMemcpyDeviceToHost, sg));
  }
  HIP_TRY(hipEventRecord(mp.ev_gemm[i], sg));
  count_gemm(c, mp.bound[i + 1] - mp.bound[i]);
  return DHR_OK;
}
static int main_chunks(Search& c, MainPass& mp) {
  dhr_index* ix = c.ix; Workspace& w = c.w; const SearchPlan& p = c.p; const int Q = c.Q;
  hipStream_t sb = mp.sb;
  int rc;
  if ((rc = main_gemm(c, mp, mp.c_lo)) != DHR_OK) return rc;
  for (int i = mp.c_lo; i < mp.c_hi; ++i) {
    if (i + 1 < mp.c_hi && (rc = main_gemm(c, mp, i + 1)) != DHR_OK) return rc;
    uint2* cand = (i & 1) ? w.cand2 : w.cand;
    uint32_t* cnt = (i & 1) ? w.cnt2 : w.cnt;
    if (c.async_ctl) {
      if (sb != mp.sg) HIP_TRY(hipStreamWaitEvent(sb, mp.ev_gemm[i], 0));
      if ((rc = rescore_select_async(c, cand, cnt, w.thr_hat, sb, nullptr, nullptr, mp.two_tier ? ((i & 1) ? w.ovf2 : w.ovf) : nullptr)) != DHR_OK) return rc;
    } else {
      HIP_TRY(hipEventSynchronize(mp.ev_gemm[i]));
      const uint32_t maxc = *(const uint32_t*)(w.h_pinned2 + 16 * (i & 1));
      unsigned long long sumc;
      memcpy(&sumc, w.h_pinned2 + 16 * (i & 1) + 8, 8);
      c.st.candidates_bound += (int64_t)sumc;
      if (getenv("DHR_DEBUG_PLAN")) fprintf(stderr, "[dhr] main chunk %d: tiles [%lld, %lld)\n", i, (long long)mp.bound[i], (long long)mp.bound[i + 1]);
      HIP_TRY(launch_mark_overflow(cnt, (uint32_t)w.cap, Q, w.fail_flags, sb));
      if ((rc = rescore_select(c, cand, cnt, w.thr_hat, maxc, sb, (int64_t)sumc, w.fail_flags)) != DHR_OK) return rc;
    }
    if (ix->progressive_thr) HIP_TRY(launch_raise_thr(w.thr_hat, c.sel.thr, Q, sb));
    if (mp.extrapolate && i + 1 < mp.M) {
      const int r = plan::extrapolated_rank(c.k, (double)(p.head + p.n_sample + mp.bound[i + 1]) / (double)ix->n_tiles);
      if (r < c.k) HIP_TRY(launch_raise_thr_rank(w.thr_hat, w.tau_hat, w.topk_keys, w.kp, r, w.margin, Q, sb));
    }
    HIP_TRY(hipEventRecord(mp.ev_done[i], sb));
  }
  return DHR_OK;
}
static int main_pass(Search& c) {
  dhr_index* ix = c.ix; Workspace& w = c.w; hipStream_t s = c.s; const SearchPlan& p = c.p;
  MainPass mp;
  c.sel.k = c.k; c.sel.kps = w.kp; c.sel.monotone = 0;
  mp.extrapolate = ix->progressive_thr >= 2 && c.whole() && c.depth == 0 && p.n_main >= 64 && c.k >= 16;
  const bool mid = c.stage == Stage::Mid;
  const bool mid_proto = mid || c.after_mid;
  mp.scatter = mp.extrapolate || (mid_proto && p.n_main >= 64);
  if (!c.after_mid) HIP_TRY(hipMemcpyAsync(w.thr_hat, w.thr, (size_t)w.q_pad * 4, hipMemcpyDeviceToDevice, s));
  if (!w.cand2) {
    int64_t tot = 0;
    HIP_TRY(re_malloc(w.cand2, (size_t)w.q_alloc * w.cap * 8, tot));
    HIP_TRY(re_malloc(w.cnt2, (size_t)w.q_alloc * 4, tot));
    if (w.arena > 0) {
      HIP_TRY(re_malloc(w.ovf2, (size_t)w.arena * 8, tot));
      const ListTier t1{w.ovf2, w.ovf_off, w.ovf_cap};
      HIP_TRY(hipMemcpy(w.tier_dev + 1, &t1, sizeof t1, hipMemcpyHostToDevice));
    }
    w.bytes += tot;
  }
  int rc;
  if ((rc = main_streams(c, mp)) != DHR_OK) return rc;
  hipStream_t sg = mp.sg, sb = mp.sb;
  mp.two_tier = c.async_ctl && w.arena > 0;
  mp.bound = plan::main_chunk_bounds(p.n_main, main_chunk_count(c, mp, mid_proto), mid_proto ? p.mid_offset : 0);
  if (mid_proto) mp.bound.insert(mp.bound.begin(), 0);
  mp.M = (int)mp.bound.size() - 1;
  mp.c_lo = c.after_mid ? 1 : 0; mp.c_hi = mid ? 1 : mp.M;
  if (mp.two_tier) {
    int64_t big = 0;
    for (int i = 0; i < mp.M; ++i) big = std::max(big, mp.bound[i + 1] - mp.bound[i]);
    HIP_TRY(launch_plan_overflow(w.plan_rows > 0 ? w.cnt_plan : nullptr, w.plan_rows > 0 ? (double)(big * TILE_ROWS) / (double)w.plan_rows : 0.0, (uint32_t)w.cap,
                                 (uint32_t)(w.cap_deep - w.cap), (uint32_t)w.arena, c.Q, w.ovf_off, w.ovf_cap, s));
  }
  if (sg != s || sb != s) {
    hipEvent_t ev_enter = nullptr;
    HIP_TRY(mp.evs.add(&ev_enter, hipEventDisableTiming));
    HIP_TRY(hipEventRecord(ev_enter, s));
    if (sg != s) HIP_TRY(hipStreamWaitEvent(sg, ev_enter, 0));
    if (sb != s) HIP_TRY(hipStreamWaitEvent(sb, ev_enter, 0));
  }
  mp.ev_gemm.resize(mp.M); mp.ev_done.resize(mp.M);
  for (int i = 0; i < mp.M; ++i) {
    HIP_TRY(mp.evs.add(&mp.ev_gemm[i], hipEventDisableTiming));
    HIP_TRY(mp.evs.add(&mp.ev_done[i], hipEventDisableTiming));
  }
  if ((rc = main_chunks(c, mp)) != DHR_OK) return rc;
  HIP_TRY(hipStreamWaitEvent(s, mp.ev_done[mp.c_hi - 1], 0));
  return DHR_OK;
}

static void debug_report_failures(const Search& c) {
  const Workspace& w = c.w; const int Q = c.Q;
  std::vector<uint32_t> ff(Q); std::vector<float> th(Q);
  (void)hipStreamSynchronize(c.s);
  (void)hipMemcpy(ff.data(), w.fail_flags, (size_t)Q * 4, hipMemcpyDeviceToHost);
  (void)hipMemcpy(th.data(), w.tau_hat, (size_t)Q * 4, hipMemcpyDeviceToHost);
  for (int q = 0; q < Q; ++q) {
    uint64_t key = 0;
    (void)hipMemcpy(&key, w.topk_keys + (size_t)q * w.kp + (c.k - 1), 8, hipMemcpyDeviceToHost);
    const float kth = key ? ordered_f32((uint32_t)(key >> 32)) : -INFINITY;
    if (ff[q] || !(kth >= th[q])) fprintf(stderr, "[dhr] depth %d query %d will be redone: list overflow %u, k-th best %.6f, threshold %.6f\n", c.depth, q, ff[q], kth, th[q]);
  }
}
static int verify_and_redo(Search& c) {
  dhr_index* ix = c.ix; Workspace& w = c.w; dhr_search_stats& st = c.st; hipStream_t s = c.s; const int Q = c.Q, k = c.k;
  if (getenv("DHR_DEBUG_FAIL")) debug_report_failures(c);
  HIP_TRY(hipMemsetAsync(w.d_max, 0, 16, s));
  HIP_TRY(launch_max_u32(w.fail_flags, Q, w.d_max + 1, (unsigned long long*)(w.d_max + 2), s));
  HIP_TRY(launch_verify(w.topk_keys, w.kp, k, w.tau_hat, Q, w.fail_flags, w.d_max, s));
  HIP_TRY(hipMemcpyAsync(w.h_pinned, w.d_max, 16, hipMemcpyDeviceToHost, s));
  if (c.async_ctl) HIP_TRY(hipMemcpyAsync(w.h_stats, w.d_stats, 32, hipMemcpyDeviceToHost, s));
  HIP_TRY(hipStreamSynchronize(s));
  if (c.async_ctl) {
    st.candidates_bound += (int64_t)((unsigned long long*)w.h_stats)[0];
    st.candidates_exact += (int64_t)((unsigned long long*)w.h_stats)[1];
  }
  const uint32_t n_fail = ((uint32_t*)w.h_pinned)[0];
  const uint32_t n_overflow = ((uint32_t*)w.h_pinned)[1];
  st.sample_fallback_queries += n_fail;
  if (n_fail == 0) return DHR_OK;

  std::vector<uint32_t> flags(Q);
  HIP_TRY(hipMemcpy(flags.data(), w.fail_flags, (size_t)Q * 4, hipMemcpyDeviceToHost));
  std::vector<int32_t> ids;
  for (int q = 0; q < Q; ++q)
    if (flags[q]) ids.push_back(q);
  int next_depth = c.depth + 1;
  if (c.depth == 0 && (int)n_overflow == 0) next_depth = 2;
  const int nf = (int)ids.size();
  DevMem tmp_mem;
  void*& tmp = tmp_mem.p;
  const size_t b32 = (size_t)nf * ix->k_rm * 4, bidx = (size_t)nf * std::max(ix->d_dlr, 8) * 2, bids = (size_t)nf * 4;
  HIP_TRY(hipMalloc(&tmp, b32 + bidx + bids + 64));
  float* f32 = (float*)tmp;
  int16_t* fidx = (int16_t*)((char*)tmp + b32);
  int32_t* d_ids = (int32_t*)((char*)tmp + b32 + bidx);
  if (hipMemcpyAsync(d_ids, ids.data(), bids, hipMemcpyHostToDevice, s) != hipSuccess) return set_error(DHR_ERR_HIP, "H2D failed");
  if (launch_gather_queries(w.q32, w.q_idx, ix->k_rm, ix->d_dlr, d_ids, nf, f32, fidx, s) != hipSuccess)
    return set_error(DHR_ERR_HIP, "gather_queries launch failed");
  dhr_query_batch sub{};
  sub.n_queries = nf; sub.mem_kind = ix->dlr_pad > 0 ? MEM_DEVICE_PADDED : DHR_MEM_DEVICE; sub.value = f32; sub.value_dtype = DHR_VAL_F32; sub.ld_value = ix->k_rm;
  sub.index = c.gate ? fidx : nullptr; sub.index_dtype = c.gate ? DHR_IDX_I16 : DHR_IDX_NONE; sub.ld_index = ix->d_dlr;
  Workspace& w2 = ix->ws_fb[next_depth - 1];
  int rc;
  if ((rc = search_core(ix, w2, &sub, k, next_depth, c.tm, st, s)) != DHR_OK) return rc;
  if (w2.kp != w.kp) return set_error(DHR_ERR_INTERNAL, "fallback workspace mismatch");
  if (launch_scatter_keys(w2.topk_keys, w.topk_keys, w.kp, d_ids, nf, s) != hipSuccess)
    return set_error(DHR_ERR_HIP, "scatter_keys launch failed");
  if (hipStreamSynchronize(s) != hipSuccess) return set_error(DHR_ERR_HIP, "fallback search failed on the device");
  return DHR_OK;
}

int search_core(dhr_index* ix, Workspace& w, const dhr_query_batch* qb, int k, int depth, Timer& tm, dhr_search_stats& st, hipStream_t s,
                Stage stage, const float* tau_ext) {
  Search c{ix, w, tm, st, s, stage, depth, k, tau_ext};
  const bool fresh = c.fresh();
  c.Q = fresh ? qb->n_queries : ix->pend.Q;
  c.gate = fresh ? (ix->d_dlr > 0 && qb->index != nullptr && qb->index_dtype != DHR_IDX_NONE) : ix->pend.gate;
  c.after_mid = stage == Stage::Finish && ix->pend.state == StagedState::AfterMid;
  c.p = search_plan_of(ix, k, depth, !c.whole());
  const SearchPlan& p = c.p;
  int rc;
  if ((rc = ensure_ws(ix, w, c.Q, k, p.first_valid, depth == 0 ? 1 : 16, c.gate || ix->gated_i8 || ix->resid8 != nullptr)) != DHR_OK) return rc;
  c.async_ctl = depth == 0 && p.S >= 2 && ix->async_ctl != 0 && !getenv("DHR_DEBUG_PLAN");
  SelectArgs& sel = c.sel;
  sel.topk_keys = w.topk_keys; sel.in_keys = w.rs_keys; sel.ld_keys = w.keys_ld; sel.cap = (uint32_t)w.cap;
  sel.k = p.r_eff; sel.kp = w.kp; sel.sort_n = select_sort_n(w.kp);
  sel.k_keep = k;
  sel.kps = 64; while (sel.kps < k) sel.kps <<= 1; sel.margin = w.margin; sel.tau = w.tau; sel.thr = w.thr;
  sel.n_queries = c.Q;

  if (fresh && (rc = prepare_and_phase0(c, qb)) != DHR_OK) return rc;
  if (!fresh && ix->pend.state == StagedState::Complete) return DHR_OK;
  if (!p.sampled) {
    if (p.rest > 0 && (rc = stream_phases(c, p.rest, 1, p.head, p.first_valid)) != DHR_OK) return rc;
    if (fresh && !c.whole()) staged_open(ix, StagedState::Complete, c.gate, c.Q, k);
    return DHR_OK;
  }
  switch (stage) {
    case Stage::Whole:
      if ((rc = sampled_run(c)) != DHR_OK || (rc = main_pass(c)) != DHR_OK) return rc;
      return verify_and_redo(c);
    case Stage::Begin: case Stage::Pre: case Stage::BeginRest:
      return sampled_run(c);
    case Stage::Mid: case Stage::Finish:
      if ((rc = adopt_thresholds(c)) != DHR_OK || (rc = main_pass(c)) != DHR_OK) return rc;
      if (stage == Stage::Mid) staged_set(ix, StagedState::AfterMid);
      return DHR_OK;
  }
  return set_error(DHR_ERR_INTERNAL, "unknown search stage");
}
```

dhr_amd/csrc/search_plan.h:

```cpp
#pragma once
#include <algorithm>
#include <cmath>
#include <cstdint>
#include <vector>
#ifndef DHR_DOC_GROUP
#define DHR_DOC_GROUP 4
#endif
namespace dhr {
namespace plan {
constexpr int TILE_ROWS = 256;
constexpr int DOC_GROUP = DHR_DOC_GROUP;
constexpr int BOOT_M = 64;
inline int64_t round_up(int64_t v, int64_t m) { return (v + m - 1) / m * m; }
inline int share_rank(int r, int shares) {
  if (shares <= 1 || r <= 0) return r;
  const double m = (double)r / shares;
  return std::min(r, (int)std::ceil(m + 5.0 * std::sqrt(m) + 4.0));
}
inline int extrapolated_rank(int k, double f) { return (int)std::ceil((double)k * f + 6.0 * std::sqrt((double)k * f * (1.0 - f)) + 4.0); }
inline int adaptive_rank(int r, double phi) {
  if (!(phi < 1.0)) return r;
  if (phi < 0.0) phi = 0.0;
  return std::max(1, std::min(r, extrapolated_rank(r, phi)));
}
constexpr int PRE_SHARE16 = 2, MID_SHARE16 = 2;
struct PlanInput {
  int64_t n_rows = 0, n_tiles = 0, first_rows = 0;
  int k = 0, sample_period = 0, sample_share = 1;
  int depth = 0;
  bool staged = false;
};
struct SearchPlan {
  int S = 0;
  int r = 0, r_eff = 0;
  bool sampled = false;
  bool bootstrap = false;
  int boot_r0 = 0, boot_m = 0;
  int64_t first = 0, first_valid = 0;
  int head_rank = 0;
  int64_t head = 0, rest = 0, n_sample = 0, n_main = 0;
  int64_t sample_rows = 0;
  int64_t pre_positions = 0; double pre_phi = 0.0; int pre_union = 0, pre_local = 0;
  int64_t mid_offset = 0; double mid_f = 0.0; int mid_union = 0, mid_local = 0;
  int64_t perm_mul = 1;
};
inline SearchPlan make_search_plan(const PlanInput& in) {
  SearchPlan p;
  const int k = in.k;
  p.r = k;
  if (in.depth < 2) {
    for (int S = in.sample_period; S >= 2; S = S >= 8 ? S / 2 : 0) {
      const int rr = share_rank(k, S);
      const int64_t head_guess = round_up(std::max<int64_t>(256, 2 * (int64_t)rr), TILE_ROWS) / TILE_ROWS;
      const int64_t rest_guess = in.n_tiles - head_guess;
      if (!(rr >= k || rest_guess < 32 * (int64_t)S || (rest_guess / S) * TILE_ROWS < 16 * (int64_t)rr)) { p.S = S; p.r = rr; break; }
    }
  }
  p.r_eff = (p.S >= 2 && in.staged) ? share_rank(p.r, in.sample_share) : p.r;
  if (p.S >= 2 && in.first_rows <= 0 && in.n_tiles >= 8) {
    const int64_t rows = ((in.n_tiles + p.S - 1) / p.S) * TILE_ROWS;
    const int r0 = adaptive_rank(p.r_eff, (double)TILE_ROWS / (double)rows);
    if (r0 <= BOOT_M) { p.bootstrap = true; p.boot_r0 = r0; p.boot_m = std::min(BOOT_M, std::max(16, 2 * r0)); }
  }
  int64_t first = 0;
  if (!p.bootstrap)
    first = in.first_rows > 0 ? std::max<int64_t>(in.first_rows, 2 * (int64_t)p.r_eff) : std::max<int64_t>(p.S >= 2 ? 256 : 512, 2 * (int64_t)p.r_eff);
  p.first = std::min(round_up(first, TILE_ROWS), round_up(in.n_rows, TILE_ROWS));
  p.first_valid = std::min(p.first, in.n_rows);
  p.head = p.first / TILE_ROWS;
  p.rest = in.n_tiles - p.head;
  p.head_rank = p.r_eff;
  p.sampled = p.S >= 2 && p.rest > 0;
  if (!p.sampled) return p;
  p.n_sample = (p.rest + p.S - 1) / p.S;
  p.n_main = p.rest - p.n_sample;
  p.sample_rows = p.first_valid + p.n_sample * TILE_ROWS;
  if (!p.bootstrap) p.head_rank = adaptive_rank(p.r_eff, (double)p.first_valid / (double)p.sample_rows);
  if (p.n_sample >= 64) {
    const int64_t a = round_up(std::max<int64_t>(DOC_GROUP, p.n_sample * PRE_SHARE16 / 16), DOC_GROUP);
    if (a < p.n_sample) {
      p.pre_positions = a;
      p.pre_phi = (double)(p.first_valid + a * TILE_ROWS) / (double)p.sample_rows;
      p.pre_union = adaptive_rank(p.r, p.pre_phi);
      p.pre_local = share_rank(p.pre_union, in.sample_share);
    }
  }
  if (p.n_main >= 64) {
    p.mid_offset = std::min<int64_t>(p.n_main, round_up(p.n_main * MID_SHARE16 / 16, DOC_GROUP));
    p.mid_f = (double)(p.head + p.n_sample + p.mid_offset) / (double)in.n_tiles;
    p.mid_union = std::min(k, extrapolated_rank(k, p.mid_f));
    p.mid_local = share_rank(p.mid_union, in.sample_share);
    p.perm_mul = (int64_t)(0.6180339887 * (double)p.n_main) | 1;
    auto gcd = [](int64_t a, int64_t b) { while (b) { const int64_t t = a % b; a = b; b = t; } return a; };
    while (gcd(p.perm_mul, p.n_main) != 1) p.perm_mul += 2;
  }
  return p;
}
inline std::vector<int64_t> main_chunk_bounds(int64_t n_main, int M_plain, int64_t mid_offset) {
  std::vector<int64_t> b((size_t)M_plain + 1, 0);
  b[0] = mid_offset;
  double acc = 0.0, tot = 0.0;
  for (int i = 0; i < M_plain; ++i) tot += 1.0 + 2.0 * (M_plain - 1 - i) / std::max(1, M_plain - 1);
  for (int i = 0; i < M_plain; ++i) {
    acc += 1.0 + 2.0 * (M_plain - 1 - i) / std::max(1, M_plain - 1);
    b[(size_t)i + 1] = std::min<int64_t>(n_main, mid_offset + round_up((int64_t)((n_main - mid_offset) * acc / tot), DOC_GROUP));
  }
  b[(size_t)M_plain] = n_main;
  return b;
}

}
}
```

include/dhr_hip.h:

```cpp
#ifndef DHR_HIP_H
#define DHR_HIP_H

#include <stdint.h>

#ifdef __cplusplus
extern "C" {
#endif

#define DHR_VERSION 105

typedef enum dhr_status {
  DHR_OK = 0,
  DHR_ERR_INVALID = -1,
  DHR_ERR_UNSUPPORTED = -2,
  DHR_ERR_HIP = -3,
  DHR_ERR_INTERNAL = -4,
  DHR_ERR_NOMEM = -5,
  DHR_ERR_PEER = -6
} dhr_status;

typedef enum dhr_idx_dtype { DHR_IDX_NONE = 0, DHR_IDX_U8 = 1, DHR_IDX_I8 = 2, DHR_IDX_I16 = 3 } dhr_idx_dtype;
typedef enum dhr_val_dtype { DHR_VAL_F16 = 0, DHR_VAL_F32 = 1, DHR_VAL_BF16 = 2 } dhr_val_dtype;
typedef enum dhr_mem_kind { DHR_MEM_HOST = 0, DHR_MEM_DEVICE = 1 } dhr_mem_kind;

typedef struct dhr_index dhr_index;

typedef struct dhr_index_desc {
  int32_t device;
  int32_t mem_kind;
  int64_t n_rows;
  int32_t d_dlr;
  int32_t d_cls;
  const void* value;
  int64_t ld_value;
  const void* index;
  int32_t index_dtype;
  int32_t idx_buckets;
  int64_t ld_index;
  int64_t row_offset;
} dhr_index_desc;

typedef struct dhr_query_batch {
  int32_t n_queries;
  int32_t mem_kind;
  const void* value;
  int32_t value_dtype;
  int32_t index_dtype;
  int64_t ld_value;
  const void* index;
  int64_t ld_index;
} dhr_query_batch;

typedef struct dhr_search_stats {
  int64_t n_rows, n_queries, k;
  int32_t phases;
  int32_t overflow_retries;
  int64_t candidates_bound;
  int64_t candidates_exact;
  int64_t gemm_rows;
  int64_t sample_fallback_queries;
  double gemm_ms, refine_ms, rescore_ms, select_ms, prep_ms, total_ms;
  double gemm_flops;
  double gemm_flops_alg;
} dhr_search_stats;

typedef enum dhr_param {
  DHR_PARAM_CAND_CAP = 1,
  DHR_PARAM_FIRST_ROWS = 2,
  DHR_PARAM_PROFILE = 3,
  DHR_PARAM_MAX_GROWTH = 4,
  DHR_PARAM_MAIN_CHUNKS = 7,
  DHR_PARAM_AUX_CUS = 9,
  DHR_PARAM_GEMM_EXCLUSIVE = 10,
  DHR_PARAM_OVERLAP_AUX = 11,
  DHR_PARAM_PROGRESSIVE_THR = 8,
  DHR_PARAM_GEMM_VARIANT = 6,
  DHR_PARAM_ASYNC_CONTROLLER = 13,
  DHR_PARAM_SAMPLE_SHARE = 12,
  DHR_PARAM_LIST_STRIDE = 14,
  DHR_PARAM_SAMPLE_PERIOD = 5
} dhr_param;

typedef enum dhr_option {
  DHR_OPT_DENSE_I8 = 1,
  DHR_OPT_GATED_I8 = 2
} dhr_option;
int dhr_set_option(int32_t option, int64_t value);
typedef enum dhr_info {
  DHR_INFO_DENSE_I8 = 1,
  DHR_INFO_I8_SCALE = 2,
  DHR_INFO_I8_ROW_ERR = 3,
  DHR_INFO_I8_ROW_NORM = 4,
  DHR_INFO_ROW_NORM_MAX = 5,
  DHR_INFO_TILE_BYTES = 6,
  DHR_INFO_GATED_I8 = 7,
  DHR_INFO_GEMM_KERNEL = 8
} dhr_info;
int dhr_index_get_info(const dhr_index* index, int32_t what, double* out);

int dhr_version(void);
void dhr_abi_sizes(int32_t out[4]);
enum { DHR_ABI_INDEX_DESC = 0, DHR_ABI_QUERY_BATCH = 1, DHR_ABI_SEARCH_STATS = 2, DHR_ABI_FILE_INFO = 3, DHR_ABI_HOST_SHARD = 4 };
int32_t dhr_abi_size(int32_t which);
const char* dhr_last_error(void);

int dhr_index_create(const dhr_index_desc* desc, dhr_index** out);
void dhr_index_destroy(dhr_index* index);
int dhr_index_set_param(dhr_index* index, int32_t param, int64_t value);
int64_t dhr_index_device_bytes(const dhr_index* index);

typedef struct dhr_file_info {
  int64_t n_rows, row_offset;
  int32_t d_dlr, d_cls, index_dtype, idx_buckets;
  uint32_t file_version, reserved;
  int64_t payload_bytes;
  int64_t blob_offset, blob_bytes;
} dhr_file_info;
int dhr_index_save(const dhr_index* index, const char* path, const void* blob, int64_t blob_bytes);
int dhr_index_file_info(const char* path, dhr_file_info* out);
int dhr_index_load(const char* path, int32_t device, int64_t row_offset, dhr_index** out);

int dhr_search(dhr_index* index, const dhr_query_batch* queries, int32_t k, float* out_scores,
               int64_t* out_rows, int32_t out_mem_kind, void* stream);

int dhr_search_rerank(dhr_index* index, const dhr_query_batch* stage1, const dhr_query_batch* full, int32_t k1, int32_t k,
                      float* out_scores, int64_t* out_rows, int32_t out_mem_kind, void* stream);

int32_t dhr_search_sample_rank(const dhr_index* index, int32_t k);
int32_t dhr_search_union_rank(const dhr_index* index, int32_t k);
int dhr_search_begin(dhr_index* index, const dhr_query_batch* queries, int32_t k, float* out_sample_scores_dev, void* stream);
int dhr_search_finish(dhr_index* index, const float* tau_hat_dev, float* out_scores, int64_t* out_rows,
                      int32_t* out_count_dev, int32_t out_mem_kind, void* stream);
int32_t dhr_search_mid_ranks(const dhr_index* index, int32_t k, int32_t* out_local, int32_t* out_union);
int dhr_search_mid(dhr_index* index, const float* tau_hat_dev, int32_t r_local, float* out_scores_dev, void* stream);
int32_t dhr_search_pre_ranks(const dhr_index* index, int32_t k, int32_t* out_local, int32_t* out_union);
int dhr_search_pre(dhr_index* index, const dhr_query_batch* queries, int32_t k, int32_t r_local, float* out_scores_dev, void* stream);
int dhr_search_begin_rest(dhr_index* index, const float* tau_dev, float* out_sample_scores_dev, void* stream);

int dhr_score_rows(dhr_index* index, const dhr_query_batch* queries, int32_t m, const int64_t* rows,
                   float* out_scores, int32_t mem_kind, void* stream);

int dhr_merge_topk(int32_t device, int32_t n_queries, int32_t n_in, const float* in_scores,
                   const int64_t* in_rows, int32_t k_out, float* out_scores, int64_t* out_rows, void* stream);
int dhr_merge_topk_host(int32_t n_queries, int32_t n_in, const float* in_scores, const int64_t* in_rows,
                        int32_t k_out, float* out_scores, int64_t* out_rows);

int dhr_merge_topk_lists(int32_t device, int32_t n_queries, int32_t n_lists, int32_t list_len, const float* in_scores,
                         const int64_t* in_rows, int32_t k_out, float* out_scores, int64_t* out_rows, void* stream);
int dhr_merge_topk_lists_host(int32_t n_queries, int32_t n_lists, int32_t list_len, const float* in_scores,
                              const int64_t* in_rows, int32_t k_out, float* out_scores, int64_t* out_rows);
int dhr_densify(int32_t device, int32_t mem_kind, const void* lexical, int32_t value_dtype, int64_t ld, int64_t batch, int32_t vocab,
                int32_t remove_dims, int32_t dims, void* out_value, int32_t out_value_dtype, int64_t ld_value, void* out_index,
                int32_t index_dtype, int64_t ld_index, void* stream);

typedef enum dhr_lexical_mode { DHR_LEX_RAW = 0, DHR_LEX_DENSIFY = 1, DHR_LEX_AGG_FULL = 2, DHR_LEX_AGG_SEMI = 3 } dhr_lexical_mode;
int dhr_lexical_head(int32_t device, int32_t mem_kind, int32_t mode, const void* logits, int32_t value_dtype, int64_t batch, int32_t n_tokens,
                     int32_t vocab, int64_t ld_batch, int64_t ld_token, const float* term_weights, int64_t ld_weights, const float* mask,
                     int64_t ld_mask, int32_t dims, int32_t remove_dims, void* out_value, int32_t out_value_dtype, int64_t ld_value,
                     void* out_index, int32_t index_dtype, int64_t ld_index, const void* cls, int32_t cls_dtype, int64_t ld_cls, int32_t cls_dim,
                     void* workspace, void* stream);
int dhr_aggregate(int32_t device, int32_t mem_kind, const void* lexical, int32_t value_dtype, int64_t ld, int64_t batch, int32_t vocab,
                  int32_t dims, int32_t remove_dims, int32_t full, void* out, int32_t out_dtype, int64_t ld_out, void* stream);

int64_t dhr_lexical_proj_workspace(int64_t batch, int32_t n_tokens, int32_t vocab, int32_t mode);
int dhr_lexical_proj_head(int32_t device, int32_t mem_kind, int32_t mode, const void* hidden, int32_t value_dtype, int64_t batch, int32_t n_tokens,
                          int32_t hidden_dim, int64_t ld_batch, int64_t ld_token, const void* weight, int32_t vocab, int64_t ld_weight,
                          const void* bias, int32_t bias_dtype, const float* term_weights, int64_t ld_weights, const float* mask, int64_t ld_mask,
                          int32_t dims, int32_t remove_dims, void* out_value, int32_t out_value_dtype, int64_t ld_value, void* out_index,
                          int32_t index_dtype, int64_t ld_index, const void* cls, int32_t cls_dtype, int64_t ld_cls, int32_t cls_dim,
                          void* workspace, int64_t workspace_bytes, void* stream);

int64_t dhr_gip_scores_workspace(int64_t n_q, int64_t n_p, int32_t dims, int32_t group);
int dhr_gip_scores(int32_t device, int32_t mem_kind, const void* q_value, int64_t ld_q_value, const void* q_index, int64_t ld_q_index, int64_t n_q,
                   const void* p_value, int64_t ld_p_value, const void* p_index, int64_t ld_p_index, int64_t n_p, int32_t dims, int32_t value_dtype,
                   int32_t index_dtype, int32_t group, float* out, int64_t ld_out, void* workspace, int64_t workspace_bytes, void* stream);
int dhr_gip_scores_backward(int32_t device, int32_t mem_kind, const void* q_value, int64_t ld_q_value, const void* q_index, int64_t ld_q_index,
                            int64_t n_q, const void* p_value, int64_t ld_p_value, const void* p_index, int64_t ld_p_index, int64_t n_p, int32_t dims,
                            int32_t value_dtype, int32_t index_dtype, int32_t group, const float* grad_out, int64_t ld_grad, float* grad_q,
                            int64_t ld_grad_q, float* grad_p, int64_t ld_grad_p, void* stream);
int dhr_densify_backward(int32_t device, int32_t mem_kind, const float* grad_value, int64_t ld_grad_value, const void* index, int32_t index_dtype,
                         int64_t ld_index, int64_t batch, int32_t vocab, int32_t remove_dims, int32_t dims, void* grad_lexical, int32_t grad_dtype,
                         int64_t ld_grad, void* stream);

int64_t dhr_lexical_head_train_workspace(int64_t batch, int32_t n_tokens);
int dhr_lexical_head_train(int32_t device, int32_t mem_kind, const void* logits, int32_t value_dtype, int64_t batch, int32_t n_tokens,
                           int32_t skip_tokens, int32_t vocab, int64_t ld_batch, int64_t ld_token, const float* term_weights, int64_t ld_weights,
                           const float* mask, int64_t ld_mask, float* out_reps, int64_t ld_reps, int16_t* out_tokens, int64_t ld_tokens,
                           void* workspace, void* stream);
int dhr_lexical_head_backward(int32_t device, int32_t mem_kind, const void* logits, int32_t value_dtype, int64_t batch, int32_t n_tokens,
                              int32_t skip_tokens, int32_t vocab, int64_t ld_batch, int64_t ld_token, const float* grad_reps, int64_t ld_grad_reps,
                              const int16_t* tokens, int64_t ld_tokens, void* workspace, void* grad_logits, int64_t ld_grad_batch,
                              int64_t ld_grad_token, float* grad_weights, int64_t ld_grad_weights, void* stream);

int64_t dhr_lexical_proj_train_workspace(int64_t batch, int32_t n_tokens, int32_t vocab, int32_t hidden_dim);
int dhr_lexical_proj_train(int32_t device, int32_t mem_kind, const void* hidden, int32_t value_dtype, int64_t batch, int32_t n_tokens,
                           int32_t skip_tokens, int32_t hidden_dim, int64_t ld_batch, int64_t ld_token, const void* weight, int32_t vocab,
                           int64_t ld_weight, const void* bias, int32_t bias_dtype, const float* term_weights, int64_t ld_weights,
                           const float* mask, int64_t ld_mask, float* out_reps, int64_t ld_reps, int16_t* out_tokens, int64_t ld_tokens,
                           float* out_pwin, int64_t ld_pwin, void* workspace, int64_t workspace_bytes, void* stream);
int dhr_lexical_proj_backward(int32_t device, int32_t mem_kind, const void* hidden, int32_t value_dtype, int64_t batch, int32_t n_tokens,
                              int32_t skip_tokens, int32_t hidden_dim, int64_t ld_batch, int64_t ld_token, const void* weight, int32_t vocab,
                              int64_t ld_weight, const void* bias, int32_t bias_dtype, const float* term_weights, int64_t ld_weights,
                              const float* mask, int64_t ld_mask, const float* grad_reps, int64_t ld_grad_reps, const int16_t* tokens,
                              int64_t ld_tokens, const float* pwin, int64_t ld_pwin, void* workspace, int64_t workspace_bytes, void* grad_hidden,
                              int32_t grad_hidden_dtype, int64_t ld_grad_batch, int64_t ld_grad_token, void* grad_weight,
                              int32_t grad_weight_dtype, int64_t ld_grad_weight, void* grad_bias, int32_t grad_bias_dtype,
                              float* grad_term_weights, int64_t ld_grad_term_weights, void* stream);

int dhr_aggregate_train(int32_t device, int32_t mem_kind, const void* lexical, int32_t value_dtype, int64_t ld, int64_t batch, int32_t vocab,
                        int32_t dims, int32_t remove_dims, int32_t full, void* out, int32_t out_dtype, int64_t ld_out, int16_t* route,
                        int64_t ld_route, void* stream);
int dhr_aggregate_backward(int32_t device, int32_t mem_kind, const void* grad_out, int32_t grad_dtype, int64_t ld_grad_out, const int16_t* route,
                           int64_t ld_route, int64_t batch, int32_t vocab, int32_t dims, int32_t remove_dims, int32_t full, void* grad_lexical,
                           int64_t ld_grad, void* stream);
int dhr_term_weight_head(int32_t device, int32_t mem_kind, const void* input_ids, int32_t id_bytes, int64_t ld_ids, const void* term_weights,
                         int32_t value_dtype, int64_t ld_weights, int64_t batch, int32_t n_tokens, int32_t skip_tokens, int32_t vocab,
                         float* out_reps, int64_t ld_reps, int16_t* out_tokens, int64_t ld_tokens, void* stream);
int dhr_term_weight_head_backward(int32_t device, int32_t mem_kind, const void* input_ids, int32_t id_bytes, int64_t ld_ids, int64_t batch,
                                  int32_t n_tokens, int32_t skip_tokens, int32_t vocab, const float* grad_reps, int64_t ld_grad_reps,
                                  const int16_t* tokens, int64_t ld_tokens, void* grad_weights, int32_t grad_dtype, int64_t ld_grad_weights,
                                  void* stream);

int dhr_maxsim_scores(int32_t device, int32_t mem_kind, const void* q, int64_t ld_q_tok, int64_t ld_q_batch, int64_t A, int64_t Lq, const void* p,
                      int64_t ld_p_tok, int64_t ld_p_batch, int64_t B, int64_t Lp, int32_t D, int32_t value_dtype, int32_t group, float* out,
                      int64_t ld_out, int16_t* arg, void* stream);
int dhr_maxsim_scores_backward(int32_t device, int32_t mem_kind, const void* q, int64_t ld_q_tok, int64_t ld_q_batch, int64_t A, int64_t Lq,
                               const void* p, int64_t ld_p_tok, int64_t ld_p_batch, int64_t B, int64_t Lp, int32_t D, int32_t value_dtype,
                               int32_t group, const int16_t* arg, const float* grad_out, int64_t ld_grad, void* dq, void* dp, int32_t grad_dtype,
                               void* stream);

int64_t dhr_train_loss_workspace(int64_t rows);
int dhr_train_loss(int32_t device, int32_t mem_kind, const void* lexical, int32_t lexical_dtype, int64_t ld_lexical, const void* semantic,
// ... 84 lines not shown
```

Baseline: 61560.

## Ramp main-pass chunk sizes by seen tiles and defer threshold load in int8 GEMM

```diff
diff --git a/dhr_amd/csrc/dhr_internal.h b/dhr_amd/csrc/dhr_internal.h
--- a/dhr_amd/csrc/dhr_internal.h
+++ b/dhr_amd/csrc/dhr_internal.h
@@ -303,7 +303,7 @@
 hipError_t launch_max_u32(const uint32_t* v, int n, uint32_t* out_max, unsigned long long* out_sum, hipStream_t s);
 hipError_t launch_lists_ready(const uint32_t* cnt, uint32_t cap, int n_queries, uint32_t per, uint32_t* offs, uint32_t* out_max, uint32_t* out_max2,
                               unsigned long long* out_sum, unsigned long long* out_sum2, uint32_t* fail_flags, uint32_t* zero, int n_zero,
-                              hipStream_t s, const uint32_t* ovf_cap = nullptr);
+                              hipStream_t s, const uint32_t* ovf_cap = nullptr, unsigned long long* out_sum3 = nullptr);
 hipError_t launch_rows_to_local(const int64_t* rows, int64_t n, int64_t row_offset, int64_t n_rows, uint32_t* out,
                                 hipStream_t s);
 hipError_t launch_mark_overflow(const uint32_t* cnt, uint32_t cap, int n_queries, uint32_t* fail_flags, hipStream_t s);
diff --git a/dhr_amd/csrc/dhr_state.h b/dhr_amd/csrc/dhr_state.h
--- a/dhr_amd/csrc/dhr_state.h
+++ b/dhr_amd/csrc/dhr_state.h
@@ -48,6 +48,7 @@
   }
 };
 static inline int idx_esize(int dt) { return dt == DHR_IDX_I16 ? 2 : 1; }
+constexpr int MAX_MAIN_CHUNKS = 65;
 
 struct Workspace {
   int q_pad = 0, kp = 0;
@@ -97,6 +98,7 @@
   uint32_t* d_max2 = nullptr;
   unsigned long long* d_stats = nullptr;
   void* h_stats = nullptr;
+  unsigned long long* d_chunk_stats = nullptr;
   uint32_t* d_ref = nullptr;
   void* h_ref = nullptr;
   void* q_stage = nullptr;  size_t q_stage_bytes = 0;
@@ -148,6 +150,7 @@
   int sample_share = 1;
   int main_chunks = 2;
   int progressive_thr = 2;
+  int chunk_ramp = 1;
   int n_cu = 256;
   int gemm_variant = 0;
   int last_gemm_kernel = 0;
@@ -171,7 +174,7 @@
 
 inline void free_ws(Workspace& w) {
   hipFree(w.q_tiles); hipFree(w.q32); hipFree(w.q_idx); hipFree(w.q16); hipFree(w.q_idx8); hipFree(w.q_inexact); hipFree(w.margin); hipFree(w.i8_mul); hipFree(w.g8_q8); hipFree(w.g8_shift); hipFree(w.g8_unit); hipFree(w.tau); hipFree(w.thr);
-  hipFree(w.cnt); hipFree(w.cand); if (!w.keys_alias) hipFree(w.rs_keys); hipFree(w.topk_keys); hipFree(w.d_max); hipFree(w.tau_hat); hipFree(w.fail_flags); hipFree(w.thr_hat); hipFree(w.cand2); hipFree(w.cnt2); hipFree(w.q_pack); hipFree(w.cand_r); hipFree(w.cnt_r); hipFree(w.thr_raise); hipFree(w.blk_off); hipFree(w.ovf); hipFree(w.ovf2); hipFree(w.ovf_off); hipFree(w.ovf_cap); hipFree(w.cnt_plan); hipFree(w.tier_dev); hipFree(w.boot_rows); hipFree(w.boot_bound);
+  hipFree(w.cnt); hipFree(w.cand); if (!w.keys_alias) hipFree(w.rs_keys); hipFree(w.topk_keys); hipFree(w.d_max); hipFree(w.tau_hat); hipFree(w.fail_flags); hipFree(w.thr_hat); hipFree(w.d_chunk_stats); hipFree(w.cand2); hipFree(w.cnt2); hipFree(w.q_pack); hipFree(w.cand_r); hipFree(w.cnt_r); hipFree(w.thr_raise); hipFree(w.blk_off); hipFree(w.ovf); hipFree(w.ovf2); hipFree(w.ovf_off); hipFree(w.ovf_cap); hipFree(w.cnt_plan); hipFree(w.tier_dev); hipFree(w.boot_rows); hipFree(w.boot_bound);
   if (w.h_pinned) hipHostFree(w.h_pinned);
   if (w.h_pinned2) hipHostFree(w.h_pinned2);
   hipFree(w.d_max2); hipFree(w.d_ref); hipFree(w.d_stats);
diff --git a/dhr_amd/csrc/gemm_g8.hip b/dhr_amd/csrc/gemm_g8.hip
--- a/dhr_amd/csrc/gemm_g8.hip
+++ b/dhr_amd/csrc/gemm_g8.hip
@@ -162,6 +162,13 @@
   const __amdgpu_buffer_rsrc_t role_rsrc = __builtin_amdgcn_make_buffer_rsrc((void*)(dma_b ? b_src : a_src), (short)0, 0x7fffffff, 0x00020000);
   int dma_soff = 0, dma_n = 0, nx_soff = 0, nx_n = 0;
   uint32_t dma_lds = 0, nx_lds = 0;
+  const bool thr_wave = !DUMP && wave == 2;
+  const __amdgpu_buffer_rsrc_t thr_rsrc = __builtin_amdgcn_make_buffer_rsrc((void*)p.thr, (short)0, 0x7fffffff, 0x00020000);
+  bool dma_thr = false, nx_thr = false;
+  auto thr_piece = [&]() __attribute__((always_inline)) {
+    if (dma_thr)
+      __builtin_amdgcn_raw_ptr_buffer_load_lds(thr_rsrc, LDS_PTR(smem + G8_META + 2048), 16, (int)lane_off, qt * (TILE_ROWS * 4), 0, 16 );
+  };
   auto dma_prepare = [&](int g) __attribute__((always_inline)) {
     const int u = 2 * g + dma_s;
     const bool sp = u < ts;
@@ -170,9 +177,10 @@
     else nx_soff = (sp ? u * S8_STAGE_A : ts * S8_STAGE_A + (u - ts) * SP_DENSE) + half_bytes;
     nx_lds = smem_u + (uint32_t)((u & 3) * G8_SLOT + (dma_b ? G8_QOFF : 0) + half_bytes);
     nx_n = g < npairs ? ((!dma_b && sp) ? 5 : 8) : 0;
+    nx_thr = thr_wave && g == npairs - 1;
     if ((G8_ABL == 4 || G8_ABL == 8) && g >= 2) nx_n = 0;
   };
-  auto dma_commit = [&]() __attribute__((always_inline)) { dma_soff = nx_soff; dma_lds = nx_lds; dma_n = nx_n; };
+  auto dma_commit = [&]() __attribute__((always_inline)) { dma_soff = nx_soff; dma_lds = nx_lds; dma_n = nx_n; dma_thr = nx_thr; };
   auto dma_piece = [&](int j) __attribute__((always_inline)) {
     if (j < dma_n) {
       __attribute__((address_space(3))) void* l = (__attribute__((address_space(3))) void*)(uintptr_t)(dma_lds + (uint32_t)(j >> 2) * 4096u);
@@ -190,6 +198,7 @@
     dma_commit();
 #pragma unroll
     for (int j = 0; j < 8; ++j) dma_piece(j);
+    thr_piece();
   };
 
   floatx16 acc[4][2];
@@ -225,6 +234,7 @@
         g8_smfmac(acc[mi][ni], fc.a[mi], fc.b[ni].v, (uint32_t)fc.pw[mi]);
       }
       if (g8_dma_piece(PH, g) >= 0) dma_piece(g8_dma_piece(PH, g));
+      if (PH == 0 && g == 7) thr_piece();
       __builtin_amdgcn_sched_barrier(0);
     }
   };
@@ -240,13 +250,14 @@
         g8_mfma(acc[mi][ni], fc.a[mi], fc.b[ni].h[0]);
       }
       if (g8_dma_piece(PH, g) >= 0) dma_piece(g8_dma_piece(PH, g));
+      if (PH == 0 && g == 7) thr_piece();
       __builtin_amdgcn_sched_barrier(0);
     }
   };
 
-  if (wave < 4 && (ts > 0 || wave == 1 || wave == 2)) {
+  if (wave < 4 && wave != 2 && (ts > 0 || wave == 1)) {
     const char* src = wave == 0 ? (const char*)(p.g8_rsum + dt * TILE_ROWS) : wave == 1 ? (const char*)(p.i8_mul + qt * TILE_ROWS)
-                    : wave == 2 ? (const char*)(p.thr + qt * TILE_ROWS) : (const char*)(p.g8_shift + qt * TILE_ROWS);
+                    : (const char*)(p.g8_shift + qt * TILE_ROWS);
     __builtin_amdgcn_global_load_lds(GLOBAL_PTR(src + lane_off), LDS_PTR(smem + G8_META + wave * 1024), 16, 0, 0);
   }
   issue_pair(0);
@@ -273,14 +284,13 @@
       for (int e = 0; e < 16; ++e) acc[mi][0][e] = acc[mi][1][e] = 0.f;
   }
   int sh_r[2];
-  float mul_r[2], thr_f[2];
+  float mul_r[2];
 #pragma unroll
   for (int ni = 0; ni < 2; ++ni) {
     const int ql = wn * 64 + ni * 32 + (lane & 31);
     mul_r[ni] = ((const float*)(smem + G8_META + 1024))[ql];
-    thr_f[ni] = ((const float*)(smem + G8_META + 2048))[ql];
     sh_r[ni] = ts > 0 ? ((const int*)(smem + G8_META + 3072))[ql] : 0;
-    asm volatile("" : "+v"(mul_r[ni]), "+v"(thr_f[ni]), "+v"(sh_r[ni]));
+    asm volatile("" : "+v"(mul_r[ni]), "+v"(sh_r[ni]));
   }
   G8Frag f0, f1;
   if (ts > 0) {
@@ -291,7 +301,7 @@
   constexpr std::integral_constant<int, 0> PH0{};
   constexpr std::integral_constant<int, 1> PH1{};
   constexpr std::integral_constant<int, 2> PH2{};
-  dma_n = 0;
+  dma_n = 0; dma_thr = false;
 #pragma unroll 1
   for (int g = 0; g + 1 < nsp; ++g) {
     blk_s8(f0, f1, 2 * g + 1, true, PH1);
@@ -361,10 +371,7 @@
   if (DUMP) { g8_dump_tile(p, acc, dt, qt, wm, wn, lane, mul_r); return; }
   int thr_r[2];
 #pragma unroll
-  for (int ni = 0; ni < 2; ++ni) {
-    asm volatile("" : "+v"(thr_f[ni]));
-    thr_r[ni] = g8_thr_units(thr_f[ni], mul_r[ni]);
-  }
+  for (int ni = 0; ni < 2; ++ni) thr_r[ni] = g8_thr_units(((const float*)(smem + G8_META + 2048))[wn * 64 + ni * 32 + (lane & 31)], mul_r[ni]);
 #if G8_ABL == 32
   if (p.n_queries >= 0) { if (__float_as_int(acc[0][0][0]) == 0x7fffffff) p.cnt[0] = 1; return; }
 #endif
diff --git a/dhr_amd/csrc/index_build.hip b/dhr_amd/csrc/index_build.hip
--- a/dhr_amd/csrc/index_build.hip
+++ b/dhr_amd/csrc/index_build.hip
@@ -67,6 +67,7 @@
       if (value < 1 || value > 64) return set_error(DHR_ERR_INVALID, "main_chunks must be in [1,64]");
       ix->main_chunks = (int)value; return DHR_OK;
     case DHR_PARAM_PROGRESSIVE_THR: ix->progressive_thr = value < 0 ? 0 : (value > 2 ? 2 : (int)value); return DHR_OK;
+    case DHR_PARAM_CHUNK_RAMP: ix->chunk_ramp = value < 0 ? 0 : (value > 2 ? 2 : (int)value); return DHR_OK;
     case DHR_PARAM_AUX_CUS:
       if (value < 0 || value > 192 || value % 8) return set_error(DHR_ERR_INVALID, "aux_cus must be a multiple of 8 in [0,192]");
       ix->aux_cus = (int)value; return DHR_OK;
diff --git a/dhr_amd/csrc/kernels.hip b/dhr_amd/csrc/kernels.hip
--- a/dhr_amd/csrc/kernels.hip
+++ b/dhr_amd/csrc/kernels.hip
@@ -622,7 +622,7 @@
                                                            uint32_t* __restrict__ offs, uint32_t* __restrict__ out_max, uint32_t* __restrict__ out_max2,
                                                            unsigned long long* __restrict__ out_sum, unsigned long long* __restrict__ out_sum2,
                                                            uint32_t* __restrict__ fail_flags, uint32_t* __restrict__ zero, int n_zero,
-                                                           const uint32_t* __restrict__ ovf_cap) {
+                                                           const uint32_t* __restrict__ ovf_cap, unsigned long long* __restrict__ out_sum3) {
   __shared__ uint32_t part[1024];
   __shared__ uint32_t wmax[16];
   __shared__ unsigned long long wsum[16];
@@ -663,14 +663,15 @@
     if (out_max2) *out_max2 = m;
     if (out_sum) atomicAdd(out_sum, tot);
     if (out_sum2) atomicAdd(out_sum2, tot);
+    if (out_sum3) atomicAdd(out_sum3, tot);
   }
   for (int j = tid; j < n_zero; j += 1024) zero[j] = 0u;
 }
 hipError_t launch_lists_ready(const uint32_t* cnt, uint32_t cap, int n_queries, uint32_t per, uint32_t* offs, uint32_t* out_max, uint32_t* out_max2,
                               unsigned long long* out_sum, unsigned long long* out_sum2, uint32_t* fail_flags, uint32_t* zero, int n_zero,
-                              hipStream_t s, const uint32_t* ovf_cap) {
+                              hipStream_t s, const uint32_t* ovf_cap, unsigned long long* out_sum3) {
   hipLaunchKernelGGL(lists_ready_kernel, dim3(1), dim3(1024), 0, s, cnt, cap, n_queries, per, offs, out_max, out_max2, out_sum, out_sum2, fail_flags,
-                     zero, n_zero, ovf_cap);
+                     zero, n_zero, ovf_cap, out_sum3);
   return hipGetLastError();
 }
 __global__ void __launch_bounds__(1024) plan_overflow_kernel(const uint32_t* __restrict__ cnt_prev, double rows_ratio, uint32_t cap, uint32_t max_extra,
@@ -2152,9 +2153,10 @@
   hipLaunchKernelGGL(make_thr_kernel, dim3((q_pad + 255) / 256), dim3(256), 0, s, tau, margin, n_queries, q_pad, thr);
   return hipGetLastError();
 }
+__device__ __forceinline__ void publish_thr(float* p, float v) { __hip_atomic_store(p, v, __ATOMIC_RELAXED, __HIP_MEMORY_SCOPE_AGENT); }
 __global__ void raise_thr_kernel(float* __restrict__ thr_hat, const float* __restrict__ thr_run, int n_queries) {
   const int q = blockIdx.x * blockDim.x + threadIdx.x;
-  if (q < n_queries) thr_hat[q] = fmaxf(thr_hat[q], thr_run[q]);
+  if (q < n_queries) publish_thr(thr_hat + q, fmaxf(thr_hat[q], thr_run[q]));
 }
 hipError_t launch_raise_thr(float* thr_hat, const float* thr_run, int n_queries, hipStream_t s) {
   hipLaunchKernelGGL(raise_thr_kernel, dim3((n_queries + 255) / 256), dim3(256), 0, s, thr_hat, thr_run, n_queries);
@@ -2177,7 +2179,7 @@
   const float t = ordered_f32((uint32_t)(key >> 32));
   if (!(t > tau_hat[q])) return;
   tau_hat[q] = t;
-  thr_hat[q] = fmaxf(thr_hat[q], t - margin[q]);
+  publish_thr(thr_hat + q, fmaxf(thr_hat[q], t - margin[q]));
 }
 hipError_t launch_raise_thr_rank(float* thr_hat, float* tau_hat, const uint64_t* topk_keys, int kp, int r, const float* margin, int n_queries, hipStream_t s) {
   hipLaunchKernelGGL(raise_thr_rank_kernel, dim3((n_queries + 255) / 256), dim3(256), 0, s, thr_hat, tau_hat, topk_keys, kp, r, margin, n_queries);
diff --git a/dhr_amd/csrc/search_core.hip b/dhr_amd/csrc/search_core.hip
--- a/dhr_amd/csrc/search_core.hip
+++ b/dhr_amd/csrc/search_core.hip
@@ -1,5 +1,6 @@
 #include "dhr_state.h"
 
+static bool debug_plan_async() { const char* e = getenv("DHR_DEBUG_PLAN"); return e && strcmp(e, "async") == 0; }
 template <typename T>
 static hipError_t re_malloc(T*& p, size_t bytes, int64_t& total) {
   if (p) hipFree(p);
@@ -96,6 +97,7 @@
   HIP_TRY(hipHostMalloc(&w.h_ref, 16, hipHostMallocDefault));
   HIP_TRY(re_malloc(w.d_stats, 32, tot));
   HIP_TRY(hipHostMalloc(&w.h_stats, 32, hipHostMallocDefault));
+  HIP_TRY(re_malloc(w.d_chunk_stats, sizeof(unsigned long long) * 2 * MAX_MAIN_CHUNKS, tot));
   w.q_pad = w.q_alloc = q_pad; w.kp = kp; w.cap = cap; w.cap_deep = cap_deep; w.arena = arena; w.cap_r = cap_r; w.keys_ld = keys_ld; w.kt = ix->kt; w.d_dlr = ix->d_dlr;
   w.bytes = tot;
   return DHR_OK;
@@ -260,7 +262,7 @@
   return DHR_OK;
 }
 static int rescore_select_async(Search& c, const uint2* cand, const uint32_t* cnt, const float* thr, hipStream_t s, uint32_t* d_fullest_bound = nullptr,
-                                uint32_t* d_fullest = nullptr, const uint2* ovf = nullptr) {
+                                uint32_t* d_fullest = nullptr, const uint2* ovf = nullptr, unsigned long long* chunk_stats = nullptr) {
   dhr_index* ix = c.ix; Workspace& w = c.w; Timer& tm = c.tm; const int Q = c.Q;
   uint32_t list_cap = (uint32_t)w.cap;
   const bool refine = uses_refine(ix, c.gate);
@@ -268,7 +270,7 @@
   const uint32_t* ovf_cap = ovf ? w.ovf_cap : nullptr;
   HIP_TRY(launch_lists_ready(cnt, (uint32_t)w.cap, Q, refine ? (uint32_t)REFINE_PER_WG : (uint32_t)RESCORE_CANDS_PER_WG, refine ? w.blk_off : w.blk_off + w.q_pad + 1,
                              d_fullest_bound, refine ? nullptr : d_fullest, w.d_stats + 0, refine ? nullptr : w.d_stats + 1, w.fail_flags,
-                             refine ? w.cnt_r : nullptr, refine ? (int)w.q_pad : 0, s, ovf_cap));
+                             refine ? w.cnt_r : nullptr, refine ? (int)w.q_pad : 0, s, ovf_cap, chunk_stats));
   if (refine) {
     RefineArgs f = base_refine_args(ix, w, Q, c.gate, thr);
     f.ovf = ovf; f.ovf_off = ovf ? w.ovf_off : nullptr; f.ovf_cap = ovf_cap;
@@ -278,7 +280,7 @@
     list_cap = (uint32_t)w.cap_r;
     cand = w.cand_r; cnt = w.cnt_r;
     HIP_TRY(launch_lists_ready(cnt, list_cap, Q, (uint32_t)RESCORE_CANDS_PER_WG, w.blk_off + w.q_pad + 1, d_fullest, nullptr, w.d_stats + 1,
-                               nullptr, w.fail_flags, nullptr, 0, s));
+                               nullptr, w.fail_flags, nullptr, 0, s, nullptr, chunk_stats ? chunk_stats + 1 : nullptr));
   }
   return rescore_and_select(c, cand, cnt, list_cap, 1, FLAT_GRID_ASYNC, s);
 }
@@ -529,14 +531,20 @@
   mp.sb = overlap ? ix->s_aux : mp.sg;
   return DHR_OK;
 }
-static int main_chunk_count(const Search& c, const MainPass& mp, bool mid_proto) {
+static int main_chunk_count(const Search& c, const MainPass& mp, bool mid_proto, int64_t ramp_seen) {
   const dhr_index* ix = c.ix; const Workspace& w = c.w; const int64_t n_main = c.p.n_main; const double rate = c.rate, rate_r = c.rate_r;
   const bool plan_read = ix->async_ctl >= 2 && c.whole();
   const int64_t plan_cap = mp.two_tier ? w.cap_deep : w.cap;
   const int64_t need = std::max((int64_t)std::ceil(1.5 * rate * (double)n_main * TILE_ROWS / (double)plan_cap),
                                 (int64_t)std::ceil(1.5 * rate_r * (double)n_main * TILE_ROWS / (double)w.cap_r));
   int64_t by_size = std::min<int64_t>(8, std::max<int64_t>(2, (n_main + 4199) / 4200));
-  const int64_t no_overflow = (3 * n_main * TILE_ROWS + 2 * std::min(plan_cap, w.cap_r) - 1) / (2 * std::min(plan_cap, w.cap_r));
+  const int64_t slots = std::min(plan_cap, w.cap_r);
+  int64_t no_overflow = (3 * n_main * TILE_ROWS + 2 * slots - 1) / (2 * slots);
+  if (ramp_seen > 0) {
+    no_overflow = 13;
+    for (int m = 1; m <= 12 && no_overflow > 12; ++m)
+      if (plan::largest_chunk(plan::main_chunk_bounds(n_main, m, 0, ramp_seen)) * TILE_ROWS <= slots) no_overflow = m;
+  }
   if (no_overflow <= 12) by_size = std::max(by_size, no_overflow);
   {
     const double k_eff = (double)c.k / (double)std::max(1, c.whole() ? 1 : ix->sample_share);
@@ -584,7 +592,8 @@
     uint32_t* cnt = (i & 1) ? w.cnt2 : w.cnt;
     if (c.async_ctl) {
       if (sb != mp.sg) HIP_TRY(hipStreamWaitEvent(sb, mp.ev_gemm[i], 0));
-      if ((rc = rescore_select_async(c, cand, cnt, w.thr_hat, sb, nullptr, nullptr, mp.two_tier ? ((i & 1) ? w.ovf2 : w.ovf) : nullptr)) != DHR_OK) return rc;
+      if ((rc = rescore_select_async(c, cand, cnt, w.thr_hat, sb, nullptr, nullptr, mp.two_tier ? ((i & 1) ? w.ovf2 : w.ovf) : nullptr,
+                                     w.d_chunk_stats + 2 * i)) != DHR_OK) return rc;
     } else {
       HIP_TRY(hipEventSynchronize(mp.ev_gemm[i]));
       const uint32_t maxc = *(const uint32_t*)(w.h_pinned2 + 16 * (i & 1));
@@ -628,13 +637,16 @@
   if ((rc = main_streams(c, mp)) != DHR_OK) return rc;
   hipStream_t sg = mp.sg, sb = mp.sb;
   mp.two_tier = c.async_ctl && w.arena > 0;
-  mp.bound = plan::main_chunk_bounds(p.n_main, main_chunk_count(c, mp, mid_proto), mid_proto ? p.mid_offset : 0);
+  const int64_t seen_tiles = p.head + p.n_sample;
+  const bool ramp_on = mp.extrapolate && !mid_proto && (ix->chunk_ramp >= 2 || (ix->chunk_ramp == 1 && seen_tiles * (w.q_pad / TILE_ROWS) >= ix->n_cu));
+  const int64_t ramp_seen = ramp_on ? seen_tiles : 0;
+  mp.bound = plan::main_chunk_bounds(p.n_main, main_chunk_count(c, mp, mid_proto, ramp_seen), mid_proto ? p.mid_offset : 0, ramp_seen);
   if (mid_proto) mp.bound.insert(mp.bound.begin(), 0);
   mp.M = (int)mp.bound.size() - 1;
   mp.c_lo = c.after_mid ? 1 : 0; mp.c_hi = mid ? 1 : mp.M;
+  if (c.async_ctl) HIP_TRY(hipMemsetAsync(w.d_chunk_stats + 2 * mp.c_lo, 0, sizeof(unsigned long long) * 2 * (size_t)(mp.c_hi - mp.c_lo), s));
   if (mp.two_tier) {
-    int64_t big = 0;
-    for (int i = 0; i < mp.M; ++i) big = std::max(big, mp.bound[i + 1] - mp.bound[i]);
+    const int64_t big = plan::largest_chunk(mp.bound);
     HIP_TRY(launch_plan_overflow(w.plan_rows > 0 ? w.cnt_plan : nullptr, w.plan_rows > 0 ? (double)(big * TILE_ROWS) / (double)w.plan_rows : 0.0, (uint32_t)w.cap,
                                  (uint32_t)(w.cap_deep - w.cap), (uint32_t)w.arena, c.Q, w.ovf_off, w.ovf_cap, s));
   }
@@ -652,6 +664,19 @@
   }
   if ((rc = main_chunks(c, mp)) != DHR_OK) return rc;
   HIP_TRY(hipStreamWaitEvent(s, mp.ev_done[mp.c_hi - 1], 0));
+  if (c.async_ctl && debug_plan_async()) {
+    std::vector<unsigned long long> cs(2 * (size_t)MAX_MAIN_CHUNKS);
+    HIP_TRY(hipStreamSynchronize(s));
+    HIP_TRY(hipMemcpy(cs.data(), w.d_chunk_stats, cs.size() * sizeof(unsigned long long), hipMemcpyDeviceToHost));
+    const bool refine = uses_refine(ix, c.gate);
+    for (int i = mp.c_lo; i < mp.c_hi; ++i) {
+      const double tiles = (double)(mp.bound[i + 1] - mp.bound[i]);
+      const double nb = (double)cs[2 * (size_t)i], ne = (double)cs[2 * (size_t)i + (refine ? 1 : 0)];
+      fprintf(stderr, "[dhr] main chunk %2d: tiles [%lld, %lld) = %5.2f %% of the pass: bound %.1f, survivors = rescored %.1f per query; per query and 1000 tiles: %.1f / %.1f\n", i,
+              (long long)mp.bound[i], (long long)mp.bound[i + 1], 100.0 * tiles / (double)std::max<int64_t>(1, p.n_main), nb / c.Q, ne / c.Q,
+              1000.0 * nb / c.Q / tiles, 1000.0 * ne / c.Q / tiles);
+    }
+  }
   return DHR_OK;
 }
 
@@ -728,7 +753,7 @@
   const SearchPlan& p = c.p;
   int rc;
   if ((rc = ensure_ws(ix, w, c.Q, k, p.first_valid, depth == 0 ? 1 : 16, c.gate || ix->gated_i8 || ix->resid8 != nullptr)) != DHR_OK) return rc;
-  c.async_ctl = depth == 0 && p.S >= 2 && ix->async_ctl != 0 && !getenv("DHR_DEBUG_PLAN");
+  c.async_ctl = depth == 0 && p.S >= 2 && ix->async_ctl != 0 && (!getenv("DHR_DEBUG_PLAN") || debug_plan_async());
   SelectArgs& sel = c.sel;
   sel.topk_keys = w.topk_keys; sel.in_keys = w.rs_keys; sel.ld_keys = w.keys_ld; sel.cap = (uint32_t)w.cap;
   sel.k = p.r_eff; sel.kp = w.kp; sel.sort_n = select_sort_n(w.kp);
diff --git a/dhr_amd/csrc/search_plan.h b/dhr_amd/csrc/search_plan.h
--- a/dhr_amd/csrc/search_plan.h
+++ b/dhr_amd/csrc/search_plan.h
@@ -96,17 +96,58 @@
   }
   return p;
 }
-inline std::vector<int64_t> main_chunk_bounds(int64_t n_main, int M_plain, int64_t mid_offset) {
+inline int64_t largest_chunk(const std::vector<int64_t>& b) {
+  int64_t big = 0;
+  for (size_t i = 0; i + 1 < b.size(); ++i) big = std::max(big, b[i + 1] - b[i]);
+  return big;
+}
+inline std::vector<int64_t> main_chunk_bounds(int64_t n_main, int M_plain, int64_t mid_offset, int64_t ramp_seen = 0) {
   std::vector<int64_t> b((size_t)M_plain + 1, 0);
   b[0] = mid_offset;
+  const int64_t span = n_main - mid_offset;
+  auto weight = [&](int i) { return 1.0 + 2.0 * (M_plain - 1 - i) / std::max(1, M_plain - 1); };
+  bool ramp = ramp_seen > 0 && M_plain >= 2 && M_plain < 62 && span > 0;
+  if (ramp && (double)ramp_seen * (std::ldexp(1.0, M_plain) - 1.0) < (double)span) ramp = false;
+  std::vector<double> sizes((size_t)M_plain, 0.0);
+  if (ramp) {
+    auto covered = [&](double lambda, std::vector<double>* sizes) {
+      double seen = (double)ramp_seen, sum = 0.0;
+      for (int i = 0; i < M_plain; ++i) {
+        const double s = std::min(seen, lambda * weight(i));
+        if (sizes) (*sizes)[(size_t)i] = s;
+        sum += s; seen += s;
+      }
+      return sum;
+    };
+    double lo = 0.0, hi = (double)span;
+    for (int it = 0; it < 64; ++it) {
+      const double mid = 0.5 * (lo + hi);
+      if (covered(mid, nullptr) < (double)span) lo = mid; else hi = mid;
+    }
+    covered(hi, &sizes);
+    bool capped = false;
+    for (int i = 0; i < M_plain; ++i) capped = capped || sizes[(size_t)i] < hi * weight(i) * (1.0 - 1e-9);
+    ramp = capped;
+  }
+  if (ramp) {
+    double acc = 0.0;
+    for (int i = 0; i < M_plain; ++i) {
+      acc += sizes[(size_t)i];
+      const int64_t seen_i = ramp_seen + (b[(size_t)i] - mid_offset);
+      const int64_t e = std::min(mid_offset + (int64_t)acc / DOC_GROUP * DOC_GROUP, b[(size_t)i] + seen_i / DOC_GROUP * DOC_GROUP);
+      b[(size_t)i + 1] = std::min<int64_t>(n_main, std::max(e, b[(size_t)i] + DOC_GROUP));
+    }
+    b[(size_t)M_plain] = n_main;
+  }
   double acc = 0.0, tot = 0.0;
-  for (int i = 0; i < M_plain; ++i) tot += 1.0 + 2.0 * (M_plain - 1 - i) / std::max(1, M_plain - 1);
+  std::vector<int64_t> plain((size_t)M_plain + 1, mid_offset);
+  for (int i = 0; i < M_plain; ++i) tot += weight(i);
   for (int i = 0; i < M_plain; ++i) {
-    acc += 1.0 + 2.0 * (M_plain - 1 - i) / std::max(1, M_plain - 1);
-    b[(size_t)i + 1] = std::min<int64_t>(n_main, mid_offset + round_up((int64_t)((n_main - mid_offset) * acc / tot), DOC_GROUP));
+    acc += weight(i);
+    plain[(size_t)i + 1] = std::min<int64_t>(n_main, mid_offset + round_up((int64_t)((n_main - mid_offset) * acc / tot), DOC_GROUP));
   }
-  b[(size_t)M_plain] = n_main;
-  return b;
+  plain[(size_t)M_plain] = n_main;
+  return (ramp && 4 * largest_chunk(b) <= 5 * largest_chunk(plain)) ? b : plain;
 }
 
 }
diff --git a/include/dhr_hip.h b/include/dhr_hip.h
--- a/include/dhr_hip.h
+++ b/include/dhr_hip.h
@@ -78,6 +78,7 @@
   DHR_PARAM_ASYNC_CONTROLLER = 13,
   DHR_PARAM_SAMPLE_SHARE = 12,
   DHR_PARAM_LIST_STRIDE = 14,
+  DHR_PARAM_CHUNK_RAMP = 15,
   DHR_PARAM_SAMPLE_PERIOD = 5
 } dhr_param;
 
```

New measurement: 61910, median of 4. About the same (+0.6%).
